# pbenner/kmerLr

Measured on NVIDIA B200. Metric: kmer_sequences_per_sec, higher is better.
Workload: dtype f64

## Files before the change

### kmerlr_b200/csrc/abi.cu

```cuda
#include <cmath>
#include <map>
#include <mutex>
#include <unordered_map>
#include <vector>

#include "common.cuh"

namespace kl {

namespace {
Ctx g_ctx;
std::mutex g_mutex;
std::unordered_map<uint64_t, std::shared_ptr<Object>> g_objects;
uint64_t g_next = 1;
thread_local std::string g_error;
}

Ctx &ctx() { return g_ctx; }

namespace {
std::multimap<size_t, void *> g_free_blocks;
std::unordered_map<void *, size_t> g_block_size;
constexpr size_t ARENA_GRAIN = (size_t)2 << 20;
}
void *arena_alloc(size_t bytes) {
  size_t want = (bytes + ARENA_GRAIN - 1) / ARENA_GRAIN * ARENA_GRAIN;
  auto it = g_free_blocks.lower_bound(want);
  if (it != g_free_blocks.end() && it->first <= 2 * want + 8 * ARENA_GRAIN) {
    void *p = it->second;
    g_free_blocks.erase(it);
    return p;
  }
  void *p = nullptr;
  cudaError_t e = cudaMalloc(&p, want);
  if (e != cudaSuccess) {
    cudaGetLastError();
    cudaStreamSynchronize(g_ctx.stream);
    for (auto &kv : g_free_blocks) { cudaFree(kv.second); g_block_size.erase(kv.second); }
    g_free_blocks.clear();
    KL_CUDA(cudaMalloc(&p, want));
  }
  g_block_size[p] = want;
  return p;
}
void arena_free(void *p) {
  auto it = g_block_size.find(p);
  if (it == g_block_size.end()) return;
  g_free_blocks.emplace(it->second, p);
}
void arena_release_all() {
  for (auto &kv : g_block_size) cudaFree(kv.first);
  g_block_size.clear();
  g_free_blocks.clear();
}

namespace {
struct ProfRec { std::string name; cudaEvent_t e0, e1; };
std::vector<ProfRec> g_prof_pending;
std::vector<cudaEvent_t> g_prof_pool;
std::unordered_map<std::string, std::pair<double, int64_t>> g_prof_totals;
cudaEvent_t prof_event() {
  if (!g_prof_pool.empty()) { cudaEvent_t e = g_prof_pool.back(); g_prof_pool.pop_back(); return e; }
  cudaEvent_t e;
  KL_CUDA(cudaEventCreate(&e));
  return e;
}
void prof_resolve() {
  if (g_prof_pending.empty()) return;
  KL_CUDA(cudaStreamSynchronize(g_ctx.stream));
  for (auto &r : g_prof_pending) {
    float ms = 0.f;
    KL_CUDA(cudaEventElapsedTime(&ms, r.e0, r.e1));
    auto &t = g_prof_totals[r.name];
    t.first += ms; t.second += 1;
    g_prof_pool.push_back(r.e0); g_prof_pool.push_back(r.e1);
  }
  g_prof_pending.clear();
}
}
void profile_begin(const char *name) {
  if (g_prof_pending.size() > 8192) prof_resolve();
  ProfRec r{name, prof_event(), prof_event()};
  KL_CUDA(cudaEventRecord(r.e0, g_ctx.stream));
  g_prof_pending.push_back(r);
}
void profile_end() { KL_CUDA(cudaEventRecord(g_prof_pending.back().e1, g_ctx.stream)); }

void require_ready() {
  if (!g_ctx.ready) fail(KMERLR_ERR_NOGPU, "kmerlr_init() has not succeeded: no usable sm_100 GPU (there is no CPU fallback)");
}

uint64_t register_object(std::shared_ptr<Object> o) {
  uint64_t h = g_next++;
  g_objects[h] = std::move(o);
  return h;
}
std::shared_ptr<Object> lookup_object(uint64_t h) {
  auto it = g_objects.find(h);
  return it == g_objects.end() ? nullptr : it->second;
}

template <typename F>
int guarded(F &&f, bool timed = true) {
  std::lock_guard<std::mutex> lock(g_mutex);
  try {
    if (g_ctx.ready) KL_CUDA(cudaSetDevice(g_ctx.device));
    if (timed && g_ctx.ready) KL_CUDA(cudaEventRecord(g_ctx.ev0, g_ctx.stream));
    f();
    if (timed && g_ctx.ready) {
      KL_CUDA(cudaEventRecord(g_ctx.ev1, g_ctx.stream));
      KL_CUDA(cudaEventSynchronize(g_ctx.ev1));
      float ms = 0.f;
      KL_CUDA(cudaEventElapsedTime(&ms, g_ctx.ev0, g_ctx.ev1));
      g_ctx.last_ms = ms;
    }
    return KMERLR_OK;
  } catch (const Error &e) {
    g_error = e.msg;
    if (g_ctx.ready) cudaGetLastError();
    return e.code;
  } catch (const std::exception &e) {
    g_error = e.what();
    return KMERLR_ERR_INTERNAL;
  }
}

}

using namespace kl;

extern "C" {

int kmerlr_version(void) { return 100; }

const char *kmerlr_last_error(void) { return g_error.c_str(); }

double kmerlr_last_device_ms(void) { return g_ctx.last_ms; }

int64_t kmerlr_launch_count(void) { return g_ctx.launches; }

int kmerlr_profile(int enable) {
  return guarded([&] {
    prof_resolve();
    if (enable) g_prof_totals.clear();
    g_ctx.profiling = enable != 0;
  }, false);
}

int kmerlr_profile_read(const char *kernel_substr, double *ms_total, int64_t *launches) {
  return guarded([&] {
    prof_resolve();
    double ms = 0.0; int64_t n = 0;
    for (auto &kv : g_prof_totals)
      if (kv.first.find(kernel_substr) != std::string::npos) { ms += kv.second.first; n += kv.second.second; }
    *ms_total = ms; *launches = n;
  }, false);
}

int kmerlr_profile_dump(char *buf, int64_t buflen) {
  return guarded([&] {
    prof_resolve();
    std::string out;
    for (auto &kv : g_prof_totals)
      out += kv.first + "\t" + std::to_string(kv.second.first) + "\t" + std::to_string(kv.second.second) + "\n";
    KL_REQUIRE((int64_t)out.size() + 1 <= buflen, "profile_dump: buffer too small");
    memcpy(buf, out.c_str(), out.size() + 1);
  }, false);
}

int kmerlr_option(const char *name, int64_t value) {
  return guarded([&] {
    KL_REQUIRE(name != nullptr, "option: null name");
    if (!strcmp(name, "implicit")) g_ctx.implicit_ok = value != 0;
    else if (!strcmp(name, "super_len")) g_ctx.super_len = (int)(value < 0 ? -1 : (value > IMP_SUPER_MAX ? IMP_SUPER_MAX : value));
    else if (!strcmp(name, "p2p")) g_ctx.p2p_ok = value != 0;
    else if (!strcmp(name, "feed_growth")) g_ctx.feed_growth = (int)(value < 100 ? 100 : (value > 400 ? 400 : value));
    else if (!strcmp(name, "small_long")) g_ctx.small_long = (int)(value < 0 ? -1 : (value > 2 ? 2 : value));
    else if (!strcmp(name, "persist_bps")) g_ctx.persist_bps = (int)(value < 0 ? 0 : value);
    else if (!strcmp(name, "p2p_allreduce")) g_ctx.p2p_allreduce = value != 0;
    else if (!strcmp(name, "persistent")) g_ctx.coop_ok = value != 0 && g_ctx.coop_supported;
    else if (!strcmp(name, "fused_ticket")) g_ctx.fused_ticket = (int)(value < 0 ? 0 : (value > 4096 ? 4096 : value));
    else if (!strcmp(name, "hot_cols")) g_ctx.hot_cols = (int)(value < 0 ? 0 : (value > 16384 ? 16384 : value));
    else fail(KMERLR_ERR_ARG, std::string("unknown option ") + name);
  }, false);
}

int kmerlr_init(int device) {
  return guarded([&] {
    if (g_ctx.ready) {
      KL_REQUIRE(device == g_ctx.device, "kmerlr_init: already initialised on another device");
      return;
    }
    int count = 0;
    cudaError_t e = cudaGetDeviceCount(&count);
    if (e != cudaSuccess || count == 0) {
      cudaGetLastError();
      fail(KMERLR_ERR_NOGPU, "no CUDA device visible (there is no CPU fallback)");
    }
    KL_REQUIRE(device >= 0 && device < count, "kmerlr_init: device index out of range");
    cudaDeviceProp prop;
    KL_CUDA(cudaGetDeviceProperties(&prop, device));
    if (prop.major != 10) fail(KMERLR_ERR_NOGPU, std::string("device is ") + prop.name + " (sm_" + std::to_string(prop.major) + std::to_string(prop.minor) + "); this library is built for sm_100a only");
    KL_CUDA(cudaSetDevice(device));
    g_ctx.device = device;
    g_ctx.sm_count = prop.multiProcessorCount;
    g_ctx.coop_supported = prop.cooperativeLaunch != 0;
    g_ctx.coop_ok = g_ctx.coop_supported;
    KL_CUDA(cudaStreamCreateWithFlags(&g_ctx.stream, cudaStreamNonBlocking));
    KL_CUDA(cudaStreamCreateWithFlags(&g_ctx.copy_stream, cudaStreamNonBlocking));
    KL_CUDA(cudaStreamCreateWithFlags(&g_ctx.alt_stream, cudaStreamNonBlocking));
    for (int i = 0; i < 2; i++) KL_CUDA(cudaEventCreateWithFlags(&g_ctx.join_ev[i], cudaEventDisableTiming));
    for (int i = 0; i < CTX_COPY_EVENTS; i++) KL_CUDA(cudaEventCreateWithFlags(&g_ctx.copy_ev[i], cudaEventDisableTiming));

    KL_CUDA(cudaEventCreate(&g_ctx.ev0));
    KL_CUDA(cudaEventCreate(&g_ctx.ev1));
    g_ctx.ready = true;
  }, false);
}

int kmerlr_shutdown(void) {
  return guarded([&] {
    g_objects.clear();
    if (g_ctx.ready) {
      cudaStreamSynchronize(g_ctx.stream);
      arena_release_all();
      comm_destroy();
      cudaEventDestroy(g_ctx.ev0); cudaEventDestroy(g_ctx.ev1);
      cudaStreamSynchronize(g_ctx.copy_stream);
      for (int i = 0; i < CTX_COPY_EVENTS; i++) cudaEventDestroy(g_ctx.copy_ev[i]);
      cudaStreamDestroy(g_ctx.copy_stream);
      cudaStreamSynchronize(g_ctx.alt_stream);
      cudaStreamDestroy(g_ctx.alt_stream);
      for (int i = 0; i < 2; i++) cudaEventDestroy(g_ctx.join_ev[i]);
      cudaStreamDestroy(g_ctx.stream);
      g_ctx = Ctx();
    }
  }, false);
}

int kmerlr_comm_unique_id(void *id128) { return guarded([&] { comm_unique_id(id128); }, false); }
int kmerlr_comm_init(int rank, int world, const void *id128) { return guarded([&] { comm_init(rank, world, id128); }, false); }
int kmerlr_comm_destroy(void) { return guarded([&] { comm_destroy(); }, false); }

int kmerlr_sequences_create(const uint8_t *seq, const int64_t *off, int64_t n, kmerlr_handle *out) {
  return guarded([&] {
    KL_REQUIRE(out, "null output handle");
    *out = register_object(sequences_create(seq, off, n));
  });
}

int kmerlr_extract_resident(const kmerlr_config *cfg, kmerlr_handle sequences, const int32_t *frozen_k,
                            const uint64_t *frozen_code, int64_t n_frozen, const int32_t *features,
                            int64_t n_features, int flags, kmerlr_handle *out) {
  return guarded([&] {
    KL_REQUIRE(cfg && out, "null argument");
    auto s = lookup<SeqSet>(sequences, "sequences");
    *out = register_object(extract(*cfg, s, frozen_k, frozen_code, n_frozen, features, n_features, flags));
  });
}

int kmerlr_extract(const kmerlr_config *cfg, const uint8_t *seq, const int64_t *off, int64_t n,
                   const int32_t *frozen_k, const uint64_t *frozen_code, int64_t n_frozen,
                   const int32_t *features, int64_t n_features, int flags, kmerlr_handle *out) {
  return guarded([&] {
    KL_REQUIRE(cfg && out, "null argument");
    *out = register_object(extract_host(*cfg, seq, off, n, frozen_k, frozen_code, n_frozen, features, n_features, flags));
  });
}

int kmerlr_matrix_info(kmerlr_handle h, int64_t *n, int64_t *m, int64_t *nnz, int64_t *n_classes) {
  return guarded([&] {
    auto M = lookup<Matrix>(h, "matrix");
    if (n) *n = M->n;
    if (m) *m = M->m;
    if (nnz) *nnz = M->nnz;
    if (n_classes) *n_classes = M->n_classes;
  }, false);
}

int kmerlr_matrix_rows_global(kmerlr_handle h, int64_t *n_global) {
  return guarded([&] {
    KL_REQUIRE(n_global, "null argument");
    *n_global = lookup<Matrix>(h, "matrix")->n_global;
  }, false);
}

int kmerlr_matrix_classes(kmerlr_handle h, int32_t *k_out, uint64_t *code_out) {
  return guarded([&] {
    auto M = lookup<Matrix>(h, "matrix");
    matrix_class_list(*M);
    for (size_t j = 0; j < M->class_k.size(); j++) { k_out[j] = M->class_k[j]; code_out[j] = M->class_code[j]; }
  }, false);
}

int kmerlr_matrix_rows(kmerlr_handle h, int64_t *rowptr, int32_t *col, double *val) {
  return guarded([&] { matrix_rows(*lookup<Matrix>(h, "matrix"), rowptr, col, val); });
}

int kmerlr_matrix_set_labels(kmerlr_handle h, const uint8_t *labels, int64_t n) {
  return guarded([&] { matrix_set_labels(*lookup<Matrix>(h, "matrix"), labels, n); });
}

int kmerlr_matrix_from_csr(int64_t n, int64_t m, const int64_t *rowptr, const int32_t *col, const double *val,
                           int flags, kmerlr_handle *out) {
  return guarded([&] {
    KL_REQUIRE(out, "null output handle");
    *out = register_object(matrix_from_csr(n, m, rowptr, col, val, flags));
  });
}

// ... 204 lines not shown
```

### kmerlr_b200/csrc/common.cuh

```cuda
#pragma once

#include <cuda_runtime.h>
#include <stdint.h>

#include <chrono>
#include <cstdio>
#include <cstdlib>
#include <cstring>
#include <memory>
#include <string>
#include <vector>

#include "../../include/kmerlr_b200.h"

namespace kl {

struct Error {
  int code;
  std::string msg;
};

[[noreturn]] inline void fail(int code, const std::string &msg) { throw Error{code, msg}; }

#define KL_CUDA(expr)                                                                              \
  do {                                                                                             \
    cudaError_t _e = (expr);                                                                       \
    if (_e != cudaSuccess)                                                                         \
      ::kl::fail(KMERLR_ERR_CUDA, std::string(#expr) + ": " + cudaGetErrorString(_e) + " (" +      \
                                      __FILE__ + ":" + std::to_string(__LINE__) + ")");            \
  } while (0)

#define KL_REQUIRE(cond, msg)                                                                      \
  do {                                                                                             \
    if (!(cond)) ::kl::fail(KMERLR_ERR_ARG, std::string(msg));                                     \
  } while (0)

#define KL_INVARIANT(cond)                                                                         \
  do {                                                                                             \
    if (!(cond)) ::kl::fail(KMERLR_ERR_INTERNAL, std::string("internal error: ") + #cond + " (" +  \
                                                     __FILE__ + ":" + std::to_string(__LINE__) + ")"); \
  } while (0)

constexpr int PEER_MAX_WORLD = 8;
constexpr int PEER_PAYLOAD = 1024 + 8;
struct PeerMail {
  unsigned long long slot[2][PEER_MAX_WORLD][PEER_PAYLOAD];
  unsigned long long flag[2][PEER_MAX_WORLD];
  unsigned long long seq;
  unsigned int senders_done;
  unsigned long long ar_flag[2][PEER_MAX_WORLD];
  unsigned long long ar_seq;
  unsigned int ar_error;
};
constexpr int64_t PEER_AR_CAP = (int64_t)4 << 20;
struct PeerBox {
  PeerMail *box[PEER_MAX_WORLD];
  unsigned long long *sym[PEER_MAX_WORLD];
  int rank, world;
};

constexpr int CTX_COPY_EVENTS = 11;
struct Ctx {
  bool ready = false;
  int device = 0;
  int sm_count = 0;
  cudaStream_t stream = nullptr;
  cudaStream_t copy_stream = nullptr;
  cudaStream_t alt_stream = nullptr;
  cudaEvent_t join_ev[2] = {nullptr, nullptr};
  cudaEvent_t copy_ev[CTX_COPY_EVENTS] = {nullptr};
  cudaEvent_t ev0 = nullptr, ev1 = nullptr;
  int64_t launches = 0;
  double last_ms = 0.0;
  bool profiling = false;
  bool implicit_ok = true;
  int super_len = -1;
  int hot_cols = 6144;
  int fused_ticket = 8;
  void *comm = nullptr;
  int rank = 0, world = 1;
  PeerBox *peer = nullptr;
  bool p2p_ok = true;
  bool p2p_allreduce = false;
  int feed_growth = 135;
  int small_long = -1;
  int persist_bps = 0;
  bool coop_supported = true;
  bool coop_ok = true;
};
Ctx &ctx();
void require_ready();

void profile_begin(const char *name);
void profile_end();

#define KL_LAUNCH(kernel, grid, block, smem, ...)                                                  \
  do {                                                                                             \
    if (::kl::ctx().profiling) ::kl::profile_begin(#kernel);                                       \
    kernel<<<(grid), (block), (smem), ::kl::ctx().stream>>>(__VA_ARGS__);                          \
    if (::kl::ctx().profiling) ::kl::profile_end();                                                \
    ::kl::ctx().launches++;                                                                        \
    KL_CUDA(cudaGetLastError());                                                                   \
  } while (0)

inline void sync_stream() { KL_CUDA(cudaStreamSynchronize(ctx().stream)); }

struct Trace {
  bool on;
  std::chrono::steady_clock::time_point t0, last;
  const char *what;
  explicit Trace(const char *w) : what(w) {
    static int env = -1;
    if (env < 0) { const char *e = getenv("KMERLR_TRACE"); env = (e && *e == '1') ? 1 : 0; }
    on = env == 1;
    if (on) t0 = last = std::chrono::steady_clock::now();
  }
  void mark(const char *phase, bool sync = true) {
    if (!on) return;
    if (sync) cudaStreamSynchronize(ctx().stream);
    auto t = std::chrono::steady_clock::now();
    fprintf(stderr, "[trace %s] %-28s %8.3f ms (total %8.3f)\n", what, phase,
            std::chrono::duration<double, std::milli>(t - last).count(),
            std::chrono::duration<double, std::milli>(t - t0).count());
    last = t;
  }
};

void *arena_alloc(size_t bytes);
void arena_free(void *p);
void arena_release_all();

template <typename T>
struct DevBuf {
  T *p = nullptr;
  size_t n = 0;
  DevBuf() = default;
  explicit DevBuf(size_t count) { alloc(count); }
  DevBuf(const DevBuf &) = delete;
  DevBuf &operator=(const DevBuf &) = delete;
  DevBuf(DevBuf &&o) noexcept : p(o.p), n(o.n) { o.p = nullptr; o.n = 0; }
  DevBuf &operator=(DevBuf &&o) noexcept {
    if (this != &o) { release(); p = o.p; n = o.n; o.p = nullptr; o.n = 0; }
    return *this;
  }
  ~DevBuf() { release(); }
  void alloc(size_t count) {
    release();
    n = count;
    if (count) p = (T *)arena_alloc(count * sizeof(T) + 32);
  }
  void release() {
    if (p) arena_free(p);
    p = nullptr; n = 0;
  }
  void zero() { if (n) KL_CUDA(cudaMemsetAsync(p, 0, n * sizeof(T), ctx().stream)); }
  void upload(const T *h, size_t count) {
    if (count) KL_CUDA(cudaMemcpyAsync(p, h, count * sizeof(T), cudaMemcpyHostToDevice, ctx().stream));
  }
  void download(T *h, size_t count) const {
    if (count) KL_CUDA(cudaMemcpyAsync(h, p, count * sizeof(T), cudaMemcpyDeviceToHost, ctx().stream));
  }
  size_t bytes() const { return n * sizeof(T); }
};

struct Object {
  virtual ~Object() {}
};

struct SeqSet : Object {
  int64_t n = 0;
  int64_t total_bases = 0;
  int64_t total_blocks = 0;
  int64_t max_len = 0;
  DevBuf<int64_t> len;
  DevBuf<int64_t> blk;
  DevBuf<uint32_t> bits2;
  DevBuf<uint16_t> inv16;
};

enum ValType : int { VAL_ONE = 0, VAL_U32 = 1, VAL_F64 = 2 };

constexpr int IMP_MAX_N = 10;
constexpr int IMP_SUPER_MAX = 11;
constexpr uint32_t NOCOL = 0xFFFFFFFFu;
struct Implicit {
  std::shared_ptr<SeqSet> seqs;
  int M = 0, N = 0, op = 0;
  int Mlo = 0;
  uint32_t level_off[16] = {0};
  uint32_t fo[16] = {0};
  DevBuf<uint32_t> bitmap, rank;
  bool binarized = false;
  int low_words = 0;
  DevBuf<uint32_t> lowbits;
  DevBuf<uint32_t> lowcol;
  DevBuf<int64_t> evptr;
  DevBuf<uint32_t> events;
};

struct Rows {
  const int64_t *rowptr;
  const uint32_t *rowcnt;
  int64_t stride;
#ifdef __CUDACC__
  __device__ __forceinline__ void range(int64_t row, int64_t &a, int64_t &b) const {
    if (stride) { a = row * stride; b = a + rowcnt[row]; }
    else { a = rowptr[row]; b = rowptr[row + 1]; }
  }
#endif
};

struct Matrix : Object {
  int64_t n = 0, m = 0, nnz = 0;
  ValType vt = VAL_U32;
  int64_t row_stride = 0;
  DevBuf<uint32_t> rowcnt;
  DevBuf<int64_t> rowptr;
  DevBuf<uint32_t> col;
  DevBuf<uint32_t> val_u32;
  DevBuf<double> val_f64;
  Rows rows() const { return Rows{rowptr.p, rowcnt.p, row_stride}; }
  bool has_csc = false;
  DevBuf<int64_t> colptr;
  DevBuf<uint32_t> crow;
  DevBuf<uint32_t> cval_u32;
  DevBuf<double> cval_f64;
  bool has_sliced = false;
  DevBuf<int64_t> slice_off;
  DevBuf<uint32_t> scol;
  DevBuf<uint32_t> sval_u32;
  DevBuf<double> sval_f64;
  bool has_packed = false, packable = false;
  int pack_row_bits = 0;
  DevBuf<uint32_t> spack, cpack;
  int bv_grid = 0, bv_row_bits = 0, bv_rows = 0;
  bool bv_ok = false;
  DevBuf<int64_t> bv_off;
  DevBuf<uint32_t> bv_pack;
  bool has_labels = false;
  DevBuf<uint8_t> labels;
  int64_t n_pos = 0, n_neg = 0;
  bool counts_global = true;
  int64_t n_classes = 0;
  DevBuf<uint32_t> class_ids;
  int class_M = 0, class_N = 0;
  uint32_t class_level_off[16] = {0};
  bool classes_on_host = true;
  std::vector<int32_t> class_k;
  std::vector<uint64_t> class_code;
  bool sharded = false;
  int64_t n_global = 0;
  bool has_maxsq = false;
  double maxsq = 0.0;
  bool has_vmax = false;
  double vmax = 0.0;
  std::shared_ptr<Implicit> imp;
  bool has_local_stats = false;
  double local_maxsq = 0.0, local_vmax = 0.0;
};

uint64_t register_object(std::shared_ptr<Object> o);
std::shared_ptr<Object> lookup_object(uint64_t h);
template <typename T>
std::shared_ptr<T> lookup(uint64_t h, const char *what) {
  auto o = std::dynamic_pointer_cast<T>(lookup_object(h));
  if (!o) fail(KMERLR_ERR_ARG, std::string("invalid ") + what + " handle");
  return o;
}

void exclusive_scan_i64(const int64_t *in, int64_t *out, int64_t n);
void exclusive_scan_u32_to_i64(const uint32_t *in, int64_t *out, int64_t n);
void exclusive_scan_u32(const uint32_t *in, uint32_t *out, int64_t n);
std::shared_ptr<SeqSet> sequences_create(const uint8_t *seq, const int64_t *off, int64_t n);
struct SeqFeed {
  virtual ~SeqFeed() {}
  virtual int chunks() const = 0;
  virtual int64_t first_row(int c) const = 0;
  virtual void feed(int c) = 0;
};
std::shared_ptr<SeqSet> sequences_begin_chunked(const uint8_t *seq, const int64_t *off, int64_t n, std::unique_ptr<SeqFeed> &feed);
std::shared_ptr<Matrix> extract(const kmerlr_config &cfg, std::shared_ptr<SeqSet> seqs, const int32_t *frozen_k,
                                const uint64_t *frozen_code, int64_t n_frozen, const int32_t *features,
                                int64_t n_features, int flags);
std::shared_ptr<Matrix> extract_host(const kmerlr_config &cfg, const uint8_t *seq, const int64_t *off, int64_t n,
                                     const int32_t *frozen_k, const uint64_t *frozen_code, int64_t n_frozen,
                                     const int32_t *features, int64_t n_features, int flags);
std::shared_ptr<Matrix> extract_gapped(const kmerlr_config &cfg, std::shared_ptr<SeqSet> seqs, const int32_t *frozen_k,
                                       const uint64_t *frozen_code, int64_t n_frozen, int flags);
void matrix_class_list(Matrix &M);
std::shared_ptr<Matrix> matrix_from_csr(int64_t n, int64_t m, const int64_t *rowptr, const int32_t *col,
                                        const double *val, int flags);
void matrix_rows(Matrix &M, int64_t *rowptr, int32_t *col, double *val);
void matrix_set_labels(Matrix &M, const uint8_t *labels, int64_t n);
void matrix_label_counts(Matrix &M);
void matrix_column_moments(Matrix &M, double *sum, double *sumsq, double *absmax, int64_t *count);
void matrix_pair_moments(Matrix &M, double *sum, double *sumsq, double *absmax, int64_t *count);
std::shared_ptr<Matrix> matrix_transform(Matrix &M, const double *offset, const double *scale, int64_t len);
void matrix_compact(Matrix &M);
void ensure_csc(Matrix &M);
void ensure_sliced(Matrix &M);
bool ensure_packed(Matrix &M);
bool ensure_blockview(Matrix &M, int grid);
std::shared_ptr<Matrix> matrix_reduce(Matrix &M, const int64_t *sel, int64_t nsel);
double matrix_maxsq(Matrix &M);
double matrix_vmax(Matrix &M);
void linear_pdf(Matrix &M, const double *theta, int64_t ntheta, int cooc, double *out_host, bool logpdf);
void gradient(Matrix &M, const double *theta, int64_t ntheta, const double cw[2], double lambda, int cooc,
              double *g_host, DevBuf<double> *g_dev = nullptr);
double loss(Matrix &M, const double *theta, int64_t ntheta, const double cw[2], double lambda, int cooc);
void coordinate(Matrix &M, double *theta, int64_t ntheta, const double cw_hook[2], double l1reg, double l2reg,
                double epsilon, double epsilon_loss, int64_t max_iter, double hook[2], int64_t *sweeps_out,
                double *delta_out);
void proxgrad(Matrix &M, double *theta, int64_t ntheta, const double cw[2], double lambda, double l2,
              double step_factor, double epsilon, double epsilon_loss, int64_t max_iter, double hook[2],
              int64_t *iters, double *delta);
void select(Matrix &M, const double cw[2], int cooc, int64_t N, double theta0, const int64_t *active_idx,
            const double *active_theta, int64_t n_active, int tie, double eps_lambda, double prev_lambda,
            uint8_t *mask, int64_t ntheta, double *lambda_out, int64_t *c_out, int *ok_out, double *g_out);
void select_from_gradient(const double *g, int64_t ntheta, int64_t N, const int64_t *active_idx, const double *active_theta,
                          int64_t n_active, int tie, double eps_lambda, double prev_lambda, uint8_t *mask,
                          double *lambda_out, int64_t *c_out, int *ok_out);
void score_windows(const kmerlr_model *models, int n_models, const SeqSet &s, int64_t W, int64_t step,
                   double *out_host, std::shared_ptr<Object> *out_dev, int layout = 0, SeqFeed *feed = nullptr);
int64_t wiggle_records(const double *pred, bool pred_on_device, int64_t n, char *out);
void save_wiggle(const char *filename, const char *track_name, int64_t n_regions, const char *const *seqnames,
                 const int64_t *from, const int64_t *slot_off, const double *pred, bool pred_on_device, int64_t window_size,
                 int64_t window_step);
std::string class_name(const kmerlr_config &cfg, int k, uint64_t code);
void export_kmers(Matrix &M, const kmerlr_config &cfg, const char *filename, bool as_float);
void export_path(const char *filename, int64_t n, const int64_t *estimator, const double *lambda, const double *norm,
                 const int64_t *theta_off, const double *theta);
void export_trace(const char *filename, int64_t n, const int64_t *duration_ns, const int64_t *iteration, const double *change,
                  const int64_t *nonzero, const double *lambda, const double *loss);

void comm_unique_id(void *id128);
void comm_init(int rank, int world, const void *id128);
void comm_destroy();
void comm_allreduce_sum_f64(double *dev, int64_t count);
void comm_allreduce_sum_i64(int64_t *dev, int64_t count);
void comm_allreduce_sum_i64_fast(int64_t *dev, int64_t count);
void comm_check_peer_errors();
void comm_allreduce_max_f64(double *dev, int64_t count);
void comm_allreduce_max_u8(uint8_t *dev, int64_t count);
void comm_allgather_f64(const double *dev_in, double *dev_out, int64_t count_per_rank);
void comm_allgather_bytes(const void *dev_in, void *dev_out, int64_t bytes_per_rank);

#ifdef __CUDACC__
__device__ __forceinline__ unsigned lane_id() { return threadIdx.x & 31u; }
__device__ __forceinline__ unsigned lanemask_lt() {
  unsigned m;
  asm("mov.u32 %0, %%lanemask_lt;" : "=r"(m));
  return m;
}
__device__ __forceinline__ uint32_t swap_pairs(uint32_t y) {
  return ((y >> 1) & 0x55555555u) | ((y & 0x55555555u) << 1);
}
__device__ __forceinline__ uint32_t kmer_op(uint32_t u, int k, int op) {
  if (op == 1) return swap_pairs(__brev(~u)) >> (32 - 2 * k);
  if (op == 2) return (~u) & ((1u << (2 * k)) - 1u);
  return swap_pairs(__brev(u)) >> (32 - 2 * k);
}
__device__ __forceinline__ double warp_sum(double v) {
#pragma unroll
  for (int o = 16; o > 0; o >>= 1) v += __shfl_xor_sync(0xffffffffu, v, o);
  return v;
}
__device__ __forceinline__ double warp_sum_down(double v) {
#pragma unroll
  for (int o = 16; o > 0; o >>= 1) v += __shfl_down_sync(0xffffffffu, v, o);
  return v;
}
__device__ __forceinline__ uint32_t smem_u32(const void *p) { return (uint32_t)__cvta_generic_to_shared(p); }
__device__ __forceinline__ void mbar_init(unsigned long long *bar, uint32_t arrivals) {
  asm volatile("mbarrier.init.shared::cta.b64 [%0], %1;" ::"r"(smem_u32(bar)), "r"(arrivals) : "memory");
  asm volatile("fence.mbarrier_init.release.cluster;" ::: "memory");
}
// ... 27 lines not shown
```

### kmerlr_b200/csrc/extract.cu

```cuda
#include <cmath>

#include "extract_kernel.cuh"

namespace kl {

namespace {

using namespace xk;

__global__ void pack_kernel(const uint8_t *__restrict__ seq, const int64_t *__restrict__ off,
                            const int64_t *__restrict__ blk, int64_t n, int64_t total_blocks, int64_t w0, int64_t w1,
                            uint32_t *__restrict__ bits2, uint16_t *__restrict__ inv16) {
  int64_t w = w0 + (int64_t)blockIdx.x * blockDim.x + threadIdx.x;
  if (w >= w1) return;
  const int64_t b = w >> 2;
  int64_t g = (int64_t)((double)b * (double)n / (double)total_blocks);
  g = g < 0 ? 0 : (g > n - 1 ? n - 1 : g);
  int64_t lo, hi, stepw = 1;
  if (blk[g] <= b) {
    lo = g; hi = g + 1;
    while (hi < n && blk[hi] <= b) { lo = hi; stepw <<= 1; hi = hi + stepw < n ? hi + stepw : n; }
  } else {
    hi = g; lo = g - 1;
    while (lo > 0 && blk[lo] > b) { hi = lo; stepw <<= 1; lo = lo - stepw > 0 ? lo - stepw : 0; }
// ... 7 lines not shown
  uint32_t bits = 0, inv = 0;
#pragma unroll
  for (int j = 0; j < 16; j++) {
    if (j0 + j < L) {
      uint32_t ch = s[j0 + j] | 0x20u, c;
      if (ch == 'a') c = 0; else if (ch == 'c') c = 1; else if (ch == 'g') c = 2; else if (ch == 't') c = 3;
      else { c = 0; inv |= 1u << j; }
      bits |= c << (2 * j);
    }
  }
  bits2[w] = bits;
  inv16[w] = (uint16_t)inv;
}

__global__ void popc_words(const uint32_t *__restrict__ bm, int64_t nw, uint32_t *__restrict__ out) {
  int64_t i = (int64_t)blockIdx.x * blockDim.x + threadIdx.x;
  if (i < nw) out[i] = __popc(bm[i]);
}
__global__ void pack_exchange(const uint32_t *__restrict__ bm, int64_t nw, unsigned long long n_local,
                              const unsigned long long *__restrict__ stats, uint32_t *__restrict__ out) {
  int64_t i = (int64_t)blockIdx.x * blockDim.x + threadIdx.x;
  if (i < nw) out[i] = bm[i];
  if (i == 0) {
    unsigned long long v[3] = {n_local, stats[0], stats[1]};
    for (int k = 0; k < 3; k++) { out[nw + 2 * k] = (uint32_t)v[k]; out[nw + 2 * k + 1] = (uint32_t)(v[k] >> 32); }
  }
}
__global__ void merge_exchange(const uint32_t *__restrict__ all, int world, int64_t nw, uint32_t *__restrict__ bm,
                               unsigned long long *__restrict__ res) {
  int64_t i = (int64_t)blockIdx.x * blockDim.x + threadIdx.x;
  const int64_t per = nw + 6;
  if (i < nw) {
    uint32_t v = 0;
    for (int r = 0; r < world; r++) v |= all[(int64_t)r * per + i];
    bm[i] = v;
  }
  if (i == 0) {
    unsigned long long n = 0, a = 0, b = 0;
    for (int r = 0; r < world; r++) {
      const uint32_t *t = all + (int64_t)r * per + nw;
      n += (unsigned long long)t[0] | ((unsigned long long)t[1] << 32);
      const unsigned long long x = (unsigned long long)t[2] | ((unsigned long long)t[3] << 32);
      const unsigned long long y = (unsigned long long)t[4] | ((unsigned long long)t[5] << 32);
      a = x > a ? x : a; b = y > b ? y : b;
    }
    res[0] = n; res[1] = a; res[2] = b;
  }
}
__global__ void enumerate_bits(const uint32_t *__restrict__ bm, const uint32_t *__restrict__ rank, int64_t nw,
                               uint32_t *__restrict__ ids) {
  int64_t w = (int64_t)blockIdx.x * blockDim.x + threadIdx.x;
  if (w >= nw) return;
  uint32_t v = bm[w], r = rank[w];
  while (v) {
    int b = __ffs(v) - 1;
    ids[r++] = (uint32_t)(w * 32 + b);
    v &= v - 1;
  }
}

struct LevelInfo {
  int M, N, op;
  uint32_t level_off[16];
};
__global__ void all_classes_bits(const LevelInfo I, uint32_t *__restrict__ bm, int64_t nw) {
  int64_t w = (int64_t)blockIdx.x * blockDim.x + threadIdx.x;
  if (w >= nw) return;
  const uint32_t id0 = (uint32_t)(w * 32);
  int k = I.M;
  while (k < I.N && id0 >= I.level_off[k + 1]) k++;
  const uint32_t u0 = id0 - I.level_off[k], nk = 1u << (2 * k);
  uint32_t v = 0;
  for (int b = 0; b < 32; b++) {
    const uint32_t u = u0 + b;
    if (u < nk && (I.op == 0 || u <= kmer_op(u, k, I.op))) v |= 1u << b;
  }
  bm[w] = v;
}
__global__ void interleave_numbering(const uint32_t *__restrict__ bits, const uint32_t *__restrict__ rank, int64_t nw,
                                     uint2 *__restrict__ out) {
  int64_t w = (int64_t)blockIdx.x * blockDim.x + threadIdx.x;
  if (w < nw) out[w] = make_uint2(bits[w], rank[w]);
}
__global__ void bitmaps_differ(const uint32_t *__restrict__ a, const uint32_t *__restrict__ b, int64_t nw,
                               uint32_t *__restrict__ flag) {
  int64_t w = (int64_t)blockIdx.x * blockDim.x + threadIdx.x;
  if (w < nw && a[w] != b[w]) atomicOr(flag, 1u);
}
__global__ void renumber_rows(uint32_t *__restrict__ col, const uint32_t *__restrict__ rowcnt, int64_t stride, int64_t n,
                              const uint32_t *__restrict__ ids, const uint32_t *__restrict__ bm,
                              const uint32_t *__restrict__ rank, const uint32_t *__restrict__ rowdup) {
  int64_t row = ((int64_t)blockIdx.x * blockDim.x + threadIdx.x) >> 5;
  if (row >= n) return;
  const unsigned lane = lane_id();
  uint32_t *c = col + row * stride;
  const uint32_t cnt = rowcnt[row];
  for (uint32_t j = lane; j < cnt; j += 32) {
    const uint32_t id = __ldg(ids + c[j]), w = __ldg(bm + (id >> 5));
    c[j] = __ldg(rank + (id >> 5)) + __popc(w & ((1u << (id & 31)) - 1u));
  }
  const uint32_t nd = rowdup ? rowdup[row] : 0u;
  uint32_t *t = c + stride - 1;
  for (uint32_t j = lane; j < nd; j += 32) {
    const uint32_t id = __ldg(ids + t[-(int64_t)j]), w = __ldg(bm + (id >> 5));
    t[-(int64_t)j] = __ldg(rank + (id >> 5)) + __popc(w & ((1u << (id & 31)) - 1u));
  }
}
__global__ void gather_events(const uint32_t *__restrict__ col, int64_t stride, int64_t n,
                              const int64_t *__restrict__ evptr, uint32_t *__restrict__ events) {
  int64_t row = ((int64_t)blockIdx.x * blockDim.x + threadIdx.x) >> 5;
  if (row >= n) return;
  const unsigned lane = lane_id();
  const int64_t a = evptr[row], cnt = evptr[row + 1] - a;
  const uint32_t *t = col + (row + 1) * stride - 1;
  for (int64_t j = lane; j < cnt; j += 32) events[a + j] = t[-j];
}
__global__ void low_columns(const uint2 *__restrict__ tl, uint32_t tl_cnt, int slots, const uint32_t *__restrict__ bm,
                            const uint32_t *__restrict__ rank, uint32_t *__restrict__ lowcol) {
  const int j = blockIdx.x * blockDim.x + threadIdx.x;
  if (j >= slots) return;
  uint32_t col = NOCOL;
  if ((uint32_t)j < tl_cnt) {
    const uint32_t id = tl[j].y, w = bm[id >> 5], bit = 1u << (id & 31);
    if (w & bit) col = rank[id >> 5] + __popc(w & (bit - 1u));
  }
  lowcol[j] = col;
}

__device__ __forceinline__ uint32_t row_lookup(const uint32_t *col, const uint32_t *val, int64_t a, int64_t b, uint32_t c) {
  int64_t lo = a, hi = b;
  while (lo < hi) {
    int64_t mid = (lo + hi) >> 1;
    if (col[mid] < c) lo = mid + 1; else hi = mid;
  }
  if (lo < b && col[lo] == c) return val ? val[lo] : 1u;
  return 0u;
}
template <bool WRITE>
__global__ void features_rows(const Rows R, const uint32_t *__restrict__ col,
                              const uint32_t *__restrict__ val, int64_t n, const int32_t *__restrict__ feat,
                              int64_t nf, uint32_t *__restrict__ cnt_out, const int64_t *__restrict__ orowptr,
                              uint32_t *__restrict__ ocol, uint32_t *__restrict__ oval) {
  int64_t row = ((int64_t)blockIdx.x * blockDim.x + threadIdx.x) >> 5;
  if (row >= n) return;
  unsigned lane = lane_id();
  int64_t a, b;
  R.range(row, a, b);
  int64_t outp = WRITE ? orowptr[row] : 0;
  uint32_t tot = 0;
  for (int64_t j0 = 0; j0 < nf; j0 += 32) {
    int64_t j = j0 + lane;
    uint32_t v = 0;
    if (j < nf) {
      int32_t i1 = feat[2 * j], i2 = feat[2 * j + 1];
      uint32_t c1 = row_lookup(col, val, a, b, (uint32_t)i1);
      if (i1 == i2) v = c1;
      else if (c1) v = c1 * row_lookup(col, val, a, b, (uint32_t)i2);
    }
    unsigned km = __ballot_sync(0xffffffffu, v != 0);
    if (WRITE && v != 0) {
      int64_t pos = outp + __popc(km & lanemask_lt());
      ocol[pos] = (uint32_t)j;
      if (oval) oval[pos] = v;
    }
    outp += __popc(km);
    tot += __popc(km);
  }
  if (!WRITE && lane == 0) cnt_out[row] = tot;
}

// ... 115 lines not shown
  hf.doff.alloc((size_t)n + 1);
  hf.doff.upload(off, (size_t)n + 1);
  s->len.alloc((size_t)(n ? n : 1));
  s->blk.alloc((size_t)n + 1);
  if (n > 0) {
    DevBuf<uint32_t> nblk((size_t)n);
    KL_LAUNCH(seq_meta_kernel, (unsigned)((n + 255) / 256), 256, 0, hf.doff.p, n, s->len.p, nblk.p);
    exclusive_scan_u32_to_i64(nblk.p, s->blk.p, n);
  } else {
    s->blk.zero();
  }
  const int64_t words = blocks * 4;
  s->bits2.alloc((size_t)words + 4);
  s->inv16.alloc((size_t)words + 4);
  KL_CUDA(cudaMemsetAsync(s->bits2.p + words, 0, 4 * sizeof(uint32_t), ctx().stream));
  KL_CUDA(cudaMemsetAsync(s->inv16.p + words, 0, 4 * sizeof(uint16_t), ctx().stream));
  hf.raw.alloc((size_t)(s->total_bases ? s->total_bases : 1));
  KL_CUDA(cudaEventRecord(ctx().copy_ev[CTX_COPY_EVENTS - 1], ctx().stream));
  KL_CUDA(cudaStreamWaitEvent(ctx().copy_stream, ctx().copy_ev[CTX_COPY_EVENTS - 1], 0));
  tr.mark("offsets, metadata");
  return s;
}

namespace {
struct FeedImpl : SeqFeed {
  HostFeed hf;
  std::shared_ptr<SeqSet> s;
  int chunks() const override { return hf.nchunks; }
  int64_t first_row(int c) const override { return hf.row[c]; }
  void feed(int c) override { if (s->n > 0) hf.feed(*s, c); }
};
}

std::shared_ptr<SeqSet> sequences_begin_chunked(const uint8_t *seq, const int64_t *off, int64_t n, std::unique_ptr<SeqFeed> &feed) {
  auto f = std::make_unique<FeedImpl>();
  f->s = sequences_begin(seq, off, n, f->hf, true);
  auto s = f->s;
  feed = std::move(f);
  return s;
}

std::shared_ptr<SeqSet> sequences_create(const uint8_t *seq, const int64_t *off, int64_t n) {
  HostFeed hf;
  auto s = sequences_begin(seq, off, n, hf);
  if (n > 0) hf.feed(*s, -1);
  sync_stream();
  return s;
}

static std::shared_ptr<Matrix> apply_features(Matrix &cls, const int32_t *features, int64_t nf) {
  for (int64_t j = 0; j < nf; j++) {
    KL_REQUIRE(features[2 * j] >= 0 && features[2 * j] < cls.m && features[2 * j + 1] >= 0 && features[2 * j + 1] < cls.m,
               "features: class index out of range");
  }
  auto out = std::make_shared<Matrix>();
  out->n = cls.n; out->m = nf; out->vt = cls.vt;
  matrix_class_list(cls);
  out->class_k = cls.class_k; out->class_code = cls.class_code; out->n_classes = cls.n_classes;
  out->sharded = cls.sharded; out->n_global = cls.n_global;
  DevBuf<int32_t> dfeat((size_t)(2 * nf));
  dfeat.upload(features, (size_t)(2 * nf));
  DevBuf<uint32_t> cnt((size_t)(cls.n ? cls.n : 1));
  const uint32_t *val = cls.vt == VAL_U32 ? cls.val_u32.p : nullptr;
  unsigned grid = (unsigned)((cls.n * 32 + 127) / 128);
  out->rowptr.alloc((size_t)cls.n + 1);
  if (cls.n > 0) {
    KL_LAUNCH((features_rows<false>), grid, 128, 0, cls.rows(), cls.col.p, val, cls.n, dfeat.p, nf, cnt.p, nullptr,
              nullptr, nullptr);
    exclusive_scan_u32_to_i64(cnt.p, out->rowptr.p, cls.n);
    KL_CUDA(cudaMemcpyAsync(&out->nnz, out->rowptr.p + cls.n, sizeof(int64_t), cudaMemcpyDeviceToHost, ctx().stream));
    sync_stream();
  } else {
    out->rowptr.zero(); out->nnz = 0;
  }
  out->col.alloc((size_t)(out->nnz ? out->nnz : 1));
  if (out->vt == VAL_U32) out->val_u32.alloc((size_t)(out->nnz ? out->nnz : 1));
  if (cls.n > 0)
    KL_LAUNCH((features_rows<true>), grid, 128, 0, cls.rows(), cls.col.p, val, cls.n, dfeat.p, nf, nullptr,
              out->rowptr.p, out->col.p, out->vt == VAL_U32 ? out->val_u32.p : nullptr);
  sync_stream();
  return out;
}

static std::shared_ptr<Matrix> extract_impl(const kmerlr_config &cfg, std::shared_ptr<SeqSet> seqs,
                                            const int32_t *frozen_k, const uint64_t *frozen_code, int64_t n_frozen,
                                            const int32_t *features, int64_t n_features, int flags, HostFeed *feed) {
  require_ready();
  const SeqSet &s = *seqs;
  KL_REQUIRE(cfg.alphabet == 0 || cfg.alphabet == 1, "alphabet: 0 = nucleotide, 1 = gapped nucleotide (IUPAC is not implemented)");
  if (cfg.alphabet == 1) {
    KL_REQUIRE(n_features == 0 || n_frozen > 0, "an explicit feature list needs a frozen class list");
    if (feed && s.n > 0) feed->feed(*seqs, -1);
    auto g = extract_gapped(cfg, seqs, frozen_k, frozen_code, n_frozen, flags);
    if (n_features > 0) return apply_features(*g, features, n_features);
    return g;
  }
  KL_REQUIRE(cfg.M >= 1 && cfg.M <= cfg.N, "need 1 <= M <= N");
  KL_REQUIRE(n_features == 0 || n_frozen > 0, "an explicit feature list needs a frozen class list");
  {
    const int nops = (cfg.complement != 0) + (cfg.reverse != 0) + (cfg.revcomp != 0);
    const bool long_sorted = cfg.N > KB_MAX && (s.max_len + 31) / 32 > 64;
    const bool long_tables = s.max_len >= 65536 && cfg.M <= KT_MAX;
    if (nops > 1 || cfg.N > MAX_N || long_sorted || long_tables) {
      if (feed && s.n > 0) feed->feed(*seqs, -1);
      auto g = extract_gapped(cfg, seqs, frozen_k, frozen_code, n_frozen, flags);
      if (n_features > 0) return apply_features(*g, features, n_features);
      return g;
    }
  }
  const bool sharded = (flags & KMERLR_FLAG_SHARDED) != 0 && ctx().world > 1;

  XParams P{};
  P.M = cfg.M; P.N = cfg.N; P.binarize = cfg.binarize != 0;
  P.op = cfg.revcomp ? 1 : (cfg.complement ? 2 : (cfg.reverse ? 3 : 0));
  P.t_lo = cfg.M; P.t_hi = cfg.N < KT_MAX ? cfg.N : KT_MAX;
  const int64_t steps = (s.max_len + 31) / 32;
  const int kb = steps > 64 ? KB_MAX : KB_DEFAULT;
  P.b_lo = cfg.M > KT_MAX + 1 ? cfg.M : KT_MAX + 1; P.b_hi = cfg.N < kb ? cfg.N : kb;
  P.s_lo = cfg.M > kb + 1 ? cfg.M : kb + 1;
  P.n = s.n;
  P.len = s.len.p; P.blk = s.blk.p; P.bits2 = s.bits2.p; P.inv16 = s.inv16.p;
  uint64_t dense = 0;
  for (int k = cfg.M; k <= cfg.N; k++) {
    P.level_off[k] = (uint32_t)dense;
    dense += ((1ull << (2 * k)) + 31) / 32 * 32;
  }
  P.level_off[cfg.N + 1] = (uint32_t)dense;
  const int64_t nbits = (int64_t)dense, nw = (nbits + 31) / 32;
  int64_t stride = 0;
  for (int k = cfg.M; k <= cfg.N; k++) {
    int64_t inst = s.max_len - k + 1; if (inst < 0) inst = 0;
    int64_t cls = (int64_t)1 << (2 * k);
    stride += inst < cls ? inst : cls;
  }
  if (stride < 1) stride = 1;
  P.stride = stride;
  bool hybrid = P.binarize && cfg.N <= IMP_MAX_N && n_features == 0 && s.n > 0;
  for (int k = cfg.M > KT_MAX + 1 ? cfg.M : KT_MAX + 1; k <= cfg.N && hybrid; k++)
    if (s.max_len - k + 1 > ((int64_t)1 << (2 * k))) hybrid = false;
  KL_INVARIANT(s.max_len < 65536 || P.t_lo > P.t_hi);
  KL_REQUIRE(s.max_len < ((int64_t)1 << 30), "sequence too long");
  int E = 0;
  if (P.s_lo <= cfg.N) {
    E = 2; while (E < steps && E < 128) E <<= 1;
    KL_INVARIANT(E <= 64);
  }
  P.bm_words = 0; P.pf_words = 0;
  int nbl = 0;
  for (int k = P.b_lo; k <= P.b_hi; k++) {
    P.bm_off[k] = (uint32_t)P.bm_words; P.pf_off[k] = (uint32_t)P.pf_words;
    P.bm_words += 1 << (2 * k - 5); P.pf_words += 1 << (2 * k - 7);
    nbl++;
  }
  P.pf_words = (P.pf_words + 3) / 4 * 4;
  P.ts_words = 32 * E > TAB_WORDS ? 32 * E : TAB_WORDS;
  P.warp_words = P.bm_words + P.pf_words + P.ts_words + 8;
  P.warp_words = (P.warp_words + 3) / 4 * 4;
  {
    int top = cfg.N < OBS_MAX_LEVEL ? cfg.N : OBS_MAX_LEVEL;
    P.obs_id_words = top >= cfg.M ? (int)(P.level_off[top + 1] / 32) : 0;
    P.obs_id_words = (P.obs_id_words + 3) / 4 * 4;
  }
  if (P.t_lo <= P.t_hi) P.tl = table_classes(P.op, P.t_lo, P.t_hi, P.level_off, &P.tl_cnt);
  P.obs_words = P.obs_id_words + (P.t_lo <= P.t_hi ? (int)((P.tl_cnt + 127) / 128 * 4) : 0);
  Trace tr("extract");
  auto out = std::make_shared<Matrix>();
  out->n = s.n; out->vt = P.binarize ? VAL_ONE : VAL_U32;
  out->sharded = sharded; out->n_global = s.n;
  out->row_stride = stride;
  out->col.alloc((size_t)(s.n ? s.n * stride : 1));
  if (!P.binarize) out->val_u32.alloc((size_t)(s.n ? s.n * stride : 1));
  out->rowcnt.alloc((size_t)(s.n ? s.n : 1));
  DevBuf<uint32_t> dummy_cnt(1);
  DevBuf<uint32_t> nb((size_t)nw), nbrank((size_t)nw + 1), pc((size_t)nw), bitmap((size_t)nw);
  std::vector<uint32_t> frozen_bits;
  LevelInfo LI{};
  LI.M = cfg.M; LI.N = cfg.N; LI.op = P.op;
  for (int k = cfg.M; k <= cfg.N + 1; k++) LI.level_off[k] = P.level_off[k];
  if (n_frozen > 0) {
    frozen_bits.assign((size_t)nw, 0u);
    uint64_t prev = 0;
    for (int64_t j = 0; j < n_frozen; j++) {
      int k = frozen_k[j];
      KL_REQUIRE(k >= cfg.M && k <= cfg.N && frozen_code[j] < (1ull << (2 * k)), "frozen class outside [M,N]");
      uint64_t id = (uint64_t)P.level_off[k] + frozen_code[j];
      KL_REQUIRE(j == 0 || id > prev, "frozen class list must be sorted by (k, code) without duplicates");
      prev = id;
      frozen_bits[id >> 5] |= 1u << (id & 31);
    }
    nb.upload(frozen_bits.data(), (size_t)nw);
  } else {
    KL_LAUNCH(all_classes_bits, (unsigned)((nw + 255) / 256), 256, 0, LI, nb.p, nw);
  }
  KL_LAUNCH(popc_words, (unsigned)((nw + 255) / 256), 256, 0, nb.p, nw, pc.p);
  exclusive_scan_u32(pc.p, nbrank.p, nw);
  bitmap.zero();
  DevBuf<uint32_t> full(1);
  full.zero();
  P.full = full.p; P.nb_words = nw;
  DevBuf<unsigned long long> stats(2);
  stats.zero();
  P.st_id = out->col.p; P.st_cnt = P.binarize ? dummy_cnt.p : out->val_u32.p; P.rowcnt = out->rowcnt.p;
  DevBuf<uint2> nbx((size_t)nw);
  KL_LAUNCH(interleave_numbering, (unsigned)((nw + 255) / 256), 256, 0, nb.p, nbrank.p, nw, nbx.p);
  P.bitmap = bitmap.p; P.nbx = nbx.p; P.filter = n_frozen > 0; P.stats = stats.p;
  P.mark = n_frozen == 0;
  DevBuf<uint32_t> lowbits, rowdup;
  if (hybrid) {
    P.events = 1;
    P.low_words = P.t_lo <= P.t_hi ? (int)((P.tl_cnt + 31) / 32) : 0;
    if (P.low_words) { lowbits.alloc((size_t)s.n * P.low_words); P.lowbits = lowbits.p; }
    rowdup.alloc((size_t)s.n);
    P.rowdup = rowdup.p;
  }
  DevBuf<uint32_t> ovf;
  P.ovf_stride = nbl * (s.max_len > 0 ? s.max_len : 1);
  if (nbl && (!P.binarize || hybrid) && s.n > 0) {
    ovf.alloc((size_t)ctx().sm_count * 64 * (size_t)P.ovf_stride);
    P.ovf = ovf.p;
  }
  tr.mark("alloc");

  if (s.n > 0) {
    const int nchunks = feed ? feed->nchunks : 1;
    DevBuf<uint32_t> ticket((size_t)nchunks);
    ticket.zero();
    const bool two_streams = feed && nchunks > 1;
    DevBuf<uint32_t> ovf2;
    if (two_streams && P.ovf) ovf2.alloc((size_t)ctx().sm_count * 64 * (size_t)P.ovf_stride);
    struct StreamSwap {
      cudaStream_t saved;
      explicit StreamSwap(cudaStream_t run) : saved(ctx().stream) { ctx().stream = run; }
      ~StreamSwap() { ctx().stream = saved; }
    };
    if (two_streams) {
      KL_CUDA(cudaEventRecord(ctx().join_ev[0], ctx().stream));
      KL_CUDA(cudaStreamWaitEvent(ctx().alt_stream, ctx().join_ev[0], 0));
    }
    uint32_t *const ovf_even = P.ovf;
    for (int c = 0; c < nchunks; c++) {
      StreamSwap on((two_streams && (c & 1)) ? ctx().alt_stream : ctx().stream);
      P.ovf = (two_streams && (c & 1) && ovf_even) ? ovf2.p : ovf_even;
      P.ticket = ticket.p + c;
      const int64_t r0 = feed ? feed->row[c] : 0, r1 = feed ? feed->row[c + 1] : s.n;
      if (feed) feed->feed(*seqs, c);
      P.row0 = r0; P.n = r1;
      switch (E) {
        case 0: launch_extract<0>(P); break;
        case 2: launch_extract<2>(P); break;
        case 4: launch_extract<4>(P); break;
        case 8: launch_extract<8>(P); break;
        case 16: launch_extract<16>(P); break;
        case 32: launch_extract<32>(P); break;
        default: launch_extract<64>(P); break;
      }
    }
    P.ovf = ovf_even;
    if (two_streams) {
      KL_CUDA(cudaEventRecord(ctx().join_ev[1], ctx().alt_stream));
      KL_CUDA(cudaStreamWaitEvent(ctx().stream, ctx().join_ev[1], 0));
    }
    P.row0 = 0; P.n = s.n;
  }
  tr.mark("extract_kernel");
  DevBuf<uint32_t> differ(1);
  differ.zero();
  DevBuf<unsigned long long> gres(3);
  if (sharded) {
    const int64_t xw = n_frozen == 0 ? nw : 0, per = xw + 6;
    DevBuf<uint32_t> mine((size_t)per), all((size_t)(per * ctx().world));
    KL_LAUNCH(pack_exchange, (unsigned)((xw + 256) / 256), 256, 0, bitmap.p, xw, (unsigned long long)s.n, stats.p, mine.p);
    comm_allgather_bytes(mine.p, all.p, per * 4);
    KL_LAUNCH(merge_exchange, (unsigned)((xw + 256) / 256), 256, 0, all.p, ctx().world, xw, bitmap.p, gres.p);
  }
  if (n_frozen == 0)
    KL_LAUNCH(bitmaps_differ, (unsigned)((nw + 255) / 256), 256, 0, bitmap.p, nb.p, nw, differ.p);
  DevBuf<int64_t> rp((size_t)s.n + 1);
  if (s.n > 0) exclusive_scan_u32_to_i64(out->rowcnt.p, rp.p, s.n); else rp.zero();
  int64_t nn = s.n;
  unsigned long long hres[3] = {0, 0, 0};
  if (sharded) gres.download(hres, 3);
  uint32_t m32 = 0, hdiffer = 0;
  unsigned long long hstats[2] = {0, 0};
  DevBuf<int64_t> evptr;
  int64_t n_events = 0;
  if (hybrid) {
    evptr.alloc((size_t)s.n + 1);
    exclusive_scan_u32_to_i64(rowdup.p, evptr.p, s.n);
    KL_CUDA(cudaMemcpyAsync(&n_events, evptr.p + s.n, sizeof(int64_t), cudaMemcpyDeviceToHost, ctx().stream));
  }
  KL_CUDA(cudaMemcpyAsync(&m32, nbrank.p + nw, sizeof(uint32_t), cudaMemcpyDeviceToHost, ctx().stream));
  KL_CUDA(cudaMemcpyAsync(&out->nnz, rp.p + s.n, sizeof(int64_t), cudaMemcpyDeviceToHost, ctx().stream));
  differ.download(&hdiffer, 1);
  stats.download(hstats, 2);
  sync_stream();
  if (sharded) {
    nn = (int64_t)hres[0];
    out->maxsq = (double)hres[1]; out->vmax = (double)hres[2];
    out->has_maxsq = out->has_vmax = true;
  }
  out->n_global = nn;
  out->has_local_stats = true;
  out->local_maxsq = (double)hstats[0]; out->local_vmax = (double)hstats[1];
  tr.mark("sizes");
  if (hdiffer) {
    DevBuf<uint32_t> rank2((size_t)nw + 1), ids_nb((size_t)(m32 ? m32 : 1));
    KL_LAUNCH(popc_words, (unsigned)((nw + 255) / 256), 256, 0, bitmap.p, nw, pc.p);
    exclusive_scan_u32(pc.p, rank2.p, nw);
    KL_LAUNCH(enumerate_bits, (unsigned)((nw + 255) / 256), 256, 0, nb.p, nbrank.p, nw, ids_nb.p);
    if (s.n > 0)
      KL_LAUNCH(renumber_rows, (unsigned)((s.n * 32 + 127) / 128), 128, 0, out->col.p, out->rowcnt.p, stride, s.n, ids_nb.p,
                bitmap.p, rank2.p, hybrid ? rowdup.p : (const uint32_t *)nullptr);
    KL_CUDA(cudaMemcpyAsync(&m32, rank2.p + nw, sizeof(uint32_t), cudaMemcpyDeviceToHost, ctx().stream));
    sync_stream();
    nb = std::move(bitmap); nbrank = std::move(rank2);
    tr.mark("renumber");
  }
  out->m = (int64_t)m32;
  out->n_classes = (int64_t)m32;
  out->class_ids.alloc((size_t)(m32 ? m32 : 1));
  KL_LAUNCH(enumerate_bits, (unsigned)((nw + 255) / 256), 256, 0, nb.p, nbrank.p, nw, out->class_ids.p);
  out->class_M = cfg.M; out->class_N = cfg.N; out->classes_on_host = false;
  for (int k = cfg.M; k <= cfg.N + 1; k++) out->class_level_off[k] = P.level_off[k];
  if (n_features > 0) { sync_stream(); return apply_features(*out, features, n_features); }
  if ((!P.binarize || hybrid) && cfg.N <= IMP_MAX_N && s.n > 0 && m32 > 0) {
    auto imp = std::make_shared<Implicit>();
    imp->seqs = seqs; imp->M = cfg.M; imp->N = cfg.N; imp->op = P.op;
    imp->Mlo = P.binarize ? (cfg.M > KT_MAX + 1 ? cfg.M : KT_MAX + 1) : cfg.M;
    uint32_t fo = 0;
    for (int k = cfg.M; k <= cfg.N + 1; k++) {
      imp->level_off[k] = P.level_off[k];
      imp->fo[k] = fo;
      if (k <= cfg.N && k >= imp->Mlo) fo += 1u << (2 * k);
    }
    if (P.binarize) {
      imp->binarized = true;
      imp->low_words = P.low_words;
      imp->lowcol.alloc((size_t)(P.low_words ? P.low_words * 32 : 1));
      if (P.low_words)
        KL_LAUNCH(low_columns, (unsigned)((P.low_words * 32 + 127) / 128), 128, 0, P.tl, P.tl_cnt, P.low_words * 32, nb.p,
                  nbrank.p, imp->lowcol.p);
      imp->lowbits = std::move(lowbits);
      imp->events.alloc((size_t)(n_events ? n_events : 1));
      KL_LAUNCH(gather_events, (unsigned)((s.n * 32 + 127) / 128), 128, 0, out->col.p, stride, s.n, evptr.p, imp->events.p);
      imp->evptr = std::move(evptr);
    }
    imp->bitmap = std::move(nb); imp->rank = std::move(nbrank);
    out->imp = imp;
  }
  sync_stream();
  return out;
}

void matrix_class_list(Matrix &M) {
  if (M.classes_on_host) return;
  std::vector<uint32_t> hid((size_t)M.n_classes);
  M.class_ids.download(hid.data(), (size_t)M.n_classes);
  sync_stream();
  M.class_k.resize((size_t)M.n_classes); M.class_code.resize((size_t)M.n_classes);
  int k = M.class_M;
  for (size_t j = 0; j < hid.size(); j++) {
    while (k < M.class_N && hid[j] >= M.class_level_off[k + 1]) k++;
    M.class_k[j] = k; M.class_code[j] = hid[j] - M.class_level_off[k];
  }
  M.classes_on_host = true;
}

std::shared_ptr<Matrix> extract(const kmerlr_config &cfg, std::shared_ptr<SeqSet> seqs, const int32_t *frozen_k,
                                const uint64_t *frozen_code, int64_t n_frozen, const int32_t *features,
                                int64_t n_features, int flags) {
  return extract_impl(cfg, seqs, frozen_k, frozen_code, n_frozen, features, n_features, flags, nullptr);
}

std::shared_ptr<Matrix> extract_host(const kmerlr_config &cfg, const uint8_t *seq, const int64_t *off, int64_t n,
                                     const int32_t *frozen_k, const uint64_t *frozen_code, int64_t n_frozen,
                                     const int32_t *features, int64_t n_features, int flags) {
  HostFeed hf;
  auto s = sequences_begin(seq, off, n, hf);
  auto out = extract_impl(cfg, s, frozen_k, frozen_code, n_frozen, features, n_features, flags, &hf);
  sync_stream();
  return out;
}

}
```

### kmerlr_b200/csrc/logistic.cu

```cuda
#include <cooperative_groups.h>

#include "common.cuh"

#include <cmath>

namespace kl {

namespace {

constexpr int RED_BLOCKS = 256;

struct PgState {
  long long iter;
  int done;
  int first;
  double delta, loss_old, loss_new, lossval;
  int error;
};

__device__ __forceinline__ int64_t ind2sub(int64_t n, int64_t k1, int64_t k2) {
  return n + (n * (n - 1) / 2) - (n - k1) * ((n - k1) - 1) / 2 + k2 - k1;
}

template <typename VT>
// ... 98 lines not shown
    double s = 0.0;
    for (int64_t p = a + lane; p < b; p += 32) s += valf(val, p) * __ldg(theta + col[p] + 1);
    s = warp_sum_down(s);
    double w = 0.0;
    if (lane == 0) {
      double z = theta[0] + s, r = -log_add0(-z);
      if (labels[row]) { w = inv_n * cw1 * (exp(r) - 1.0); lossterm[row] = -cw1 * r; }
      else             { w = inv_n * cw0 * exp(r);         lossterm[row] = cw0 * log_add0(z); }
      bias_acc += __double2ll_rn(w * scale);
    }
    if (!scatter) return;
    w = __shfl_sync(0xffffffffu, w, 0);
    const double ws = w * scale;
    for (int64_t p = a + lane; p < b; p += 32) {
      const uint32_t c = col[p];
      const unsigned long long q = (unsigned long long)__double2ll_rn(ws * valf(val, p));
      if (c < (uint32_t)hot_cols) {
        const uint32_t lo = (uint32_t)q, hi = (uint32_t)(q >> 32);
        const uint32_t old = atomicAdd(&hot_lo[c], lo);
        const uint32_t add_hi = hi + ((old + lo) < old ? 1u : 0u);
        if (add_hi) atomicAdd(&hot_hi[c], add_hi);
      } else atomicAdd(&G[c + 1], q);
    }
  };
  if (ticket) {
    for (;;) {
      unsigned long long t0 = 0;
      if (lane == 0) t0 = atomicAdd(ticket, (unsigned long long)rpb);
      const int64_t first = (int64_t)__shfl_sync(0xffffffffu, t0, 0);
      if (first >= n) break;
      const int64_t last = first + rpb < n ? first + rpb : n;
      for (int64_t row = first; row < last; row++) do_row(row);
    }
  } else {
    const int64_t first = (int64_t)blockIdx.x * rpb, last = first + rpb < n ? first + rpb : n;
    for (int64_t row = first + (threadIdx.x >> 5); row < last; row += (blockDim.x >> 5)) do_row(row);
  }
  if (lane == 0 && bias_acc != 0) atomicAdd(&G[0], (unsigned long long)bias_acc);
  __syncthreads();
  for (int i = threadIdx.x; i < hot_cols; i += blockDim.x) {
    unsigned long long v = ((unsigned long long)hot_hi[i] << 32) | hot_lo[i];
    if (v) atomicAdd(&G[i + 1], v);
  }
}

struct ImpParams {
  int M, N, op;
  int Mlo;
  int S, c;
  uint32_t sup0;
  uint32_t level_off[16], fo[16];
};

__global__ void imp_build_T(const ImpParams P, const uint32_t *__restrict__ bitmap, const uint32_t *__restrict__ rank,
                            const double *__restrict__ theta, double *__restrict__ T, int64_t total,
                            const PgState *st) {
  if (st && st->done == 1) return;
  const int64_t t = (int64_t)blockIdx.x * blockDim.x + threadIdx.x;
  if (t >= total) return;
  int j = P.Mlo;
  while (j < P.N && t >= (int64_t)P.fo[j + 1]) j++;
  const uint32_t u = (uint32_t)(t - P.fo[j]);
  double s = 0.0;
  for (int k = P.Mlo; k <= j; k++) {
    uint32_t c = u >> (2 * (j - k));
    if (P.op) c = min(c, kmer_op(c, k, P.op));
    const uint32_t id = P.level_off[k] + c, w = bitmap[id >> 5], bit = 1u << (id & 31);
    if (w & bit) s += theta[rank[id >> 5] + __popc(w & (bit - 1u)) + 1];
  }
  T[t] = s;
}

__global__ void imp_build_TS(const ImpParams P, double *__restrict__ T, const PgState *st) {
  if (st && st->done == 1) return;
  const uint32_t U = blockIdx.x * blockDim.x + threadIdx.x;
  if (U >= (1u << (2 * P.S))) return;
  const uint32_t maskN = (1u << (2 * P.N)) - 1u;
  const double *TN = T + P.fo[P.N];
  double s = 0.0;
  for (int t = 0; t < P.c; t++) s += TN[(U >> (2 * (P.S - P.N - t))) & maskN];
  T[P.sup0 + U] = s;
}

__global__ void imp_fold_super(const ImpParams P, unsigned long long *__restrict__ H, const PgState *st) {
  if (st && st->done == 1) return;
  const uint32_t U = blockIdx.x * blockDim.x + threadIdx.x;
  if (U >= (1u << (2 * P.S))) return;
  const unsigned long long h = H[P.sup0 + U];
  if (!h) return;
  const uint32_t maskN = (1u << (2 * P.N)) - 1u;
  for (int t = 0; t < P.c; t++) atomicAdd(H + P.fo[P.N] + ((U >> (2 * (P.S - P.N - t))) & maskN), h);
}

__global__ void imp_build_low(const uint32_t *__restrict__ lowcol, int low_words, int lwp,
                              const double *__restrict__ theta, double *__restrict__ lowtab, const PgState *st) {
  if (st && st->done == 1) return;
  const int e = blockIdx.x * blockDim.x + threadIdx.x;
  if (e >= 128 * lwp) return;
  const int l = e % lwp, v = (e / lwp) & 15, i = e / (16 * lwp);
  double s = 0.0;
  if (l < low_words)
    for (int b = 0; b < 4; b++)
      if ((v >> b) & 1) {
        const uint32_t col = lowcol[l * 32 + 4 * i + b];
        if (col != NOCOL) s += theta[col + 1];
      }
  lowtab[e] = s;
}

constexpr uint32_t IMP_NOIDX = 0xFFFFFFFFu, IMP_SINGLES = 0xFFFFFFFEu;

struct ImpWindow {
  unsigned long long rev;
  uint32_t inv;
  int left;
  __device__ __forceinline__ void load(const uint32_t *__restrict__ b2, const uint16_t *__restrict__ iv, int L, int p0) {
    left = L - p0;
    if (p0 >= L) { rev = 0ull; inv = 0xFFFFFFFFu; return; }
    const int wi = p0 >> 4, sh = p0 & 15;
    const uint32_t w0 = __ldg(b2 + wi), w1 = __ldg(b2 + wi + 1), w2 = __ldg(b2 + wi + 2);
    const uint32_t lo = __funnelshift_r(w0, w1, 2 * sh), hi = __funnelshift_r(w1, w2, 2 * sh);
    rev = ((unsigned long long)swap_pairs(__brev(lo)) << 32) | swap_pairs(__brev(hi));
    const unsigned long long iw = (unsigned long long)__ldg(iv + wi) | ((unsigned long long)__ldg(iv + wi + 1) << 16) |
                                  ((unsigned long long)__ldg(iv + wi + 2) << 32);
    inv = (uint32_t)(iw >> sh);
    if (left < 32) inv |= 0xFFFFFFFFu << left;
  }
  __device__ __forceinline__ uint32_t code(int x, int k) const {
    return (uint32_t)(rev >> (64 - 2 * (x + k))) & ((1u << (2 * k)) - 1u);
  }
};

__device__ __forceinline__ uint32_t imp_group(const ImpParams &P, const ImpWindow &W, int x) {
  if (x >= W.left) return IMP_NOIDX;
  const uint32_t bits = (W.inv >> x) & ((1u << P.S) - 1u);
  return bits == 0u ? P.sup0 + W.code(x, P.S) : IMP_SINGLES;
}
__device__ __forceinline__ uint32_t imp_single(const ImpParams &P, const ImpWindow &W, int x) {
  const uint32_t bits = W.inv >> x;
  int lf = bits ? __ffs(bits) - 1 : P.N;
  if (lf > P.N) lf = P.N;
  if (lf < P.Mlo) return IMP_NOIDX;
  return P.fo[lf] + W.code(x, lf);
}

struct ImpArgs {
  int64_t n;
  const int64_t *len, *blk;
  const uint32_t *bits2;
  const uint16_t *inv16;
  const double *T, *theta;
  const uint8_t *labels;
  double cw0, cw1, inv_n, scale;
  unsigned long long *H, *G;
  double *lossterm;
  const PgState *st;
  int scatter;
  int rpb;
  int gw;
  const uint32_t *lowbits;
  int low_words, lwp;
  const double *lowtab;
  const int64_t *evptr;
  const uint32_t *events;
  unsigned long long *q_out;
};

constexpr int IMP_R = 2;

#ifndef KL_IMP_MINB
#define KL_IMP_MINB 0
#endif
template <int CACHE, bool BIN>
__global__ void
// ... 109 lines not shown
      const int G = gpl[r];
      if (CACHE > 0) {
#pragma unroll
        for (int i = 0; i < CC; i++) {
          if (IDX[r][i] < IMP_SINGLES) atomicAdd(A.H + IDX[r][i], q);
          else if (IDX[r][i] == IMP_SINGLES)
            for (int t = 0; t < c; t++) {
              const uint32_t i1 = imp_single(P, W[r], i * c + t);
              if (i1 != IMP_NOIDX) atomicAdd(A.H + i1, q);
            }
        }
      } else {
        const int L = (int)A.len[row];
        const uint32_t *b2 = A.bits2 + A.blk[row] * 4;
        const uint16_t *iv = A.inv16 + A.blk[row] * 4;
        const int p0 = (int)lane * G * c;
        for (int g0 = 0; g0 < G; g0 += A.gw) {
          ImpWindow V;
          V.load(b2, iv, L, p0 + g0 * c);
          const int ge = G - g0 < A.gw ? G - g0 : A.gw;
          for (int i = 0; i < ge; i++) {
            const uint32_t ix = imp_group(P, V, i * c);
            if (ix == IMP_SINGLES) {
              for (int t = 0; t < c; t++) {
                const uint32_t i1 = imp_single(P, V, i * c + t);
                if (i1 != IMP_NOIDX) atomicAdd(A.H + i1, q);
              }
            } else if (ix != IMP_NOIDX) atomicAdd(A.H + ix, q);
          }
        }
      }
      if (BIN) {
        const unsigned long long nq = 0ull - q;
        const int64_t e0 = A.evptr[row];
        const uint32_t nd = (uint32_t)(A.evptr[row + 1] - e0);
        for (uint32_t e = lane; e < nd; e += 32) atomicAdd(A.G + A.events[e0 + e] + 1, nq);
      }
    }
  }
  if (bias_acc != 0) atomicAdd(&s_bias, (unsigned long long)bias_acc);
  __syncthreads();
  if (threadIdx.x == 0 && s_bias != 0ull) atomicAdd(&A.G[0], s_bias);
}

__global__ void __launch_bounds__(256) low_accumulate(const uint32_t *__restrict__ lowbits, int low_words, int w0, int64_t n,
                                                      const unsigned long long *__restrict__ q,
                                                      const uint32_t *__restrict__ lowcol, unsigned long long *__restrict__ G,
                                                      const PgState *st) {
  if (st && st->done == 1) return;
  __shared__ unsigned long long sacc[32 * 32];
  const unsigned lane = lane_id();
  const int word = w0 + (int)lane, wib = threadIdx.x >> 5;
  const bool on = word < low_words;
  const int64_t nwarps = ((int64_t)gridDim.x * blockDim.x) >> 5;
  unsigned long long acc[32];
#pragma unroll
  for (int b = 0; b < 32; b++) acc[b] = 0ull;
  for (int64_t row = ((int64_t)blockIdx.x * blockDim.x + threadIdx.x) >> 5; row < n; row += nwarps) {
    const unsigned long long qq = q[row];
    const uint32_t w = on ? __ldcs(lowbits + row * low_words + word) : 0u;
#pragma unroll
    for (int b = 0; b < 32; b++)
      if ((w >> b) & 1u) acc[b] += qq;
  }
  for (int i = threadIdx.x; i < 1024; i += blockDim.x) sacc[i] = 0ull;
  __syncthreads();
  for (int v = 0; v < (int)(blockDim.x >> 5); v++) {
    if (wib == v) {
#pragma unroll
      for (int b = 0; b < 32; b++) sacc[b * 32 + lane] += acc[b];
    }
    __syncthreads();
  }
  for (int i = threadIdx.x; i < 1024; i += blockDim.x) {
    const int b = i >> 5, l = i & 31;
    const unsigned long long v = sacc[i];
    if (v && w0 + l < low_words) {
      const uint32_t col = lowcol[(w0 + l) * 32 + b];
      if (col != NOCOL) atomicAdd(G + col + 1, v);
    }
  }
}

__global__ void imp_fold_level(const ImpParams P, int j, unsigned long long *__restrict__ H, const PgState *st) {
  if (st && st->done == 1) return;
  const uint32_t u = blockIdx.x * blockDim.x + threadIdx.x;
  if (u >= (1u << (2 * j))) return;
  const unsigned long long *c = H + P.fo[j + 1] + 4ull * u;
  H[P.fo[j] + u] += c[0] + c[1] + c[2] + c[3];
}

__global__ void imp_columns(const ImpParams P, const uint32_t *__restrict__ col_id, int64_t m,
                            const unsigned long long *__restrict__ F, unsigned long long *__restrict__ G,
                            const PgState *st) {
  if (st && st->done == 1) return;
  const int64_t j = (int64_t)blockIdx.x * blockDim.x + threadIdx.x;
  if (j >= m) return;
  const uint32_t id = col_id[j];
  int k = P.M;
  while (k < P.N && id >= P.level_off[k + 1]) k++;
  if (k < P.Mlo) return;
  const uint32_t c = id - P.level_off[k];
  unsigned long long g = F[P.fo[k] + c];
  if (P.op) { const uint32_t r = kmer_op(c, k, P.op); if (r != c) g += F[P.fo[k] + r]; }
  G[j + 1] += g;
}

template <typename VT>
__global__ void scatter_w(const Rows R, const uint32_t *__restrict__ col,
                          const VT *__restrict__ val, int64_t n, const double *__restrict__ w, double scale,
                          unsigned long long *__restrict__ G) {
  int64_t row = ((int64_t)blockIdx.x * blockDim.x + threadIdx.x) >> 5;
  if (row >= n) return;
  unsigned lane = lane_id();
  const double ws = w[row] * scale;
  if (lane == 0) atomicAdd(&G[0], (unsigned long long)__double2ll_rn(ws));
  int64_t a, b;
  R.range(row, a, b);
  for (int64_t p = a + lane; p < b; p += 32)
    atomicAdd(&G[col[p] + 1], (unsigned long long)__double2ll_rn(ws * valf(val, p)));
}

__global__ void finalize_g(const unsigned long long *__restrict__ G, int64_t count, double inv_scale,
                           double *__restrict__ g) {
  int64_t j = (int64_t)blockIdx.x * blockDim.x + threadIdx.x;
  if (j < count) g[j] = (double)(long long)G[j] * inv_scale;
}

constexpr int PAIR_T = 32;
constexpr int PAIR_CH = 256;
template <typename VT>
__global__ void __launch_bounds__(256) pairs_gradient(const int64_t *__restrict__ colptr, const uint32_t *__restrict__ crow,
                                                      const VT *__restrict__ cval, int64_t m, int64_t n, int ntile,
                                                      const double *__restrict__ w, double *__restrict__ g) {
  extern __shared__ __align__(16) double Bd[];
  __shared__ int64_t pb[PAIR_T];
  double *st_t = Bd + PAIR_CH * PAIR_T + (threadIdx.x >> 5) * PAIR_CH;
  unsigned short *st_r = reinterpret_cast<unsigned short *>(Bd + PAIR_CH * PAIR_T + 8 * PAIR_CH) + (threadIdx.x >> 5) * PAIR_CH;
  int64_t rest = blockIdx.x;
  int ta = 0;
  while (rest >= ntile - ta) { rest -= ntile - ta; ta++; }
  const int tb = ta + (int)rest;
  const int64_t a0 = (int64_t)ta * PAIR_T, b0 = (int64_t)tb * PAIR_T;
  const unsigned lane = lane_id();
  const int wib = threadIdx.x >> 5;
  int64_t pa[4], ea[4];
  double acc[4];
#pragma unroll
  for (int i = 0; i < 4; i++) {
    const int64_t a = a0 + wib * 4 + i;
    pa[i] = a < m ? colptr[a] : 0; ea[i] = a < m ? colptr[a + 1] : 0;
    acc[i] = 0.0;
  }
  if (threadIdx.x < PAIR_T) pb[threadIdx.x] = b0 + threadIdx.x < m ? colptr[b0 + threadIdx.x] : 0;
  for (int64_t lo = 0; lo < n; lo += PAIR_CH) {
    const int64_t hi = lo + PAIR_CH < n ? lo + PAIR_CH : n;
    for (int i = threadIdx.x; i < PAIR_CH * PAIR_T / 2; i += blockDim.x) reinterpret_cast<double2 *>(Bd)[i] = make_double2(0.0, 0.0);
    __syncthreads();
#pragma unroll
    for (int i = 0; i < 4; i++) {
      const int bc = wib * 4 + i;
      const int64_t b = b0 + bc;
      if (b >= m) continue;
      int64_t p = pb[bc];
      const int64_t end = colptr[b + 1];
      for (;;) {
        const int64_t q = p + lane;
        const uint32_t r = q < end ? crow[q] : 0xFFFFFFFFu;
        const bool in = q < end && (int64_t)r < hi;
        if (in) Bd[(r - lo) * PAIR_T + bc] = valf(cval, q);
        const int cnt = __popc(__ballot_sync(0xffffffffu, in));
        p += cnt;
        if (cnt < 32) break;
      }
      __syncwarp();
      if (lane == 0) pb[bc] = p;
    }
    __syncthreads();
#pragma unroll
    for (int i = 0; i < 4; i++) {
      int64_t p = pa[i];
      int cnt_tot = 0;
      for (;;) {
        const int64_t q = p + lane;
        const uint32_t r = q < ea[i] ? crow[q] : 0xFFFFFFFFu;
        const bool in = q < ea[i] && (int64_t)r < hi;
        if (in) { st_r[cnt_tot + lane] = (unsigned short)(r - lo); st_t[cnt_tot + lane] = __ldg(w + r) * valf(cval, q); }
        const int cnt = __popc(__ballot_sync(0xffffffffu, in));
        p += cnt; cnt_tot += cnt;
        if (cnt < 32) break;
      }
      pa[i] = p;
      __syncwarp();
      double a_ = acc[i];
      int e = 0;
      for (; e + 4 <= cnt_tot; e += 4) {
        double d[4], t[4];
#pragma unroll
        for (int q = 0; q < 4; q++) { t[q] = st_t[e + q]; d[q] = Bd[(int)st_r[e + q] * PAIR_T + lane]; }
#pragma unroll
        for (int q = 0; q < 4; q++) a_ += t[q] * d[q];
      }
      for (; e < cnt_tot; e++) a_ += st_t[e] * Bd[(int)st_r[e] * PAIR_T + lane];
      acc[i] = a_;
      __syncwarp();
    }
    __syncthreads();
  }
#pragma unroll
  for (int i = 0; i < 4; i++) {
    const int64_t a = a0 + wib * 4 + i, b = b0 + lane;
    if (a < m && b < m && a < b) g[ind2sub(m, a, b)] = acc[i];
  }
}

__global__ void add_l1_sign(const double *__restrict__ theta, double *__restrict__ g, int64_t ntheta, double lambda) {
  int64_t j = (int64_t)blockIdx.x * blockDim.x + threadIdx.x;
  if (j < 1 || j >= ntheta) return;
  if (theta[j] < 0) g[j] -= lambda; else if (theta[j] > 0) g[j] += lambda;
}

__global__ void sum_ranks(const double *__restrict__ gathered, int world, int64_t count, double *__restrict__ out) {
  int64_t j = (int64_t)blockIdx.x * blockDim.x + threadIdx.x;
  if (j >= count) return;
  double s = 0.0;
  for (int r = 0; r < world; r++) s += gathered[(int64_t)r * count + j];
  out[j] = s;
}

__global__ void pack_loss_slots(const PgState *st, const double *__restrict__ local, unsigned long long *__restrict__ slots,
                                int rank, int world) {
  if (st && st->done == 1) return;
  const int r = threadIdx.x;
  if (r < world) slots[r] = r == rank ? (unsigned long long)__double_as_longlong(local[0]) : 0ull;
}
__global__ void unpack_loss_slots(const PgState *st, const unsigned long long *__restrict__ slots, int world,
                                  double *__restrict__ out) {
  if (st && st->done == 1) return;
  if (threadIdx.x == 0) {
    double s = 0.0;
    for (int r = 0; r < world; r++) s += __longlong_as_double((long long)slots[r]);
    out[0] = s;
  }
}

__global__ void l1_partials(const PgState *st, const double *__restrict__ theta, int64_t ntheta, double lambda,
                            double *__restrict__ l1part) {
  if (st && st->done == 1) return;
  __shared__ double sh[256];
  double s = 0.0;
  if (!isnan(lambda) && lambda != 0.0)
    for (int64_t j = 1 + (int64_t)blockIdx.x * blockDim.x + threadIdx.x; j < ntheta; j += (int64_t)gridDim.x * blockDim.x)
      s += lambda * fabs(theta[j]);
  sh[threadIdx.x] = s;
  __syncthreads();
  for (int o = 128; o > 0; o >>= 1) {
    if ((int)threadIdx.x < o) sh[threadIdx.x] += sh[threadIdx.x + o];
    __syncthreads();
  }
  if (threadIdx.x == 0) l1part[blockIdx.x] = sh[0];
}
__global__ void hook_kernel(PgState *st, const double *__restrict__ losssum, const double *__restrict__ l1part, int nparts,
                            double inv_n, double eps_loss) {
  if (st->done == 1) return;
  double l1 = 0.0;
  for (int b = threadIdx.x; b < nparts; b += 32) l1 += l1part[b];
  l1 = warp_sum_down(l1);
  if (threadIdx.x == 0) {
    double l = losssum[0] * inv_n + l1;
    st->lossval = l;
    if (st->first) { st->first = 0; return; }
    double t = st->loss_old; st->loss_old = st->loss_new; st->loss_new = t;
    if (eps_loss != 0.0) {
      st->loss_new = l;
      if (st->done == 0 && fabs(st->loss_old - st->loss_new) < eps_loss) st->done = 1;
    }
    if (st->done == 2) st->done = 1;
  }
}

__global__ void prox_update(const PgState *st, double *__restrict__ theta, const unsigned long long *__restrict__ G,
                            double inv_scale, int64_t ntheta, double step, double lambda,
                            double *__restrict__ blockmax) {
  if (st->done) return;
  __shared__ double shx[256], shd[256], shn[256];
  double mx = 0.0, md = 0.0, nn = 0.0;
  for (int64_t k = (int64_t)blockIdx.x * blockDim.x + threadIdx.x; k < ntheta; k += (int64_t)gridDim.x * blockDim.x) {
    double g = (double)(long long)G[k] * inv_scale;
    double t0 = theta[k], t1 = t0 - step * g;
    if (k > 0) {
      if (t1 >= 0.0) t1 = fmax(fabs(t1) - step * lambda, 0.0);
      else           t1 = -fmax(fabs(t1) - step * lambda, 0.0);
    }
    theta[k] = t1;
    if (isnan(t1)) nn = 1.0;
    mx = fmax(mx, fabs(t1));
    md = fmax(md, fabs(t1 - t0));
  }
  shx[threadIdx.x] = mx; shd[threadIdx.x] = md; shn[threadIdx.x] = nn;
  __syncthreads();
  for (int o = 128; o > 0; o >>= 1) {
    if ((int)threadIdx.x < o) {
      shx[threadIdx.x] = fmax(shx[threadIdx.x], shx[threadIdx.x + o]);
      shd[threadIdx.x] = fmax(shd[threadIdx.x], shd[threadIdx.x + o]);
      shn[threadIdx.x] = fmax(shn[threadIdx.x], shn[threadIdx.x + o]);
    }
    __syncthreads();
  }
  if (threadIdx.x == 0) { blockmax[3 * blockIdx.x] = shx[0]; blockmax[3 * blockIdx.x + 1] = shd[0]; blockmax[3 * blockIdx.x + 2] = shn[0]; }
}
__global__ void prox_finish(PgState *st, const double *__restrict__ blockmax, int nblocks, double eps, long long max_iter) {
  if (st->done) return;
  double mx = 0.0, md = 0.0, nn = 0.0;
  for (int i = threadIdx.x; i < nblocks; i += 32) {
    mx = fmax(mx, blockmax[3 * i]); md = fmax(md, blockmax[3 * i + 1]); nn = fmax(nn, blockmax[3 * i + 2]);
  }
#pragma unroll
  for (int o = 16; o > 0; o >>= 1) {
    mx = fmax(mx, __shfl_xor_sync(0xffffffffu, mx, o));
    md = fmax(md, __shfl_xor_sync(0xffffffffu, md, o));
    nn = fmax(nn, __shfl_xor_sync(0xffffffffu, nn, o));
  }
  if (threadIdx.x == 0) {
    st->iter += 1;
    if (nn != 0.0) { st->delta = nan(""); st->done = 1; return; }
    st->delta = mx != 0.0 ? md / mx : md;
    if ((mx != 0.0 && md / mx <= eps) || (mx == 0.0 && md == 0.0)) st->done = 1;
    else if (st->iter >= max_iter) st->done = 2;
  }
}

constexpr int SMALL_MAX_THETA = 1024;

template <int BT = 256>
__device__ __forceinline__ void small_tail(PgState *st, const double *blockloss, int nblocks, double *theta,
                                           unsigned long long *G,
                                           double inv_scale, int64_t ntheta, double inv_n, double lambda,
                                           double eps_loss, double step, double eps, long long max_iter,
                                           bool clear_g = true, int replicas = 1) {
  constexpr int NW = BT / 32;
  __shared__ double sh[3][NW];
  __shared__ int s_done;
  const int t = threadIdx.x, lane = t & 31, wid = t >> 5;
  double s = 0.0, l1 = 0.0;
  for (int i = t; i < nblocks; i += 4 * BT) {
    const double v0 = __ldcg(blockloss + i);
    const double v1 = i + BT < nblocks ? __ldcg(blockloss + i + BT) : 0.0;
    const double v2 = i + 2 * BT < nblocks ? __ldcg(blockloss + i + 2 * BT) : 0.0;
    const double v3 = i + 3 * BT < nblocks ? __ldcg(blockloss + i + 3 * BT) : 0.0;
    s += v0; s += v1; s += v2; s += v3;
  }
  if (!isnan(lambda) && lambda != 0.0)
    for (int64_t j = 1 + t; j < ntheta; j += BT) l1 += lambda * fabs(theta[j]);
#pragma unroll
  for (int o = 16; o > 0; o >>= 1) { s += __shfl_down_sync(0xffffffffu, s, o); l1 += __shfl_down_sync(0xffffffffu, l1, o); }
  if (lane == 0) { sh[0][wid] = s; sh[1][wid] = l1; }
  __syncthreads();
  if (t == 0) {
    double ssum = sh[0][0], lsum = sh[1][0];
    for (int w = 1; w < NW; w++) { ssum += sh[0][w]; lsum += sh[1][w]; }
    const double l = ssum * inv_n + lsum;
    st->lossval = l;
    if (st->first) st->first = 0;
    else {
      double tmp = st->loss_old; st->loss_old = st->loss_new; st->loss_new = tmp;
      if (eps_loss != 0.0) {
        st->loss_new = l;
        if (st->done == 0 && fabs(st->loss_old - st->loss_new) < eps_loss) st->done = 1;
      }
      if (st->done == 2) st->done = 1;
    }
    s_done = st->done;
  }
  __syncthreads();
  if (!s_done) {
    double mx = 0.0, md = 0.0, nn = 0.0;
    for (int64_t k = t; k < ntheta; k += BT) {
      unsigned long long gi = __ldcg(G + k);
      for (int r = 1; r < replicas; r++) gi += __ldcg(G + r * ntheta + k);
      double g = (double)(long long)gi * inv_scale;
      double t0 = theta[k], t1 = t0 - step * g;
      if (k > 0) {
        if (t1 >= 0.0) t1 = fmax(fabs(t1) - step * lambda, 0.0);
        else           t1 = -fmax(fabs(t1) - step * lambda, 0.0);
      }
      theta[k] = t1;
      if (isnan(t1)) nn = 1.0;
      mx = fmax(mx, fabs(t1));
      md = fmax(md, fabs(t1 - t0));
    }
#pragma unroll
    for (int o = 16; o > 0; o >>= 1) {
      mx = fmax(mx, __shfl_down_sync(0xffffffffu, mx, o));
      md = fmax(md, __shfl_down_sync(0xffffffffu, md, o));
      nn = fmax(nn, __shfl_down_sync(0xffffffffu, nn, o));
    }
    if (lane == 0) { sh[0][wid] = mx; sh[1][wid] = md; sh[2][wid] = nn; }
    __syncthreads();
    if (t == 0) {
      for (int w = 1; w < NW; w++) { mx = fmax(mx, sh[0][w]); md = fmax(md, sh[1][w]); nn = fmax(nn, sh[2][w]); }
      st->iter += 1;
      if (nn != 0.0) { st->delta = nan(""); st->done = 1; }
      else {
        st->delta = mx != 0.0 ? md / mx : md;
        if ((mx != 0.0 && md / mx <= eps) || (mx == 0.0 && md == 0.0)) st->done = 1;
        else if (st->iter >= max_iter) st->done = 2;
// ... 391 lines not shown
  if (threadIdx.x == 0) out[0] = sh[0];
}
__global__ void __launch_bounds__(256) small_tail_kernel(PgState *st, const double *partials, int nparts, double *theta,
                                                         unsigned long long *G, double inv_scale, int64_t ntheta,
                                                         double inv_n, double lambda, double eps_loss, double step,
                                                         double eps, long long max_iter) {
  if (st->done == 1) return;
  small_tail(st, partials, nparts, theta, G, inv_scale, ntheta, inv_n, lambda, eps_loss, step, eps, max_iter);
}

__global__ void __launch_bounds__(256) small_p2p_tail_kernel(PgState *st, const PeerBox *pb, const double *__restrict__ blockloss,
                                                             int nblocks, double *theta, unsigned long long *G,
                                                             double *scratch, double inv_scale, int64_t ntheta, double inv_n,
                                                             double lambda, double eps_loss, double step, double eps,
                                                             long long max_iter) {
  if (st->done == 1) return;
  __shared__ double shs[256];
  __shared__ int s_timeout;
  const int t = threadIdx.x, me = pb->rank, world = pb->world;
  PeerMail *mine = pb->box[me];
  const unsigned long long seq = mine->seq + 1ull;
  const int par = (int)(seq & 1ull);
  if ((int)blockIdx.x < world) {
    const int dst_rank = (int)blockIdx.x;
    double s = 0.0;
    for (int i = t; i < nblocks; i += 256) s += blockloss[i];
    shs[t] = s;
    __syncthreads();
    for (int o = 128; o > 0; o >>= 1) {
      if (t < o) shs[t] += shs[t + o];
      __syncthreads();
    }
    unsigned long long *dst = pb->box[dst_rank]->slot[par][me];
    for (int64_t k = t; k < ntheta; k += 256) dst[k] = G[k];
    if (t == 0) dst[ntheta] = (unsigned long long)__double_as_longlong(shs[0]);
    __threadfence_system();
    __syncthreads();
    if (t == 0) {
      *(volatile unsigned long long *)&pb->box[dst_rank]->flag[par][me] = seq;
      __threadfence();
      atomicAdd(&mine->senders_done, 1u);
    }
    return;
  }
  if (t == 0) s_timeout = 0;
  __syncthreads();
  if (t < world) {
    volatile unsigned long long *g = &mine->flag[par][t];
    const long long t0 = clock64();
    while (*g < seq)
      if (clock64() - t0 > 6000000000LL) { s_timeout = 1; break; }
  }
  if (t == 32) {
    volatile unsigned int *d = &mine->senders_done;
    const long long t0 = clock64();
    while (*d < (unsigned)world)
      if (clock64() - t0 > 6000000000LL) { s_timeout = 1; break; }
  }
  __syncthreads();
  if (s_timeout) {
    if (t == 0) { st->error = 1; st->done = 1; mine->senders_done = 0u; }
    return;
  }
  __threadfence_system();
  for (int64_t k = t; k < ntheta; k += 256) {
    unsigned long long g = 0ull;
    for (int r = 0; r < world; r++) g += __ldcv(&mine->slot[par][r][k]);
    G[k] = g;
  }
  if (t < world) scratch[t] = __longlong_as_double((long long)__ldcv(&mine->slot[par][t][ntheta]));
  __threadfence();
  __syncthreads();
  if (t == 0) { mine->senders_done = 0u; mine->seq = seq; }
  small_tail(st, scratch, world, theta, G, inv_scale, ntheta, inv_n, lambda, eps_loss, step, eps, max_iter);
}

constexpr int PROX_BLOCKS = 256;

struct Work {
  DevBuf<double> theta, w, lossterm, g, red, scalars, gathered, blockmax;
  DevBuf<unsigned long long> G, H;
  DevBuf<double> T, lowtab;
  DevBuf<unsigned long long> q;
  double scale = 1.0, inv_scale = 1.0;
};

template <typename VT>
const VT *csr_val(const Matrix &M);
template <> const uint32_t *csr_val<uint32_t>(const Matrix &M) { return M.vt == VAL_U32 ? M.val_u32.p : nullptr; }
template <> const double *csr_val<double>(const Matrix &M) { return M.val_f64.p; }
template <typename VT>
const VT *sliced_val(const Matrix &M);
template <> const uint32_t *sliced_val<uint32_t>(const Matrix &M) { return M.vt == VAL_U32 ? M.sval_u32.p : nullptr; }
template <> const double *sliced_val<double>(const Matrix &M) { return M.sval_f64.p; }
template <typename VT>
const void *persistent_kernel(bool sharded, int long_mode) {
  if (sharded) return long_mode == 2 ? (const void *)fused_small_persistent<VT, true, 2>
                    : long_mode == 1 ? (const void *)fused_small_persistent<VT, true, 1> : (const void *)fused_small_persistent<VT, true, 0>;
  return long_mode == 2 ? (const void *)fused_small_persistent<VT, false, 2>
       : long_mode == 1 ? (const void *)fused_small_persistent<VT, false, 1> : (const void *)fused_small_persistent<VT, false, 0>;
}
template <typename VT>
const VT *csc_val(const Matrix &M);
template <> const uint32_t *csc_val<uint32_t>(const Matrix &M) { return M.vt == VAL_U32 ? M.cval_u32.p : nullptr; }
template <> const double *csc_val<double>(const Matrix &M) { return M.cval_f64.p; }

inline unsigned warp_grid(int64_t items, int threads) { return (unsigned)((items * 32 + threads - 1) / threads); }

void reduce_sum(const Matrix &M, const double *x, int64_t n, Work &wk, double *out, const PgState *st,
                bool all_ranks = true) {
  KL_LAUNCH(reduce_stage1, RED_BLOCKS, 256, 0, x, n, wk.red.p, st);
  KL_LAUNCH(reduce_stage2, 1, 32, 0, wk.red.p, RED_BLOCKS, out, st);
  if (M.sharded && all_ranks) {
    comm_allgather_f64(out, wk.gathered.p, 1);
    KL_LAUNCH(sum_ranks, 1, 32, 0, wk.gathered.p, ctx().world, (int64_t)1, out);
  }
}

constexpr int64_t PAIR_TERMS_MAX = 8192;
struct PairTerms {
  bool sparse = false;
  DevBuf<PairTerm> dev;
  int n = 0;
};
void collect_pair_terms(const Matrix &M, const double *theta_host, int64_t ntheta, int cooc, PairTerms &T) {
  if (!cooc) return;
  std::vector<PairTerm> h;
  const uint64_t *bits = reinterpret_cast<const uint64_t *>(theta_host);
  for (int64_t j = M.m + 1; j < ntheta; j++) {
    if (j + 8 <= ntheta && (((bits[j] | bits[j + 1] | bits[j + 2] | bits[j + 3] | bits[j + 4] | bits[j + 5] | bits[j + 6] | bits[j + 7]) << 1) == 0)) { j += 7; continue; }
    if (theta_host[j] == 0.0) continue;
    if ((int64_t)h.size() >= PAIR_TERMS_MAX) return;
    int64_t a, b;
    kmerlr_coeff_sub2ind(M.m, j - 1, &a, &b);
    h.push_back(PairTerm{(uint32_t)a, (uint32_t)b, theta_host[j]});
  }
  T.sparse = true; T.n = (int)h.size();
  T.dev.alloc(h.size() ? h.size() : 1);
  T.dev.upload(h.data(), h.size());
  sync_stream();
}

template <typename VT, int MODE>
void launch_rows(const Matrix &M, const double *theta, int cooc, const double cw[2], double *out, double *lossterm,
                 const PgState *st, const PairTerms *T = nullptr) {
  if (M.n == 0) return;
  double inv_n = 1.0 / (double)M.n_global;
  const bool sparse = cooc && T && T->sparse;
  KL_LAUNCH((rows_kernel<VT, MODE>), warp_grid(M.n, 256), 256, 0, M.rows(), M.col.p, csr_val<VT>(M), M.n, M.m,
            theta, sparse ? 2 : cooc, M.labels.p, cw ? cw[0] : 1.0, cw ? cw[1] : 1.0, inv_n, out, lossterm, st,
            sparse ? T->dev.p : (const PairTerm *)nullptr, sparse ? T->n : 0);
}

void set_scale(Matrix &M, Work &wk, const double cw[2]) {
  double bound = std::fmax(std::fabs(cw[0]), std::fabs(cw[1])) * std::fmax(matrix_vmax(M), 1.0);
  if (!(bound > 0.0) || !std::isfinite(bound)) bound = 1.0;
  int e = 60 - (int)std::ceil(std::log2(bound));
  if (e > 1000) e = 1000;
  wk.scale = std::ldexp(1.0, e);
  wk.inv_scale = std::ldexp(1.0, -e);
}

bool use_implicit(const Matrix &M) {
  static int env = -1;
  if (env < 0) { const char *e = getenv("KMERLR_IMPLICIT"); env = (e && *e == '0') ? 0 : 1; }
  if (!(env == 1 && ctx().implicit_ok && M.imp)) return false;
  return M.imp->binarized ? M.vt == VAL_ONE : M.vt == VAL_U32;
}

int super_length(int N) {
  int S = ctx().super_len;
  if (S < 0) S = N <= 8 ? 10 : IMP_SUPER_MAX;
  if (S > IMP_SUPER_MAX) S = IMP_SUPER_MAX;
  return S < N ? N : S;
}

template <int CACHE, bool BIN>
void launch_imp_pass(const ImpParams &P, const ImpArgs &A, size_t smem) {
  if (smem > 48 * 1024)
    KL_CUDA(cudaFuncSetAttribute((imp_pass<CACHE, BIN>), cudaFuncAttributeMaxDynamicSharedMemorySize, (int)smem));
  const int64_t blocks = (A.n + A.rpb - 1) / A.rpb;
  KL_LAUNCH((imp_pass<CACHE, BIN>), (unsigned)blocks, 256, smem, P, A);
}

void launch_implicit(Matrix &M, Work &wk, const double cw[2], const PgState *st, int scatter) {
  const Implicit &I = *M.imp;
  const SeqSet &S = *I.seqs;
  ImpParams P{};
  P.M = I.M; P.N = I.N; P.op = I.op; P.Mlo = I.Mlo;
  for (int k = 0; k < 16; k++) { P.level_off[k] = I.level_off[k]; P.fo[k] = I.fo[k]; }
  const bool levels = I.Mlo <= I.N;
  P.S = levels ? super_length(I.N) : I.N;
  P.c = P.S - I.N + 1;
  const int64_t tlev = levels ? I.fo[I.N + 1] : 0, tsup = P.c > 1 ? (int64_t)1 << (2 * P.S) : 0, total = tlev + tsup;
  P.sup0 = P.c > 1 ? (uint32_t)tlev : I.fo[I.N];
  if (wk.T.n < (size_t)(total ? total : 1)) { wk.T.alloc((size_t)(total ? total : 1)); wk.H.alloc((size_t)(total ? total : 1)); }
  if (scatter && total) KL_CUDA(cudaMemsetAsync(wk.H.p, 0, (size_t)total * sizeof(unsigned long long), ctx().stream));
  if (levels) {
    KL_LAUNCH(imp_build_T, (unsigned)((tlev + 255) / 256), 256, 0, P, I.bitmap.p, I.rank.p, wk.theta.p, wk.T.p, tlev, st);
    if (P.c > 1) KL_LAUNCH(imp_build_TS, (unsigned)((tsup + 255) / 256), 256, 0, P, wk.T.p, st);
  }
  ImpArgs A{};
  A.n = M.n; A.len = S.len.p; A.blk = S.blk.p; A.bits2 = S.bits2.p; A.inv16 = S.inv16.p;
  A.T = wk.T.p; A.theta = wk.theta.p; A.labels = M.labels.p;
  A.cw0 = cw[0]; A.cw1 = cw[1]; A.inv_n = 1.0 / (double)M.n_global; A.scale = wk.scale;
  A.H = wk.H.p; A.G = wk.G.p; A.lossterm = wk.lossterm.p; A.st = st; A.scatter = scatter;
  A.rpb = I.binarized ? 128 : 32;
  while ((M.n + A.rpb - 1) / A.rpb > 0x7fffffffLL) A.rpb *= 2;
  size_t smem = 0;
  if (I.binarized) {
    A.lowbits = I.lowbits.p; A.low_words = I.low_words; A.lwp = I.low_words <= 32 ? 32 : 64;
    if (!wk.lowtab.p) { wk.lowtab.alloc((size_t)128 * 64); wk.q.alloc((size_t)M.n); }
    A.lowtab = wk.lowtab.p; A.evptr = I.evptr.p; A.events = I.events.p; A.q_out = wk.q.p;
    smem = (size_t)128 * A.lwp * sizeof(double);
    KL_LAUNCH(imp_build_low, (unsigned)((128 * A.lwp + 255) / 256), 256, 0, I.lowcol.p, I.low_words, A.lwp, wk.theta.p,
              wk.lowtab.p, st);
  }
  A.gw = (32 - P.S) / P.c + 1;
  const int64_t groups_per_lane = ((S.max_len + P.c - 1) / P.c + 31) / 32;
  const int64_t cached = groups_per_lane <= A.gw ? groups_per_lane : 1000;
  if (I.binarized) {
    if (cached <= 4) launch_imp_pass<4, true>(P, A, smem);
    else if (cached <= 8) launch_imp_pass<8, true>(P, A, smem);
    else launch_imp_pass<0, true>(P, A, smem);
  } else {
    if (cached <= 4) launch_imp_pass<4, false>(P, A, smem);
    else if (cached <= 8) launch_imp_pass<8, false>(P, A, smem);
    else launch_imp_pass<0, false>(P, A, smem);
  }
  if (!scatter) return;
  if (I.binarized)
    for (int w0 = 0; w0 < I.low_words; w0 += 32)
      KL_LAUNCH(low_accumulate, (unsigned)(ctx().sm_count * 2), 256, 0, I.lowbits.p, I.low_words, w0, M.n, wk.q.p, I.lowcol.p,
                wk.G.p, st);
  if (!scatter) return;
  if (!levels) return;
  if (P.c > 1) KL_LAUNCH(imp_fold_super, (unsigned)((tsup + 255) / 256), 256, 0, P, wk.H.p, st);
  for (int j = I.N - 1; j >= I.Mlo; j--)
    KL_LAUNCH(imp_fold_level, (unsigned)(((1u << (2 * j)) + 255) / 256), 256, 0, P, j, wk.H.p, st);
  KL_LAUNCH(imp_columns, (unsigned)((M.m + 255) / 256), 256, 0, P, M.class_ids.p, M.m, wk.H.p, wk.G.p, st);
}

template <typename VT>
void launch_fused(Matrix &M, Work &wk, const double cw[2], const PgState *st, int scatter = 1) {
  if (scatter) KL_CUDA(cudaMemsetAsync(wk.G.p, 0, (size_t)(M.m + 2 + PEER_MAX_WORLD) * sizeof(unsigned long long), ctx().stream));
  if (M.n > 0) {
    if (use_implicit(M)) {
      launch_implicit(M, wk, cw, st, scatter);
    } else {
      int hot = ctx().hot_cols;
      if (hot > M.m) hot = (int)M.m;
      const size_t smem = (size_t)hot * 8;
      KL_CUDA(cudaFuncSetAttribute(fused_kernel<VT>, cudaFuncAttributeMaxDynamicSharedMemorySize, HOT_COLS_MAX * 8));
      const int tk = ctx().fused_ticket;
      if (tk > 0) {
        unsigned long long *ticket = wk.G.p + M.m + 1 + PEER_MAX_WORLD;
        KL_CUDA(cudaMemsetAsync(ticket, 0, sizeof(unsigned long long), ctx().stream));
        int per_sm = 0;
        KL_CUDA(cudaOccupancyMaxActiveBlocksPerMultiprocessor(&per_sm, fused_kernel<VT>, 256, smem));
        if (per_sm < 1) per_sm = 1;
        int64_t blocks = (int64_t)ctx().sm_count * per_sm, need = (M.n + 8 * tk - 1) / (8 * tk);
        if (blocks > need) blocks = need;
        KL_LAUNCH((fused_kernel<VT>), (unsigned)blocks, 256, smem, M.rows(), M.col.p, csr_val<VT>(M), M.n, M.m, wk.theta.p,
                  M.labels.p, cw[0], cw[1], 1.0 / (double)M.n_global, wk.scale, wk.G.p, wk.lossterm.p, st, scatter, hot, tk,
                  ticket);
      } else {
        int rpb = FUSED_RPB;
        while ((M.n + rpb - 1) / rpb > 0x7fffffffLL) rpb *= 2;
        KL_LAUNCH((fused_kernel<VT>), (unsigned)((M.n + rpb - 1) / rpb), 256, smem, M.rows(), M.col.p, csr_val<VT>(M), M.n,
                  M.m, wk.theta.p, M.labels.p, cw[0], cw[1], 1.0 / (double)M.n_global, wk.scale, wk.G.p, wk.lossterm.p, st,
                  scatter, hot, rpb, (unsigned long long *)nullptr);
      }
    }
  }
}

void alloc_work(const Matrix &M, int64_t ntheta, Work &wk) {
  wk.theta.alloc((size_t)ntheta);
  wk.w.alloc((size_t)(M.n ? M.n : 1));
  wk.lossterm.alloc((size_t)(M.n ? M.n : 1));
  wk.g.alloc((size_t)ntheta);
  wk.G.alloc((size_t)M.m + 2 + PEER_MAX_WORLD);
  wk.red.alloc(RED_BLOCKS);
  wk.scalars.alloc(8);
  wk.blockmax.alloc(4 * PROX_BLOCKS);
  wk.gathered.alloc((size_t)(M.sharded ? ntheta * ctx().world : 1));
}

void check_theta(const Matrix &M, int64_t ntheta, int cooc) {
  if (cooc) KL_INVARIANT(ntheta == kmerlr_coeff_dim(M.m));
  else KL_INVARIANT(ntheta == M.m + 1);
}

template <typename F>
void dispatch_vt(const Matrix &M, F &&f) {
  if (M.vt == VAL_F64) f((double *)nullptr);
  else f((uint32_t *)nullptr);
}

}

void linear_pdf(Matrix &M, const double *theta, int64_t ntheta, int cooc, double *out_host, bool logpdf) {
  require_ready();
  check_theta(M, ntheta, cooc);
  DevBuf<double> dth((size_t)ntheta), out((size_t)(M.n ? M.n : 1));
  dth.upload(theta, (size_t)ntheta);
  PairTerms terms;
  collect_pair_terms(M, theta, ntheta, cooc, terms);
  dispatch_vt(M, [&](auto *tag) {
    using VT = typename std::remove_pointer<decltype(tag)>::type;
    if (logpdf) launch_rows<VT, 1>(M, dth.p, cooc, nullptr, out.p, nullptr, nullptr, &terms);
    else launch_rows<VT, 0>(M, dth.p, cooc, nullptr, out.p, nullptr, nullptr, &terms);
  });
  out.download(out_host, (size_t)M.n);
  sync_stream();
}

void gradient(Matrix &M, const double *theta, int64_t ntheta, const double cw[2], double lambda, int cooc,
              double *g_host, DevBuf<double> *g_dev) {
  require_ready();
  check_theta(M, ntheta, cooc);
  KL_REQUIRE(M.has_labels, "gradient: the matrix has no labels (kmerlr_matrix_set_labels)");
  Work wk; alloc_work(M, ntheta, wk);
  set_scale(M, wk, cw);
  wk.theta.upload(theta, (size_t)ntheta);
  wk.g.zero();
  dispatch_vt(M, [&](auto *tag) {
    using VT = typename std::remove_pointer<decltype(tag)>::type;
    if (!cooc) {
      launch_fused<VT>(M, wk, cw, nullptr);
      if (M.sharded) comm_allreduce_sum_i64_fast((int64_t *)wk.G.p, M.m + 1);
    } else {
      PairTerms terms;
      collect_pair_terms(M, theta, ntheta, cooc, terms);
      launch_rows<VT, 2>(M, wk.theta.p, cooc, cw, wk.w.p, wk.lossterm.p, nullptr, &terms);
      ensure_csc(M);
      KL_CUDA(cudaMemsetAsync(wk.G.p, 0, (size_t)(M.m + 1) * sizeof(unsigned long long), ctx().stream));
      if (M.n > 0)
        KL_LAUNCH((scatter_w<VT>), warp_grid(M.n, 256), 256, 0, M.rows(), M.col.p, csr_val<VT>(M), M.n, wk.w.p,
                  wk.scale, wk.G.p);
      if (M.sharded) comm_allreduce_sum_i64((int64_t *)wk.G.p, M.m + 1);
      if (M.m > 1) {
        const int ntile = (int)((M.m + PAIR_T - 1) / PAIR_T);
        const size_t smem = (size_t)PAIR_CH * PAIR_T * sizeof(double) + (size_t)8 * PAIR_CH * (sizeof(double) + sizeof(unsigned short));
        KL_CUDA(cudaFuncSetAttribute(pairs_gradient<VT>, cudaFuncAttributeMaxDynamicSharedMemorySize, (int)smem));
        KL_LAUNCH((pairs_gradient<VT>), (unsigned)((int64_t)ntile * (ntile + 1) / 2), 256, smem, M.colptr.p, M.crow.p,
                  csc_val<VT>(M), M.m, M.n, ntile, wk.w.p, wk.g.p);
        if (M.sharded) {
          comm_allgather_f64(wk.g.p, wk.gathered.p, ntheta);
          KL_LAUNCH(sum_ranks, (unsigned)((ntheta + 255) / 256), 256, 0, wk.gathered.p, ctx().world, ntheta, wk.g.p);
        }
      }
    }
  });
  KL_LAUNCH(finalize_g, (unsigned)((M.m + 1 + 255) / 256), 256, 0, wk.G.p, M.m + 1, wk.inv_scale, wk.g.p);
  if (!std::isnan(lambda) && lambda != 0.0)
    KL_LAUNCH(add_l1_sign, (unsigned)((ntheta + 255) / 256), 256, 0, wk.theta.p, wk.g.p, ntheta, lambda);
  if (g_host) wk.g.download(g_host, (size_t)ntheta);
  sync_stream();
  if (M.sharded) comm_check_peer_errors();
  if (g_dev) *g_dev = std::move(wk.g);
}

double loss(Matrix &M, const double *theta, int64_t ntheta, const double cw[2], double lambda, int cooc) {
  require_ready();
  check_theta(M, ntheta, cooc);
  KL_REQUIRE(M.has_labels, "loss: the matrix has no labels (kmerlr_matrix_set_labels)");
  if (M.n_global == 0) return 0.0;
  Work wk; alloc_work(M, ntheta, wk);
  wk.theta.upload(theta, (size_t)ntheta);
  PairTerms terms;
  collect_pair_terms(M, theta, ntheta, cooc, terms);
  dispatch_vt(M, [&](auto *tag) {
    using VT = typename std::remove_pointer<decltype(tag)>::type;
    launch_rows<VT, 2>(M, wk.theta.p, cooc, cw, wk.w.p, wk.lossterm.p, nullptr, &terms);
  });
  reduce_sum(M, wk.lossterm.p, M.n, wk, wk.scalars.p, nullptr);
  double s = 0.0;
  wk.scalars.download(&s, 1);
  sync_stream();
  double r = s / (double)M.n_global;
  if (!std::isnan(lambda) && lambda != 0.0)
    for (int64_t j = 1; j < M.m + 1; j++) r += lambda * std::fabs(theta[j]);
  return r;
}

void proxgrad(Matrix &M, double *theta, int64_t ntheta, const double cw[2], double lambda, double l2,
              double step_factor, double epsilon, double epsilon_loss, int64_t max_iter, double hook[2],
              int64_t *iters, double *delta) {
  require_ready();
  check_theta(M, ntheta, 0);
  KL_REQUIRE(M.has_labels, "proxgrad: the matrix has no labels (kmerlr_matrix_set_labels)");
  KL_REQUIRE(M.n_global > 0, "proxgrad: empty data set");
  Trace tr("proxgrad");
  double L = 0.25 * (matrix_maxsq(M) + 1.0) + l2 / (double)M.n_global;
  double step = 1.0 / (2.0 * L + std::fmin(2.0 * l2, L)) * step_factor;
  Work wk; alloc_work(M, ntheta, wk);
  set_scale(M, wk, cw);
  wk.theta.upload(theta, (size_t)ntheta);
  DevBuf<PgState> st(1);
  PgState h{};
  h.iter = 0; h.done = max_iter > 0 ? 0 : 1; h.first = 1; h.delta = 0.0;
  h.loss_old = hook ? hook[0] : NAN; h.loss_new = hook ? hook[1] : NAN; h.lossval = NAN; h.error = 0;
  st.upload(&h, 1);
  const double inv_n = 1.0 / (double)M.n_global;
  const bool small = ntheta <= SMALL_MAX_THETA && !use_implicit(M);
  const bool p2p = M.sharded && ctx().peer && ctx().p2p_ok;
  bool persistent = small && ctx().coop_ok && (!M.sharded || p2p);
  bool long_rows = persistent && M.nnz > 0 && (ctx().small_long >= 1 || (ctx().small_long < 0 && M.nnz >= 4 * M.n));
  DevBuf<double> wbuf;
  bool packed = false;
  if (long_rows) { ensure_sliced(M); ensure_csc(M); packed = ensure_packed(M); wbuf.alloc((size_t)M.n); }
  int long_mode = long_rows ? 1 : 0;
  size_t dyn_smem = 0;
  const bool want_block = long_rows && packed && (ctx().small_long == 2 || ctx().small_long < 0);
  const int64_t BATCH = persistent ? 4096 : (small ? 256 : 16);
  int small_blocks = 0;
  DevBuf<double> blockloss;
  DevBuf<unsigned int> counter;
  DevBuf<unsigned long long> G3;
  if (small) {
    int64_t nb = (int64_t)ctx().sm_count * SMALL_BLOCKS_PER_SM, need = (M.n + 63) / 64;
    if (persistent) {
      auto resident = [&](int mode, size_t smem) {
        int per_sm = 0;
        dispatch_vt(M, [&](auto *tag) {
          using VT = typename std::remove_pointer<decltype(tag)>::type;
          if (smem > 16 * 1024)
            KL_CUDA(cudaFuncSetAttribute(persistent_kernel<VT>(M.sharded, mode), cudaFuncAttributeMaxDynamicSharedMemorySize, 32 * 1024));
          KL_CUDA(cudaOccupancyMaxActiveBlocksPerMultiprocessor(&per_sm, persistent_kernel<VT>(M.sharded, mode), PERSIST_THREADS, smem));
        });
        if (ctx().persist_bps > 0 && ctx().persist_bps < per_sm) per_sm = ctx().persist_bps;
        return per_sm;
      };
      if (want_block) {
        int per_sm = resident(2, 0);
        for (int round = 0; round < 4 && per_sm >= 1; round++) {
          int64_t g = (int64_t)ctx().sm_count * per_sm;
          if (g > need) g = need;
          const size_t smem = (size_t)((M.n + g - 1) / g + 1) * sizeof(double);
          const int p2 = smem <= 32 * 1024 ? resident(2, smem) : 0;
          if (p2 >= per_sm) { dyn_smem = smem; break; }
          per_sm = p2;
        }
        if (per_sm >= 1 && dyn_smem > 0) {
          int64_t g = (int64_t)ctx().sm_count * per_sm;
          if (g > need) g = need;
          if (ensure_blockview(M, (int)g)) { long_mode = 2; nb = (int64_t)ctx().sm_count * per_sm; }
          else dyn_smem = 0;
        } else dyn_smem = 0;
      }
      if (long_mode != 2 && long_rows && ctx().small_long < 0 && M.nnz < 8 * M.n) { long_rows = false; long_mode = 0; }
      if (long_mode != 2) {
        const int per_sm = resident(long_mode, 0);
        KL_INVARIANT(per_sm >= 1);
        nb = (int64_t)ctx().sm_count * per_sm;
      }
    }
    small_blocks = (int)(nb < need ? nb : need);
    if (small_blocks < 1) small_blocks = 1;
    blockloss.alloc((size_t)small_blocks * (persistent ? 2 : 1));
    if (persistent) { G3.alloc((size_t)(3 * SMALL_REPLICAS * ntheta)); G3.zero(); }
    counter.alloc(1);
    counter.zero();
    KL_CUDA(cudaMemsetAsync(wk.G.p, 0, (size_t)ntheta * sizeof(unsigned long long), ctx().stream));
  }
  int64_t issued = 0;
  while (true) {
    int64_t nb = max_iter + 1 - issued;
    if (nb > BATCH) nb = BATCH;
    if (nb < 1) nb = 1;
    issued += nb;
    if (persistent) {
      dispatch_vt(M, [&](auto *tag) {
        using VT = typename std::remove_pointer<decltype(tag)>::type;
        Rows rows = M.rows();
        const uint32_t *colp = M.col.p;
        const VT *valp = csr_val<VT>(M);
        int64_t n = M.n, nt = ntheta;
        double *thp = wk.theta.p;
        const uint8_t *lab = M.labels.p;
        double cw0 = cw[0], cw1 = cw[1], invn = inv_n, scale = wk.scale, inv_scale = wk.inv_scale;
        unsigned long long *Gp = G3.p;
        double *bl = blockloss.p;
        PgState *stp = st.p;
        long long pass0 = (long long)(issued - nb), mi = (long long)max_iter;
        int npass = (int)nb;
        double lam = lambda, el = epsilon_loss, stp_size = step, eps = epsilon;
        const PeerBox *pbp = ctx().peer;
        unsigned long long *gx = wk.G.p;
        double *scr = wk.gathered.p;
        unsigned int *abortp = counter.p;
        LongView<VT> lv{};
        if (long_rows) {
          lv.slice_off = M.slice_off.p; lv.scol = M.scol.p; lv.sval = sliced_val<VT>(M);
          lv.colptr = M.colptr.p; lv.crow = M.crow.p; lv.cval = csc_val<VT>(M);
          if (packed) { lv.spack = M.spack.p; lv.cpack = M.cpack.p; lv.row_bits = M.pack_row_bits; }
          lv.wbuf = wbuf.p; lv.nnz = M.nnz;
          if (long_mode == 2) { lv.bv_off = M.bv_off.p; lv.bv_pack = M.bv_pack.p; lv.bv_row_bits = M.bv_row_bits; }
        }
        void *args[] = {&rows, &colp, &valp, &n, &nt, &thp, &lab, &cw0, &cw1, &invn, &scale, &Gp, &bl, &stp, &pass0, &npass,
                        &inv_scale, &lam, &el, &stp_size, &eps, &mi, &pbp, &gx, &scr, &abortp, &lv};
        if (ctx().profiling) profile_begin("fused_small_persistent");
        const cudaError_t e = cudaLaunchCooperativeKernel(
            persistent_kernel<VT>(M.sharded, long_mode),
            dim3((unsigned)small_blocks), dim3(PERSIST_THREADS), args, dyn_smem, ctx().stream);
        if (ctx().profiling) profile_end();
        if (e == cudaErrorCooperativeLaunchTooLarge && !M.sharded) {
          (void)cudaGetLastError();
          persistent = false;
        } else {
          KL_CUDA(e);
          ctx().launches++;
        }
      });
    }
    for (int64_t it = 0; it < nb && !persistent; it++) {
      const int scatter = (issued - nb + it) < max_iter ? 1 : 0;
      if (small) {
        dispatch_vt(M, [&](auto *tag) {
          using VT = typename std::remove_pointer<decltype(tag)>::type;
          KL_LAUNCH((fused_small_kernel<VT>), (unsigned)small_blocks, 256, 0, M.rows(), M.col.p, csr_val<VT>(M), M.n, ntheta,
                    wk.theta.p, M.labels.p, cw[0], cw[1], inv_n, wk.scale, wk.G.p, blockloss.p, st.p, scatter,
                    M.sharded ? (unsigned int *)nullptr : counter.p, wk.inv_scale, lambda, epsilon_loss, step, epsilon,
                    (long long)max_iter);
        });
        if (M.sharded && ctx().peer && ctx().p2p_ok) {
          KL_LAUNCH(small_p2p_tail_kernel, (unsigned)(ctx().world + 1), 256, 0, st.p, ctx().peer, blockloss.p, small_blocks, wk.theta.p, wk.G.p,
                    wk.gathered.p, wk.inv_scale, ntheta, inv_n, lambda, epsilon_loss, step, epsilon, (long long)max_iter);
        } else if (M.sharded) {
          unsigned long long *slots = wk.G.p + ntheta;
          KL_LAUNCH(small_presum_kernel, 1, 256, 0, st.p, blockloss.p, small_blocks, wk.scalars.p);
          KL_LAUNCH(pack_loss_slots, 1, 32, 0, st.p, wk.scalars.p, slots, ctx().rank, ctx().world);
          if (scatter) comm_allreduce_sum_i64((int64_t *)wk.G.p, ntheta + ctx().world);
          else comm_allreduce_sum_i64((int64_t *)slots, ctx().world);
          KL_LAUNCH(small_tail_kernel, 1, 256, 0, st.p, reinterpret_cast<const double *>(slots), ctx().world, wk.theta.p,
                    wk.G.p, wk.inv_scale, ntheta, inv_n, lambda, epsilon_loss, step, epsilon, (long long)max_iter);
        }
        continue;
      }
      dispatch_vt(M, [&](auto *tag) {
        using VT = typename std::remove_pointer<decltype(tag)>::type;
        launch_fused<VT>(M, wk, cw, st.p, scatter);
        reduce_sum(M, wk.lossterm.p, M.n, wk, wk.scalars.p, st.p, false);
        if (M.sharded) {
          unsigned long long *slots = wk.G.p + M.m + 1;
          KL_LAUNCH(pack_loss_slots, 1, 32, 0, st.p, wk.scalars.p, slots, ctx().rank, ctx().world);
          if (scatter) comm_allreduce_sum_i64_fast((int64_t *)wk.G.p, M.m + 1 + ctx().world);
          else comm_allreduce_sum_i64_fast((int64_t *)slots, ctx().world);
          KL_LAUNCH(unpack_loss_slots, 1, 32, 0, st.p, slots, ctx().world, wk.scalars.p);
        }
        KL_LAUNCH(l1_partials, PROX_BLOCKS, 256, 0, st.p, wk.theta.p, M.m + 1, lambda, wk.blockmax.p + 3 * PROX_BLOCKS);
        KL_LAUNCH(hook_kernel, 1, 32, 0, st.p, wk.scalars.p, wk.blockmax.p + 3 * PROX_BLOCKS, PROX_BLOCKS, inv_n, epsilon_loss);
        KL_LAUNCH(prox_update, PROX_BLOCKS, 256, 0, st.p, wk.theta.p, wk.G.p, wk.inv_scale, ntheta, step, lambda,
                  wk.blockmax.p);
        KL_LAUNCH(prox_finish, 1, 32, 0, st.p, wk.blockmax.p, PROX_BLOCKS, epsilon, (long long)max_iter);
      });
    }
    st.download(&h, 1);
    sync_stream();
    if (h.error) fail(KMERLR_ERR_CUDA, "proxgrad: a rank did not answer the gradient exchange over peer memory");
    if (M.sharded) comm_check_peer_errors();
    if (h.done == 1) break;
  }
  wk.theta.download(theta, (size_t)ntheta);
  sync_stream();
  tr.mark("iterations");
  if (hook) { hook[0] = h.loss_old; hook[1] = h.loss_new; }
  if (iters) *iters = (int64_t)h.iter;
  if (delta) *delta = h.delta;
}

}
```

### kmerlr_b200/csrc/matrix.cu

```cuda
#include "common.cuh"

#include <cmath>

namespace kl {

namespace {

constexpr int RS_THREADS = 256;
constexpr int RS_GROUPS = 32;
constexpr int RS_WARP_ITEMS = 32 * RS_GROUPS;
constexpr int RS_TILE = (RS_THREADS / 32) * RS_WARP_ITEMS;

__global__ void __launch_bounds__(RS_THREADS) radix_hist(const uint32_t *__restrict__ keys, int64_t nnz, int shift,
                                                         uint32_t *__restrict__ hist, int64_t ntiles) {
  __shared__ uint32_t h[256];
  h[threadIdx.x] = 0;
  __syncthreads();
  int64_t base = (int64_t)blockIdx.x * RS_TILE;
#pragma unroll 8
  for (int i = 0; i < RS_TILE / RS_THREADS; i++) {
    int64_t p = base + (int64_t)i * RS_THREADS + threadIdx.x;
    if (p < nnz) atomicAdd(&h[(keys[p] >> shift) & 255u], 1u);
  }
  __syncthreads();
// ... 231 lines not shown
      const unsigned long long y = __shfl_xor_sync(0xffffffffu, tm, o);
      tm = y > tm ? y : tm;
    }
    if (lane == 0) { s1[pi] = t1; s2[pi] = t2; mx[pi] = tm; cnt[pi] = tc; }
  }
}

template <typename VT>
__global__ void transform_dense(const Rows R, const uint32_t *__restrict__ col, const VT *__restrict__ val, int64_t n,
                                int64_t m, const double *__restrict__ offset, const double *__restrict__ scale,
                                uint32_t *__restrict__ ocol, double *__restrict__ oval) {
  const int64_t row = ((int64_t)blockIdx.x * blockDim.x + threadIdx.x) >> 5;
  if (row >= n) return;
  int64_t a, b;
  R.range(row, a, b);
  for (int64_t j = lane_id(); j < m; j += 32) {
    int64_t lo = a, hi = b;
    while (lo < hi) { const int64_t mid = (lo + hi) >> 1; if (col[mid] < (uint32_t)j) lo = mid + 1; else hi = mid; }
    const double v = (lo < b && col[lo] == (uint32_t)j) ? (val ? (double)val[lo] : 1.0) : 0.0;
    double t = v - offset[j + 1];
    if (scale) t *= scale[j + 1];
    ocol[row * m + j] = (uint32_t)j;
    oval[row * m + j] = t;
  }
}
template <typename VT>
__global__ void transform_scale(const uint32_t *__restrict__ col, const VT *__restrict__ val, int64_t nnz,
                                const double *__restrict__ scale, double *__restrict__ oval) {
  const int64_t p = (int64_t)blockIdx.x * blockDim.x + threadIdx.x;
  if (p < nnz) oval[p] = (val ? (double)val[p] : 1.0) * scale[col[p] + 1];
}

}

std::shared_ptr<Matrix> matrix_transform(Matrix &M, const double *offset, const double *scale, int64_t len) {
  require_ready();
  KL_REQUIRE(len == M.m + 1, "transform: offset / scale must have one entry per coefficient (m + 1)");
  KL_REQUIRE(offset || scale, "transform: neither offset nor scale given");
  auto R = std::make_shared<Matrix>();
  R->n = M.n; R->m = M.m; R->vt = VAL_F64;
  R->sharded = M.sharded; R->n_global = M.n_global;
  R->n_classes = M.n_classes; R->class_k = M.class_k; R->class_code = M.class_code;
  DevBuf<double> doff, dsc;
  if (offset) { doff.alloc((size_t)len); doff.upload(offset, (size_t)len); }
  if (scale) { dsc.alloc((size_t)len); dsc.upload(scale, (size_t)len); }
  R->rowptr.alloc((size_t)M.n + 1);
  if (offset) {
    KL_REQUIRE(M.n * M.m < ((int64_t)1 << 31), "transform: a data transform with an offset makes the rows dense; "
               "this matrix would not fit (apply it to the reduced matrix of the selected features)");
    R->nnz = M.n * M.m;
    R->col.alloc((size_t)(R->nnz ? R->nnz : 1));
    R->val_f64.alloc((size_t)(R->nnz ? R->nnz : 1));
    std::vector<int64_t> rp((size_t)M.n + 1);
    for (int64_t i = 0; i <= M.n; i++) rp[(size_t)i] = i * M.m;
    R->rowptr.upload(rp.data(), (size_t)M.n + 1);
    if (M.n > 0 && M.m > 0) {
      const unsigned grid = (unsigned)((M.n * 32 + 127) / 128);
      if (M.vt == VAL_U32)
        KL_LAUNCH((transform_dense<uint32_t>), grid, 128, 0, M.rows(), M.col.p, M.val_u32.p, M.n, M.m, doff.p, dsc.p, R->col.p, R->val_f64.p);
      else if (M.vt == VAL_F64)
        KL_LAUNCH((transform_dense<double>), grid, 128, 0, M.rows(), M.col.p, M.val_f64.p, M.n, M.m, doff.p, dsc.p, R->col.p, R->val_f64.p);
      else
        KL_LAUNCH((transform_dense<uint32_t>), grid, 128, 0, M.rows(), M.col.p, (const uint32_t *)nullptr, M.n, M.m, doff.p, dsc.p, R->col.p, R->val_f64.p);
    }
    sync_stream();
  } else {
    matrix_compact(M);
    R->nnz = M.nnz;
    R->col.alloc((size_t)(R->nnz ? R->nnz : 1));
    R->val_f64.alloc((size_t)(R->nnz ? R->nnz : 1));
    KL_CUDA(cudaMemcpyAsync(R->rowptr.p, M.rowptr.p, (size_t)(M.n + 1) * sizeof(int64_t), cudaMemcpyDeviceToDevice, ctx().stream));
    if (M.nnz > 0) {
      KL_CUDA(cudaMemcpyAsync(R->col.p, M.col.p, (size_t)M.nnz * sizeof(uint32_t), cudaMemcpyDeviceToDevice, ctx().stream));
      const unsigned grid = (unsigned)((M.nnz + 255) / 256);
      if (M.vt == VAL_U32) KL_LAUNCH((transform_scale<uint32_t>), grid, 256, 0, M.col.p, M.val_u32.p, M.nnz, dsc.p, R->val_f64.p);
      else if (M.vt == VAL_F64) KL_LAUNCH((transform_scale<double>), grid, 256, 0, M.col.p, M.val_f64.p, M.nnz, dsc.p, R->val_f64.p);
      else KL_LAUNCH((transform_scale<uint32_t>), grid, 256, 0, M.col.p, (const uint32_t *)nullptr, M.nnz, dsc.p, R->val_f64.p);
    }
    sync_stream();
  }
  if (M.has_labels) {
    R->labels.alloc((size_t)(M.n ? M.n : 1));
    KL_CUDA(cudaMemcpyAsync(R->labels.p, M.labels.p, (size_t)M.n, cudaMemcpyDeviceToDevice, ctx().stream));
    R->n_pos = M.n_pos; R->n_neg = M.n_neg; R->counts_global = M.counts_global; R->has_labels = true;
    sync_stream();
  }
  return R;
}

void matrix_pair_moments(Matrix &M, double *sum, double *sumsq, double *absmax, int64_t *count) {
  require_ready();
  KL_REQUIRE(M.vt != VAL_F64, "pair_moments: only count / binarized matrices (integer values) are supported");
  KL_REQUIRE(!M.sharded, "pair_moments: not available on a sharded matrix");
  const int64_t np = M.m * (M.m - 1) / 2;
  if (np <= 0) return;
  ensure_csc(M);
  DevBuf<unsigned long long> d((size_t)(4 * np));
  if (M.vt == VAL_U32)
    KL_LAUNCH((pair_moments<uint32_t>), (unsigned)(ctx().sm_count * 8), 256, 0, M.colptr.p, M.crow.p, M.cval_u32.p, M.m, d.p,
              d.p + np, d.p + 2 * np, d.p + 3 * np);
  else
    KL_LAUNCH((pair_moments<uint32_t>), (unsigned)(ctx().sm_count * 8), 256, 0, M.colptr.p, M.crow.p, (const uint32_t *)nullptr,
              M.m, d.p, d.p + np, d.p + 2 * np, d.p + 3 * np);
  std::vector<unsigned long long> h((size_t)(4 * np));
  d.download(h.data(), (size_t)(4 * np));
  sync_stream();
  for (int64_t j = 0; j < np; j++) {
    sum[j] = (double)h[(size_t)j]; sumsq[j] = (double)h[(size_t)(np + j)];
    absmax[j] = (double)h[(size_t)(2 * np + j)]; count[j] = (int64_t)h[(size_t)(3 * np + j)];
  }
}

void matrix_column_moments(Matrix &M, double *sum, double *sumsq, double *absmax, int64_t *count) {
  require_ready();
  KL_REQUIRE(M.vt != VAL_F64, "column_moments: only count / binarized matrices (integer values) are supported");
  DevBuf<unsigned long long> d((size_t)(4 * (M.m ? M.m : 1)));
  d.zero();
  if (M.n > 0 && M.m > 0)
    KL_LAUNCH((column_moments<uint32_t>), (unsigned)((M.n * 32 + 255) / 256), 256, 0, M.rows(), M.col.p,
              M.vt == VAL_U32 ? M.val_u32.p : (const uint32_t *)nullptr, M.n, d.p, d.p + M.m, d.p + 2 * M.m, d.p + 3 * M.m);
  if (M.sharded) {
    DevBuf<double> mxd((size_t)(M.m ? M.m : 1));
    std::vector<unsigned long long> tmp((size_t)M.m);
    KL_CUDA(cudaMemcpyAsync(tmp.data(), d.p + 2 * M.m, (size_t)M.m * 8, cudaMemcpyDeviceToHost, ctx().stream));
    sync_stream();
    std::vector<double> hm((size_t)M.m);
    for (int64_t j = 0; j < M.m; j++) hm[(size_t)j] = (double)tmp[(size_t)j];
    mxd.upload(hm.data(), (size_t)M.m);
    comm_allreduce_max_f64(mxd.p, M.m);
    mxd.download(hm.data(), (size_t)M.m);
    KL_CUDA(cudaMemsetAsync(d.p + 2 * M.m, 0, (size_t)M.m * 8, ctx().stream));
    comm_allreduce_sum_i64((int64_t *)d.p, 4 * M.m);
    sync_stream();
    for (int64_t j = 0; j < M.m; j++) absmax[j] = hm[(size_t)j];
  }
  std::vector<unsigned long long> h((size_t)(4 * M.m));
  d.download(h.data(), (size_t)(4 * M.m));
  sync_stream();
  for (int64_t j = 0; j < M.m; j++) {
    sum[j] = (double)h[(size_t)j];
    sumsq[j] = (double)h[(size_t)(M.m + j)];
    if (!M.sharded) absmax[j] = (double)h[(size_t)(2 * M.m + j)];
    count[j] = (int64_t)h[(size_t)(3 * M.m + j)];
  }
}

std::shared_ptr<Matrix> matrix_from_csr(int64_t n, int64_t m, const int64_t *rowptr, const int32_t *col,
                                        const double *val, int flags) {
  require_ready();
  KL_REQUIRE(n >= 0 && m >= 0 && rowptr && rowptr[0] == 0, "from_csr: bad arguments");
  int64_t nnz = rowptr[n];
  for (int64_t i = 0; i < n; i++) {
    KL_REQUIRE(rowptr[i + 1] >= rowptr[i], "from_csr: rowptr must be non-decreasing");
    for (int64_t p = rowptr[i]; p < rowptr[i + 1]; p++) {
      KL_REQUIRE(col[p] >= 0 && col[p] < m, "from_csr: column out of range");
      KL_REQUIRE(p == rowptr[i] || col[p] > col[p - 1], "from_csr: columns must be strictly increasing in a row");
    }
  }
  auto M = std::make_shared<Matrix>();
  M->n = n; M->m = m; M->nnz = nnz; M->vt = VAL_F64;
  M->sharded = (flags & KMERLR_FLAG_SHARDED) != 0 && ctx().world > 1;
  M->n_global = n;
  M->rowptr.alloc((size_t)n + 1);
  M->col.alloc((size_t)(nnz ? nnz : 1));
  M->val_f64.alloc((size_t)(nnz ? nnz : 1));
  M->rowptr.upload(rowptr, (size_t)n + 1);
  std::vector<uint32_t> c32((size_t)nnz);
  for (int64_t p = 0; p < nnz; p++) c32[p] = (uint32_t)col[p];
  M->col.upload(c32.data(), (size_t)nnz);
  M->val_f64.upload(val, (size_t)nnz);
  if (M->sharded) {
    DevBuf<int64_t> tmp(1);
    int64_t nn = n;
    tmp.upload(&nn, 1);
    comm_allreduce_sum_i64(tmp.p, 1);
    tmp.download(&nn, 1);
    sync_stream();
    M->n_global = nn;
  }
  sync_stream();
  return M;
}

template <typename VT>
__global__ void gather_rows(const uint32_t *__restrict__ rowcnt, int64_t stride, int64_t n,
                            const int64_t *__restrict__ rowptr, const uint32_t *__restrict__ col,
                            const VT *__restrict__ val, uint32_t *__restrict__ ocol, VT *__restrict__ oval) {
  int64_t row = ((int64_t)blockIdx.x * blockDim.x + threadIdx.x) >> 5;
  if (row >= n) return;
  const unsigned lane = lane_id();
  const int64_t a = row * stride, o = rowptr[row];
  const uint32_t c = rowcnt[row];
  for (uint32_t j = lane; j < c; j += 32) {
    ocol[o + j] = col[a + j];
    if (val) oval[o + j] = val[a + j];
  }
}

void matrix_compact(Matrix &M) {
  if (M.row_stride == 0) return;
  require_ready();
  M.rowptr.alloc((size_t)M.n + 1);
  if (M.n > 0) exclusive_scan_u32_to_i64(M.rowcnt.p, M.rowptr.p, M.n); else M.rowptr.zero();
  DevBuf<uint32_t> ncol((size_t)(M.nnz ? M.nnz : 1)), nval;
  if (M.vt == VAL_U32) nval.alloc((size_t)(M.nnz ? M.nnz : 1));
  if (M.n > 0)
    KL_LAUNCH((gather_rows<uint32_t>), (unsigned)((M.n * 32 + 127) / 128), 128, 0, M.rowcnt.p, M.row_stride, M.n,
              M.rowptr.p, M.col.p, M.vt == VAL_U32 ? M.val_u32.p : (const uint32_t *)nullptr, ncol.p,
              M.vt == VAL_U32 ? nval.p : (uint32_t *)nullptr);
  sync_stream();
  M.col = std::move(ncol);
  if (M.vt == VAL_U32) M.val_u32 = std::move(nval);
  M.rowcnt.release();
  M.row_stride = 0;
}

void matrix_rows(Matrix &M, int64_t *rowptr, int32_t *col, double *val) {
  require_ready();
  matrix_compact(M);
  M.rowptr.download(rowptr, (size_t)M.n + 1);
  std::vector<uint32_t> c32((size_t)M.nnz);
  M.col.download(c32.data(), (size_t)M.nnz);
  std::vector<uint32_t> v32;
  if (M.vt == VAL_U32) { v32.resize((size_t)M.nnz); M.val_u32.download(v32.data(), (size_t)M.nnz); }
  else if (M.vt == VAL_F64) M.val_f64.download(val, (size_t)M.nnz);
  sync_stream();
  for (int64_t p = 0; p < M.nnz; p++) {
    col[p] = (int32_t)c32[p];
    if (M.vt == VAL_U32) val[p] = (double)v32[p];
    else if (M.vt == VAL_ONE) val[p] = 1.0;
  }
}

void matrix_set_labels(Matrix &M, const uint8_t *labels, int64_t n) {
  require_ready();
  KL_REQUIRE(n == M.n, "labels: length does not match the number of rows");
  M.labels.alloc((size_t)(n ? n : 1));
  std::vector<uint8_t> l((size_t)n);
  int64_t ones = 0;
  for (int64_t i = 0; i < n; i++) { const uint8_t v = labels[i] != 0; l[i] = v; ones += v; }
  M.labels.upload(l.data(), (size_t)n);
  sync_stream();
  M.n_neg = n - ones; M.n_pos = ones;
  M.counts_global = !M.sharded;
  M.has_labels = true;
}

void matrix_label_counts(Matrix &M) {
  if (M.counts_global) return;
  int64_t cnt[2] = {M.n_neg, M.n_pos};
  DevBuf<int64_t> tmp(2);
  tmp.upload(cnt, 2);
  comm_allreduce_sum_i64(tmp.p, 2);
  tmp.download(cnt, 2);
  sync_stream();
  M.n_neg = cnt[0]; M.n_pos = cnt[1];
  M.counts_global = true;
}

template <typename VT>
static void build_csc(Matrix &M, const VT *val, VT *cval) {
  const int64_t nnz = M.nnz, ntiles = (nnz + RS_TILE - 1) / RS_TILE;
  int bits = 1;
  while (((int64_t)1 << bits) < M.m) bits++;
  const int passes = (bits + 7) / 8;
  Trace tr("csc");
  DevBuf<uint32_t> hist((size_t)(256 * ntiles));
  DevBuf<int64_t> offs((size_t)(256 * ntiles) + 1);
  DevBuf<uint32_t> kA((size_t)nnz), kB(passes > 1 ? (size_t)nnz : 1), rA(passes > 1 ? (size_t)nnz : 1),
      rB(passes > 2 ? (size_t)nnz : 1);
  DevBuf<VT> vA(val && passes > 1 ? (size_t)nnz : 1), vB(val && passes > 2 ? (size_t)nnz : 1);
  const uint32_t *kin = M.col.p, *rin = nullptr;
  const VT *vin = val;
  tr.mark("alloc");
  for (int ps = 0; ps < passes; ps++) {
    const bool last = ps == passes - 1;
    uint32_t *kout = (ps & 1) ? kB.p : kA.p;
    if (passes == 1) kout = kA.p;
    uint32_t *rout = last ? M.crow.p : ((ps & 1) ? rB.p : rA.p);
    VT *vout = val ? (last ? cval : ((ps & 1) ? vB.p : vA.p)) : nullptr;
    KL_LAUNCH(radix_hist, (unsigned)ntiles, RS_THREADS, 0, kin, nnz, 8 * ps, hist.p, ntiles);
    exclusive_scan_u32_to_i64(hist.p, offs.p, 256 * ntiles);
    const size_t smem = (size_t)RS_TILE * (8 + (val ? sizeof(VT) : 0));
    if (ps == 0) {
      KL_CUDA(cudaFuncSetAttribute(radix_scatter<VT, true>, cudaFuncAttributeMaxDynamicSharedMemorySize, (int)smem));
      KL_LAUNCH((radix_scatter<VT, true>), (unsigned)ntiles, RS_THREADS, smem, kin, rin, M.rowptr.p, M.n, vin, nnz, 8 * ps,
                offs.p, ntiles, kout, rout, vout);
    } else {
      KL_CUDA(cudaFuncSetAttribute(radix_scatter<VT, false>, cudaFuncAttributeMaxDynamicSharedMemorySize, (int)smem));
      KL_LAUNCH((radix_scatter<VT, false>), (unsigned)ntiles, RS_THREADS, smem, kin, rin, M.rowptr.p, M.n, vin, nnz, 8 * ps,
                offs.p, ntiles, kout, rout, vout);
    }
    kin = kout; rin = rout; vin = vout;
    tr.mark("pass");
  }
  KL_LAUNCH(lower_bounds, (unsigned)((M.m + 1 + 255) / 256), 256, 0, kin, nnz, M.m, M.colptr.p);
  sync_stream();
}

void ensure_csc(Matrix &M) {
  if (M.has_csc) return;
  matrix_compact(M);
  M.colptr.alloc((size_t)M.m + 1);
  M.crow.alloc((size_t)(M.nnz ? M.nnz : 1));
  if (M.m == 0 || M.n == 0 || M.nnz == 0) {
    M.colptr.zero();
  } else if (M.vt == VAL_U32) {
    M.cval_u32.alloc((size_t)(M.nnz ? M.nnz : 1));
    build_csc<uint32_t>(M, M.val_u32.p, M.cval_u32.p);
  } else if (M.vt == VAL_F64) {
    M.cval_f64.alloc((size_t)(M.nnz ? M.nnz : 1));
    build_csc<double>(M, M.val_f64.p, M.cval_f64.p);
  } else {
    build_csc<uint32_t>(M, nullptr, nullptr);
  }
  sync_stream();
  M.has_csc = true;
}

__global__ void slice_widths(const int64_t *__restrict__ rowptr, int64_t n, int64_t nslices, uint32_t *__restrict__ width32) {
  const int64_t s = (int64_t)blockIdx.x * blockDim.x + threadIdx.x;
  if (s >= nslices) return;
  int64_t w = 0;
  for (int64_t r = 32 * s; r < 32 * s + 32 && r < n; r++) w = max(w, rowptr[r + 1] - rowptr[r]);
  width32[s] = (uint32_t)w;
}

template <typename VT>
__global__ void slice_fill(const int64_t *__restrict__ rowptr, const uint32_t *__restrict__ col, const VT *__restrict__ val,
                           int64_t n, const int64_t *__restrict__ slice_off, uint32_t *__restrict__ scol, VT *__restrict__ sval) {
  const int64_t row = (int64_t)blockIdx.x * blockDim.x + threadIdx.x;
// ... 124 lines not shown
}

bool ensure_blockview(Matrix &M, int grid) {
  if (M.bv_grid == grid) return M.bv_ok;
  M.bv_grid = grid; M.bv_ok = false;
  if (!ensure_packed(M) || grid < 1 || M.m < 1 || M.m > 1024) return false;
  const int64_t rows = (M.n + grid - 1) / grid + 1;
  int rb = 1;
  while (((int64_t)1 << rb) < rows) rb++;
  if (rb + 10 > 28 || rows * 8 > 32 * 1024) return false;
  DevBuf<int64_t> lb((size_t)(grid + 1) * M.m), start((size_t)grid * M.m);
  DevBuf<uint32_t> width((size_t)grid);
  const uint32_t rmask = (1u << M.pack_row_bits) - 1u;
  KL_LAUNCH(bv_bounds, (unsigned)(((int64_t)(grid + 1) * M.m + 255) / 256), 256, 0, M.colptr.p, M.cpack.p, rmask, M.n, M.m, grid, lb.p);
  KL_LAUNCH(bv_starts, (unsigned)((grid + 127) / 128), 128, 0, lb.p, M.m, grid, start.p, width.p);
  M.bv_off.alloc((size_t)grid + 1);
  exclusive_scan_u32_to_i64(width.p, M.bv_off.p, grid);
  int64_t total = 0;
  KL_CUDA(cudaMemcpyAsync(&total, M.bv_off.p + grid, sizeof(int64_t), cudaMemcpyDeviceToHost, ctx().stream));
  sync_stream();
  M.bv_pack.alloc((size_t)(total > 0 ? 256 * total : 1));
  KL_CUDA(cudaMemsetAsync(M.bv_pack.p, 0xFF, (size_t)(total > 0 ? 256 * total : 1) * sizeof(uint32_t), ctx().stream));
  DevBuf<unsigned int> bad(1);
  bad.zero();
  KL_LAUNCH(bv_fill, (unsigned)(((int64_t)grid * M.m + 255) / 256), 256, 0, lb.p, start.p, width.p, M.bv_off.p, M.cpack.p,
            M.pack_row_bits, M.n, M.m, grid, rb, M.bv_pack.p, bad.p);
  unsigned int nbad = 0;
  bad.download(&nbad, 1);
  sync_stream();
  if (nbad) return false;
  M.bv_row_bits = rb; M.bv_rows = (int)rows;
  M.bv_ok = true;
  return true;
}

std::shared_ptr<Matrix> matrix_reduce(Matrix &M, const int64_t *sel, int64_t nsel) {
  require_ready();
  KL_REQUIRE(nsel >= 1 && sel[0] == 0, "reduce: sel[0] must be the bias (0)");
  const int64_t dim = kmerlr_coeff_dim(M.m);
  std::vector<int64_t> A((size_t)(nsel - 1)), B((size_t)(nsel - 1));
  for (int64_t j = 1; j < nsel; j++) {
    KL_REQUIRE(sel[j] > sel[j - 1] && sel[j] < dim, "reduce: coefficient indices must be ascending and in range");
    if (sel[j] >= M.m + 1) {
      int64_t i1, i2;
      kmerlr_coeff_sub2ind(M.m, sel[j] - 1, &i1, &i2);
      A[j - 1] = i1; B[j - 1] = i2;
    } else {
      A[j - 1] = sel[j] - 1; B[j - 1] = -1;
    }
  }
  auto R = std::make_shared<Matrix>();
  R->n = M.n; R->m = nsel - 1; R->vt = VAL_F64;
  R->sharded = M.sharded; R->n_global = M.n_global;
  const int64_t ns = nsel - 1;
  DevBuf<int64_t> dA((size_t)(ns ? ns : 1)), dB((size_t)(ns ? ns : 1));
  dA.upload(A.data(), (size_t)ns); dB.upload(B.data(), (size_t)ns);
  DevBuf<uint32_t> cnt((size_t)(M.n ? M.n : 1));
  R->rowptr.alloc((size_t)M.n + 1);
  unsigned wgrid = (unsigned)((M.n * 32 + 127) / 128);
  auto run = [&](auto *valp) {
    using VT = typename std::remove_const<typename std::remove_pointer<decltype(valp)>::type>::type;
    if (M.n > 0) {
      KL_LAUNCH((reduce_rows<VT, false>), wgrid, 128, 0, M.rows(), M.col.p, valp, M.n, dA.p, dB.p, ns, cnt.p,
                nullptr, nullptr, nullptr);
      exclusive_scan_u32_to_i64(cnt.p, R->rowptr.p, M.n);
      KL_CUDA(cudaMemcpyAsync(&R->nnz, R->rowptr.p + M.n, sizeof(int64_t), cudaMemcpyDeviceToHost, ctx().stream));
      sync_stream();
    } else {
      R->rowptr.zero(); R->nnz = 0;
    }
    R->col.alloc((size_t)(R->nnz ? R->nnz : 1));
    R->val_f64.alloc((size_t)(R->nnz ? R->nnz : 1));
    if (M.n > 0)
      KL_LAUNCH((reduce_rows<VT, true>), wgrid, 128, 0, M.rows(), M.col.p, valp, M.n, dA.p, dB.p, ns, nullptr,
                R->rowptr.p, R->col.p, R->val_f64.p);
    sync_stream();
  };
  if (M.vt == VAL_U32) run((const uint32_t *)M.val_u32.p);
  else if (M.vt == VAL_F64) run((const double *)M.val_f64.p);
  else run((const uint32_t *)nullptr);
  if (M.has_labels) {
    R->labels.alloc((size_t)(M.n ? M.n : 1));
    KL_CUDA(cudaMemcpyAsync(R->labels.p, M.labels.p, (size_t)M.n, cudaMemcpyDeviceToDevice, ctx().stream));
    R->n_pos = M.n_pos; R->n_neg = M.n_neg; R->counts_global = M.counts_global; R->has_labels = true;
    sync_stream();
  }
  return R;
}

static void ensure_stats(Matrix &M) {
  if (M.has_maxsq && M.has_vmax) return;
  double v[2] = {0.0, 0.0};
  if (M.has_local_stats) {
    v[0] = M.local_maxsq; v[1] = M.local_vmax;
  } else {
    matrix_compact(M);
    DevBuf<unsigned long long> d(2);
    d.zero();
    if (M.n > 0) {
      unsigned wgrid = (unsigned)((M.n * 32 + 127) / 128);
      if (M.vt == VAL_U32) KL_LAUNCH((row_sqnorm_max<uint32_t>), wgrid, 128, 0, M.rows(), M.val_u32.p, M.n, d.p);
      else if (M.vt == VAL_F64) KL_LAUNCH((row_sqnorm_max<double>), wgrid, 128, 0, M.rows(), M.val_f64.p, M.n, d.p);
      else KL_LAUNCH((row_sqnorm_max<uint32_t>), wgrid, 128, 0, M.rows(), (const uint32_t *)nullptr, M.n, d.p);
    }
    if (M.nnz > 0) {
      if (M.vt == VAL_U32) KL_LAUNCH((abs_max<uint32_t>), 1024, 256, 0, M.val_u32.p, M.nnz, d.p + 1);
      else if (M.vt == VAL_F64) KL_LAUNCH((abs_max<double>), 1024, 256, 0, M.val_f64.p, M.nnz, d.p + 1);
    }
    unsigned long long bits[2] = {0, 0};
    d.download(bits, 2);
    sync_stream();
    memcpy(v, bits, sizeof(v));
    if (M.vt == VAL_ONE) v[1] = M.nnz > 0 ? 1.0 : 0.0;
  }
  if (M.sharded) {
    DevBuf<double> t(2);
    t.upload(v, 2);
    comm_allreduce_max_f64(t.p, 2);
    t.download(v, 2);
    sync_stream();
  }
  M.maxsq = v[0]; M.has_maxsq = true;
  M.vmax = v[1]; M.has_vmax = true;
}

double matrix_maxsq(Matrix &M) {
  ensure_stats(M);
  return M.maxsq;
}

double matrix_vmax(Matrix &M) {
  ensure_stats(M);
  return M.vmax;
}

}
```

Before: 53.58 million.

## Cache class numbering, fuse fold/tail kernels, batch host readbacks via pinned staging

Caches the all-classes numbering (bits, rank, interleaved table) in the context so repeated extractions skip rebuilding it. Batches the extraction's small device-to-host reads into one pinned staging download and fuses the row-count sum with the bitmap comparison. Merges the fold-level kernels into a single ticketed kernel that does the small levels in the last block. Fuses the loss reduction, L1 partials and hook into a pass-tail kernel, and counts labels on the GPU. Together these aim to cut launch count and host synchronisation, but they add persistent cached state and ticket-based cross-block ordering that must stay correct.

```diff
diff --git a/kmerlr_b200/csrc/abi.cu b/kmerlr_b200/csrc/abi.cu
--- a/kmerlr_b200/csrc/abi.cu
+++ b/kmerlr_b200/csrc/abi.cu
@@ -52,6 +52,18 @@
   for (auto &kv : g_block_size) cudaFree(kv.first);
   g_block_size.clear();
   g_free_blocks.clear();
+}
+
+void *host_staging(size_t bytes) {
+  KL_CUDA(cudaEventSynchronize(g_ctx.staging_ev));
+  if (bytes > g_ctx.staging_bytes) {
+    if (g_ctx.staging) KL_CUDA(cudaFreeHost(g_ctx.staging));
+    g_ctx.staging = nullptr; g_ctx.staging_bytes = 0;
+    const size_t want = (bytes + ARENA_GRAIN - 1) / ARENA_GRAIN * ARENA_GRAIN;
+    KL_CUDA(cudaMallocHost(&g_ctx.staging, want));
+    g_ctx.staging_bytes = want;
+  }
+  return g_ctx.staging;
 }
 
 namespace {
@@ -214,6 +226,7 @@
 
     KL_CUDA(cudaEventCreate(&g_ctx.ev0));
     KL_CUDA(cudaEventCreate(&g_ctx.ev1));
+    KL_CUDA(cudaEventCreateWithFlags(&g_ctx.staging_ev, cudaEventDisableTiming));
     g_ctx.ready = true;
   }, false);
 }
@@ -226,6 +239,8 @@
       arena_release_all();
       comm_destroy();
       cudaEventDestroy(g_ctx.ev0); cudaEventDestroy(g_ctx.ev1);
+      cudaEventDestroy(g_ctx.staging_ev);
+      if (g_ctx.staging) cudaFreeHost(g_ctx.staging);
       cudaStreamSynchronize(g_ctx.copy_stream);
       for (int i = 0; i < CTX_COPY_EVENTS; i++) cudaEventDestroy(g_ctx.copy_ev[i]);
       cudaStreamDestroy(g_ctx.copy_stream);
diff --git a/kmerlr_b200/csrc/common.cuh b/kmerlr_b200/csrc/common.cuh
--- a/kmerlr_b200/csrc/common.cuh
+++ b/kmerlr_b200/csrc/common.cuh
@@ -60,6 +60,7 @@
 };
 
 constexpr int CTX_COPY_EVENTS = 11;
+struct Numbering;
 struct Ctx {
   bool ready = false;
   int device = 0;
@@ -70,6 +71,10 @@
   cudaEvent_t join_ev[2] = {nullptr, nullptr};
   cudaEvent_t copy_ev[CTX_COPY_EVENTS] = {nullptr};
   cudaEvent_t ev0 = nullptr, ev1 = nullptr;
+  void *staging = nullptr;
+  size_t staging_bytes = 0;
+  cudaEvent_t staging_ev = nullptr;
+  std::vector<std::shared_ptr<const Numbering>> numbering;
   int64_t launches = 0;
   double last_ms = 0.0;
   bool profiling = false;
@@ -105,6 +110,9 @@
 
 inline void sync_stream() { KL_CUDA(cudaStreamSynchronize(ctx().stream)); }
 
+void *host_staging(size_t bytes);
+inline void host_staging_done() { KL_CUDA(cudaEventRecord(ctx().staging_ev, ctx().stream)); }
+
 struct Trace {
   bool on;
   std::chrono::steady_clock::time_point t0, last;
@@ -180,6 +188,14 @@
 
 enum ValType : int { VAL_ONE = 0, VAL_U32 = 1, VAL_F64 = 2 };
 
+struct Numbering {
+  int M = 0, N = 0, op = 0;
+  int64_t nw = 0;
+  uint32_t count = 0;
+  DevBuf<uint32_t> bits, rank;
+  DevBuf<uint2> nbx;
+};
+
 constexpr int IMP_MAX_N = 10;
 constexpr int IMP_SUPER_MAX = 11;
 constexpr uint32_t NOCOL = 0xFFFFFFFFu;
@@ -189,7 +205,7 @@
   int Mlo = 0;
   uint32_t level_off[16] = {0};
   uint32_t fo[16] = {0};
-  DevBuf<uint32_t> bitmap, rank;
+  std::shared_ptr<const Numbering> num;
   bool binarized = false;
   int low_words = 0;
   DevBuf<uint32_t> lowbits;
@@ -241,6 +257,8 @@
   DevBuf<uint8_t> labels;
   int64_t n_pos = 0, n_neg = 0;
   bool counts_global = true;
+  bool counts_pending = false;
+  DevBuf<unsigned long long> label_ones;
   int64_t n_classes = 0;
   DevBuf<uint32_t> class_ids;
   int class_M = 0, class_N = 0;
@@ -292,6 +310,7 @@
                                         const double *val, int flags);
 void matrix_rows(Matrix &M, int64_t *rowptr, int32_t *col, double *val);
 void matrix_set_labels(Matrix &M, const uint8_t *labels, int64_t n);
+void matrix_label_counts_local(Matrix &M);
 void matrix_label_counts(Matrix &M);
 void matrix_column_moments(Matrix &M, double *sum, double *sumsq, double *absmax, int64_t *count);
 void matrix_pair_moments(Matrix &M, double *sum, double *sumsq, double *absmax, int64_t *count);
diff --git a/kmerlr_b200/csrc/extract.cu b/kmerlr_b200/csrc/extract.cu
--- a/kmerlr_b200/csrc/extract.cu
+++ b/kmerlr_b200/csrc/extract.cu
@@ -113,10 +113,20 @@
   int64_t w = (int64_t)blockIdx.x * blockDim.x + threadIdx.x;
   if (w < nw) out[w] = make_uint2(bits[w], rank[w]);
 }
-__global__ void bitmaps_differ(const uint32_t *__restrict__ a, const uint32_t *__restrict__ b, int64_t nw,
-                               uint32_t *__restrict__ flag) {
-  int64_t w = (int64_t)blockIdx.x * blockDim.x + threadIdx.x;
-  if (w < nw && a[w] != b[w]) atomicOr(flag, 1u);
+__global__ void extract_totals(const uint32_t *__restrict__ rowcnt, int64_t n, const uint32_t *__restrict__ a,
+                               const uint32_t *__restrict__ b, int64_t nw, unsigned long long *__restrict__ tot) {
+  __shared__ unsigned long long sh;
+  if (threadIdx.x == 0) sh = 0ull;
+  __syncthreads();
+  const int64_t stride = (int64_t)gridDim.x * blockDim.x, i0 = (int64_t)blockIdx.x * blockDim.x + threadIdx.x;
+  unsigned long long s = 0ull;
+  for (int64_t i = i0; i < n; i += stride) s += rowcnt[i];
+  if (b)
+    for (int64_t w = i0; w < nw; w += stride)
+      if (a[w] != b[w]) tot[3] = 1ull;
+  if (s) atomicAdd(&sh, s);
+  __syncthreads();
+  if (threadIdx.x == 0 && sh) atomicAdd(tot, sh);
 }
 __global__ void renumber_rows(uint32_t *__restrict__ col, const uint32_t *__restrict__ rowcnt, int64_t stride, int64_t n,
                               const uint32_t *__restrict__ ids, const uint32_t *__restrict__ bm,
@@ -398,6 +408,29 @@
   return out;
 }
 
+static void number_set(Numbering &S) {
+  const int64_t nw = S.nw;
+  DevBuf<uint32_t> pc((size_t)nw);
+  KL_LAUNCH(popc_words, (unsigned)((nw + 255) / 256), 256, 0, S.bits.p, nw, pc.p);
+  exclusive_scan_u32(pc.p, S.rank.p, nw);
+  S.nbx.alloc((size_t)nw);
+  KL_LAUNCH(interleave_numbering, (unsigned)((nw + 255) / 256), 256, 0, S.bits.p, S.rank.p, nw, S.nbx.p);
+}
+
+static std::shared_ptr<const Numbering> numbering_all(const LevelInfo &LI, int64_t nw) {
+  for (auto &s : ctx().numbering)
+    if (s->M == LI.M && s->N == LI.N && s->op == LI.op) return s;
+  auto S = std::make_shared<Numbering>();
+  S->M = LI.M; S->N = LI.N; S->op = LI.op; S->nw = nw;
+  S->bits.alloc((size_t)nw); S->rank.alloc((size_t)nw + 1);
+  KL_LAUNCH(all_classes_bits, (unsigned)((nw + 255) / 256), 256, 0, LI, S->bits.p, nw);
+  number_set(*S);
+  KL_CUDA(cudaMemcpyAsync(&S->count, S->rank.p + nw, sizeof(uint32_t), cudaMemcpyDeviceToHost, ctx().stream));
+  sync_stream();
+  ctx().numbering.push_back(S);
+  return S;
+}
+
 static std::shared_ptr<Matrix> extract_impl(const kmerlr_config &cfg, std::shared_ptr<SeqSet> seqs,
                                             const int32_t *frozen_k, const uint64_t *frozen_code, int64_t n_frozen,
                                             const int32_t *features, int64_t n_features, int flags, HostFeed *feed) {
@@ -488,11 +521,12 @@
   if (!P.binarize) out->val_u32.alloc((size_t)(s.n ? s.n * stride : 1));
   out->rowcnt.alloc((size_t)(s.n ? s.n : 1));
   DevBuf<uint32_t> dummy_cnt(1);
-  DevBuf<uint32_t> nb((size_t)nw), nbrank((size_t)nw + 1), pc((size_t)nw), bitmap((size_t)nw);
+  DevBuf<uint32_t> bitmap((size_t)nw);
   std::vector<uint32_t> frozen_bits;
   LevelInfo LI{};
   LI.M = cfg.M; LI.N = cfg.N; LI.op = P.op;
   for (int k = cfg.M; k <= cfg.N + 1; k++) LI.level_off[k] = P.level_off[k];
+  std::shared_ptr<const Numbering> num;
   if (n_frozen > 0) {
     frozen_bits.assign((size_t)nw, 0u);
     uint64_t prev = 0;
@@ -504,22 +538,23 @@
       prev = id;
       frozen_bits[id >> 5] |= 1u << (id & 31);
     }
-    nb.upload(frozen_bits.data(), (size_t)nw);
+    auto F = std::make_shared<Numbering>();
+    F->M = cfg.M; F->N = cfg.N; F->op = P.op; F->nw = nw; F->count = (uint32_t)n_frozen;
+    F->bits.alloc((size_t)nw); F->rank.alloc((size_t)nw + 1);
+    F->bits.upload(frozen_bits.data(), (size_t)nw);
+    number_set(*F);
+    num = F;
   } else {
-    KL_LAUNCH(all_classes_bits, (unsigned)((nw + 255) / 256), 256, 0, LI, nb.p, nw);
-  }
-  KL_LAUNCH(popc_words, (unsigned)((nw + 255) / 256), 256, 0, nb.p, nw, pc.p);
-  exclusive_scan_u32(pc.p, nbrank.p, nw);
+    num = numbering_all(LI, nw);
+  }
+  DevBuf<unsigned long long> tot(9);
+  tot.zero();
   bitmap.zero();
   DevBuf<uint32_t> full(1);
   full.zero();
   P.full = full.p; P.nb_words = nw;
-  DevBuf<unsigned long long> stats(2);
-  stats.zero();
   P.st_id = out->col.p; P.st_cnt = P.binarize ? dummy_cnt.p : out->val_u32.p; P.rowcnt = out->rowcnt.p;
-  DevBuf<uint2> nbx((size_t)nw);
-  KL_LAUNCH(interleave_numbering, (unsigned)((nw + 255) / 256), 256, 0, nb.p, nbrank.p, nw, nbx.p);
-  P.bitmap = bitmap.p; P.nbx = nbx.p; P.filter = n_frozen > 0; P.stats = stats.p;
+  P.bitmap = bitmap.p; P.nbx = num->nbx.p; P.filter = n_frozen > 0; P.stats = tot.p + 1;
   P.mark = n_frozen == 0;
   DevBuf<uint32_t> lowbits, rowdup;
   if (hybrid) {
@@ -579,37 +614,38 @@
     P.row0 = 0; P.n = s.n;
   }
   tr.mark("extract_kernel");
-  DevBuf<uint32_t> differ(1);
-  differ.zero();
-  DevBuf<unsigned long long> gres(3);
+  unsigned long long *const gres = tot.p + 6;
   if (sharded) {
     const int64_t xw = n_frozen == 0 ? nw : 0, per = xw + 6;
     DevBuf<uint32_t> mine((size_t)per), all((size_t)(per * ctx().world));
-    KL_LAUNCH(pack_exchange, (unsigned)((xw + 256) / 256), 256, 0, bitmap.p, xw, (unsigned long long)s.n, stats.p, mine.p);
+    KL_LAUNCH(pack_exchange, (unsigned)((xw + 256) / 256), 256, 0, bitmap.p, xw, (unsigned long long)s.n, tot.p + 1, mine.p);
     comm_allgather_bytes(mine.p, all.p, per * 4);
-    KL_LAUNCH(merge_exchange, (unsigned)((xw + 256) / 256), 256, 0, all.p, ctx().world, xw, bitmap.p, gres.p);
-  }
-  if (n_frozen == 0)
-    KL_LAUNCH(bitmaps_differ, (unsigned)((nw + 255) / 256), 256, 0, bitmap.p, nb.p, nw, differ.p);
-  DevBuf<int64_t> rp((size_t)s.n + 1);
-  if (s.n > 0) exclusive_scan_u32_to_i64(out->rowcnt.p, rp.p, s.n); else rp.zero();
-  int64_t nn = s.n;
-  unsigned long long hres[3] = {0, 0, 0};
-  if (sharded) gres.download(hres, 3);
-  uint32_t m32 = 0, hdiffer = 0;
-  unsigned long long hstats[2] = {0, 0};
+    KL_LAUNCH(merge_exchange, (unsigned)((xw + 256) / 256), 256, 0, all.p, ctx().world, xw, bitmap.p, gres);
+  }
+  {
+    int64_t blocks = ((s.n > nw ? s.n : nw) + 255) / 256;
+    if (blocks > 4 * ctx().sm_count) blocks = 4 * ctx().sm_count;
+    KL_LAUNCH(extract_totals, (unsigned)(blocks ? blocks : 1), 256, 0, out->rowcnt.p, s.n, bitmap.p,
+              n_frozen == 0 ? num->bits.p : (const uint32_t *)nullptr, nw, tot.p);
+  }
   DevBuf<int64_t> evptr;
-  int64_t n_events = 0;
   if (hybrid) {
     evptr.alloc((size_t)s.n + 1);
     exclusive_scan_u32_to_i64(rowdup.p, evptr.p, s.n);
-    KL_CUDA(cudaMemcpyAsync(&n_events, evptr.p + s.n, sizeof(int64_t), cudaMemcpyDeviceToHost, ctx().stream));
-  }
-  KL_CUDA(cudaMemcpyAsync(&m32, nbrank.p + nw, sizeof(uint32_t), cudaMemcpyDeviceToHost, ctx().stream));
-  KL_CUDA(cudaMemcpyAsync(&out->nnz, rp.p + s.n, sizeof(int64_t), cudaMemcpyDeviceToHost, ctx().stream));
-  differ.download(&hdiffer, 1);
-  stats.download(hstats, 2);
+    KL_CUDA(cudaMemcpyAsync(tot.p + 4, evptr.p + s.n, sizeof(int64_t), cudaMemcpyDeviceToDevice, ctx().stream));
+  }
+  uint32_t m32 = num->count;
+  out->class_ids.alloc((size_t)(m32 ? m32 : 1));
+  KL_LAUNCH(enumerate_bits, (unsigned)((nw + 255) / 256), 256, 0, num->bits.p, num->rank.p, nw, out->class_ids.p);
+  unsigned long long *htot = (unsigned long long *)host_staging(9 * sizeof(unsigned long long));
+  tot.download(htot, 9);
+  host_staging_done();
   sync_stream();
+  out->nnz = (int64_t)htot[0];
+  const unsigned long long hstats[2] = {htot[1], htot[2]}, hres[3] = {htot[6], htot[7], htot[8]};
+  const bool hdiffer = htot[3] != 0;
+  const int64_t n_events = (int64_t)htot[4];
+  int64_t nn = s.n;
   if (sharded) {
     nn = (int64_t)hres[0];
     out->maxsq = (double)hres[1]; out->vmax = (double)hres[2];
@@ -620,22 +656,28 @@
   out->local_maxsq = (double)hstats[0]; out->local_vmax = (double)hstats[1];
   tr.mark("sizes");
   if (hdiffer) {
-    DevBuf<uint32_t> rank2((size_t)nw + 1), ids_nb((size_t)(m32 ? m32 : 1));
-    KL_LAUNCH(popc_words, (unsigned)((nw + 255) / 256), 256, 0, bitmap.p, nw, pc.p);
-    exclusive_scan_u32(pc.p, rank2.p, nw);
-    KL_LAUNCH(enumerate_bits, (unsigned)((nw + 255) / 256), 256, 0, nb.p, nbrank.p, nw, ids_nb.p);
+    auto obs = std::make_shared<Numbering>();
+    obs->M = cfg.M; obs->N = cfg.N; obs->op = P.op; obs->nw = nw;
+    obs->rank.alloc((size_t)nw + 1);
+    {
+      DevBuf<uint32_t> pc((size_t)nw);
+      KL_LAUNCH(popc_words, (unsigned)((nw + 255) / 256), 256, 0, bitmap.p, nw, pc.p);
+      exclusive_scan_u32(pc.p, obs->rank.p, nw);
+    }
     if (s.n > 0)
-      KL_LAUNCH(renumber_rows, (unsigned)((s.n * 32 + 127) / 128), 128, 0, out->col.p, out->rowcnt.p, stride, s.n, ids_nb.p,
-                bitmap.p, rank2.p, hybrid ? rowdup.p : (const uint32_t *)nullptr);
-    KL_CUDA(cudaMemcpyAsync(&m32, rank2.p + nw, sizeof(uint32_t), cudaMemcpyDeviceToHost, ctx().stream));
+      KL_LAUNCH(renumber_rows, (unsigned)((s.n * 32 + 127) / 128), 128, 0, out->col.p, out->rowcnt.p, stride, s.n,
+                out->class_ids.p, bitmap.p, obs->rank.p, hybrid ? rowdup.p : (const uint32_t *)nullptr);
+    KL_CUDA(cudaMemcpyAsync(&obs->count, obs->rank.p + nw, sizeof(uint32_t), cudaMemcpyDeviceToHost, ctx().stream));
     sync_stream();
-    nb = std::move(bitmap); nbrank = std::move(rank2);
+    obs->bits = std::move(bitmap);
+    m32 = obs->count;
+    num = obs;
+    out->class_ids.alloc((size_t)(m32 ? m32 : 1));
+    KL_LAUNCH(enumerate_bits, (unsigned)((nw + 255) / 256), 256, 0, num->bits.p, num->rank.p, nw, out->class_ids.p);
     tr.mark("renumber");
   }
   out->m = (int64_t)m32;
   out->n_classes = (int64_t)m32;
-  out->class_ids.alloc((size_t)(m32 ? m32 : 1));
-  KL_LAUNCH(enumerate_bits, (unsigned)((nw + 255) / 256), 256, 0, nb.p, nbrank.p, nw, out->class_ids.p);
   out->class_M = cfg.M; out->class_N = cfg.N; out->classes_on_host = false;
   for (int k = cfg.M; k <= cfg.N + 1; k++) out->class_level_off[k] = P.level_off[k];
   if (n_features > 0) { sync_stream(); return apply_features(*out, features, n_features); }
@@ -654,14 +696,14 @@
       imp->low_words = P.low_words;
       imp->lowcol.alloc((size_t)(P.low_words ? P.low_words * 32 : 1));
       if (P.low_words)
-        KL_LAUNCH(low_columns, (unsigned)((P.low_words * 32 + 127) / 128), 128, 0, P.tl, P.tl_cnt, P.low_words * 32, nb.p,
-                  nbrank.p, imp->lowcol.p);
+        KL_LAUNCH(low_columns, (unsigned)((P.low_words * 32 + 127) / 128), 128, 0, P.tl, P.tl_cnt, P.low_words * 32,
+                  num->bits.p, num->rank.p, imp->lowcol.p);
       imp->lowbits = std::move(lowbits);
       imp->events.alloc((size_t)(n_events ? n_events : 1));
       KL_LAUNCH(gather_events, (unsigned)((s.n * 32 + 127) / 128), 128, 0, out->col.p, stride, s.n, evptr.p, imp->events.p);
       imp->evptr = std::move(evptr);
     }
-    imp->bitmap = std::move(nb); imp->rank = std::move(nbrank);
+    imp->num = num;
     out->imp = imp;
   }
   sync_stream();
diff --git a/kmerlr_b200/csrc/logistic.cu b/kmerlr_b200/csrc/logistic.cu
--- a/kmerlr_b200/csrc/logistic.cu
+++ b/kmerlr_b200/csrc/logistic.cu
@@ -204,14 +204,40 @@
   T[P.sup0 + U] = s;
 }
 
-__global__ void imp_fold_super(const ImpParams P, unsigned long long *__restrict__ H, const PgState *st) {
+constexpr int IMP_FOLD_TAIL = 7;
+constexpr int IMP_FOLD_THREADS = 1024;
+__global__ void __launch_bounds__(IMP_FOLD_THREADS) imp_fold(const ImpParams P, int level, int tail_top,
+                                                             unsigned long long *__restrict__ H, unsigned int *ticket,
+                                                             const PgState *st) {
   if (st && st->done == 1) return;
-  const uint32_t U = blockIdx.x * blockDim.x + threadIdx.x;
-  if (U >= (1u << (2 * P.S))) return;
-  const unsigned long long h = H[P.sup0 + U];
-  if (!h) return;
-  const uint32_t maskN = (1u << (2 * P.N)) - 1u;
-  for (int t = 0; t < P.c; t++) atomicAdd(H + P.fo[P.N] + ((U >> (2 * (P.S - P.N - t))) & maskN), h);
+  const uint32_t u = blockIdx.x * blockDim.x + threadIdx.x;
+  if (level == P.N) {
+    if (u < (1u << (2 * P.S))) {
+      const unsigned long long h = H[P.sup0 + u];
+      const uint32_t maskN = (1u << (2 * P.N)) - 1u;
+      if (h)
+        for (int t = 0; t < P.c; t++) atomicAdd(H + P.fo[P.N] + ((u >> (2 * (P.S - P.N - t))) & maskN), h);
+    }
+  } else if (level >= P.Mlo && u < (1u << (2 * level))) {
+    const unsigned long long *c = H + P.fo[level + 1] + 4ull * u;
+    H[P.fo[level] + u] += c[0] + c[1] + c[2] + c[3];
+  }
+  if (tail_top < P.Mlo) return;
+  __shared__ int s_last;
+  __threadfence();
+  __syncthreads();
+  if (threadIdx.x == 0) s_last = atomicAdd(ticket, 1u) == gridDim.x - 1 ? 1 : 0;
+  __syncthreads();
+  if (!s_last) return;
+  __threadfence();
+  for (int j = tail_top; j >= P.Mlo; j--) {
+    for (uint32_t v = threadIdx.x; v < (1u << (2 * j)); v += blockDim.x) {
+      const unsigned long long *c = H + P.fo[j + 1] + 4ull * v;
+      H[P.fo[j] + v] = __ldcg(H + P.fo[j] + v) + __ldcg(c) + __ldcg(c + 1) + __ldcg(c + 2) + __ldcg(c + 3);
+    }
+    __syncthreads();
+  }
+  if (threadIdx.x == 0) *ticket = 0u;
 }
 
 __global__ void imp_build_low(const uint32_t *__restrict__ lowcol, int low_words, int lwp,
@@ -487,20 +513,8 @@
   }
 }
 
-__global__ void imp_fold_level(const ImpParams P, int j, unsigned long long *__restrict__ H, const PgState *st) {
-  if (st && st->done == 1) return;
-  const uint32_t u = blockIdx.x * blockDim.x + threadIdx.x;
-  if (u >= (1u << (2 * j))) return;
-  const unsigned long long *c = H + P.fo[j + 1] + 4ull * u;
-  H[P.fo[j] + u] += c[0] + c[1] + c[2] + c[3];
-}
-
-__global__ void imp_columns(const ImpParams P, const uint32_t *__restrict__ col_id, int64_t m,
-                            const unsigned long long *__restrict__ F, unsigned long long *__restrict__ G,
-                            const PgState *st) {
-  if (st && st->done == 1) return;
-  const int64_t j = (int64_t)blockIdx.x * blockDim.x + threadIdx.x;
-  if (j >= m) return;
+__device__ __forceinline__ void imp_column(const ImpParams &P, const uint32_t *__restrict__ col_id, int64_t j,
+                                           const unsigned long long *__restrict__ F, unsigned long long *__restrict__ G) {
   const uint32_t id = col_id[j];
   int k = P.M;
   while (k < P.N && id >= P.level_off[k + 1]) k++;
@@ -639,40 +653,14 @@
   const int r = threadIdx.x;
   if (r < world) slots[r] = r == rank ? (unsigned long long)__double_as_longlong(local[0]) : 0ull;
 }
-__global__ void unpack_loss_slots(const PgState *st, const unsigned long long *__restrict__ slots, int world,
-                                  double *__restrict__ out) {
-  if (st && st->done == 1) return;
-  if (threadIdx.x == 0) {
-    double s = 0.0;
-    for (int r = 0; r < world; r++) s += __longlong_as_double((long long)slots[r]);
-    out[0] = s;
-  }
-}
-
-__global__ void l1_partials(const PgState *st, const double *__restrict__ theta, int64_t ntheta, double lambda,
-                            double *__restrict__ l1part) {
-  if (st && st->done == 1) return;
-  __shared__ double sh[256];
-  double s = 0.0;
-  if (!isnan(lambda) && lambda != 0.0)
-    for (int64_t j = 1 + (int64_t)blockIdx.x * blockDim.x + threadIdx.x; j < ntheta; j += (int64_t)gridDim.x * blockDim.x)
-      s += lambda * fabs(theta[j]);
-  sh[threadIdx.x] = s;
-  __syncthreads();
-  for (int o = 128; o > 0; o >>= 1) {
-    if ((int)threadIdx.x < o) sh[threadIdx.x] += sh[threadIdx.x + o];
-    __syncthreads();
-  }
-  if (threadIdx.x == 0) l1part[blockIdx.x] = sh[0];
-}
-__global__ void hook_kernel(PgState *st, const double *__restrict__ losssum, const double *__restrict__ l1part, int nparts,
-                            double inv_n, double eps_loss) {
-  if (st->done == 1) return;
+
+__device__ __forceinline__ void hook_warp(PgState *st, double losssum, const double *l1part, int nparts, double inv_n,
+                                          double eps_loss) {
   double l1 = 0.0;
-  for (int b = threadIdx.x; b < nparts; b += 32) l1 += l1part[b];
+  for (int b = (int)lane_id(); b < nparts; b += 32) l1 += __ldcg(l1part + b);
   l1 = warp_sum_down(l1);
-  if (threadIdx.x == 0) {
-    double l = losssum[0] * inv_n + l1;
+  if (lane_id() == 0) {
+    double l = losssum * inv_n + l1;
     st->lossval = l;
     if (st->first) { st->first = 0; return; }
     double t = st->loss_old; st->loss_old = st->loss_new; st->loss_new = t;
@@ -684,11 +672,72 @@
   }
 }
 
-__global__ void prox_update(const PgState *st, double *__restrict__ theta, const unsigned long long *__restrict__ G,
+__global__ void unpack_loss_hook(PgState *st, const unsigned long long *__restrict__ slots, int world,
+                                 double *__restrict__ out, const double *l1part, int nparts, double inv_n, double eps_loss) {
+  if (st->done == 1) return;
+  double s = 0.0;
+  if (threadIdx.x == 0) {
+    for (int r = 0; r < world; r++) s += __longlong_as_double((long long)slots[r]);
+    out[0] = s;
+  }
+  hook_warp(st, s, l1part, nparts, inv_n, eps_loss);
+}
+
+__device__ __forceinline__ double block_sum_256(double *sh, double v) {
+  sh[threadIdx.x] = v;
+  __syncthreads();
+  for (int o = 128; o > 0; o >>= 1) {
+    if ((int)threadIdx.x < o) sh[threadIdx.x] += sh[threadIdx.x + o];
+    __syncthreads();
+  }
+  const double r = sh[0];
+  __syncthreads();
+  return r;
+}
+
+__global__ void __launch_bounds__(256) pass_tail(PgState *st, const ImpParams P, const uint32_t *__restrict__ col_id,
+                                                 int64_t m, const unsigned long long *__restrict__ F,
+                                                 unsigned long long *__restrict__ G, const double *__restrict__ lossterm,
+                                                 int64_t n, double *__restrict__ part, double *__restrict__ losssum,
+                                                 const double *__restrict__ theta, int64_t ntheta, double lambda,
+                                                 double *__restrict__ l1part, int hook, double inv_n, double eps_loss,
+                                                 unsigned int *ticket) {
+  if (st && st->done == 1) return;
+  __shared__ double sh[256];
+  __shared__ int s_last;
+  const int64_t stride = (int64_t)gridDim.x * blockDim.x, i0 = (int64_t)blockIdx.x * blockDim.x + threadIdx.x;
+  if (F)
+    for (int64_t j = i0; j < m; j += stride) imp_column(P, col_id, j, F, G);
+  double s = 0.0;
+  for (int64_t i = i0; i < n; i += stride) s += lossterm[i];
+  s = block_sum_256(sh, s);
+  if (threadIdx.x == 0) part[blockIdx.x] = s;
+  double l1 = 0.0;
+  if (!isnan(lambda) && lambda != 0.0)
+    for (int64_t j = 1 + i0; j < ntheta; j += stride) l1 += lambda * fabs(theta[j]);
+  l1 = block_sum_256(sh, l1);
+  if (threadIdx.x == 0) l1part[blockIdx.x] = l1;
+  __threadfence();
+  __syncthreads();
+  if (threadIdx.x == 0) s_last = atomicAdd(ticket, 1u) == gridDim.x - 1 ? 1 : 0;
+  __syncthreads();
+  if (!s_last) return;
+  __threadfence();
+  if (threadIdx.x < 32) {
+    double t = 0.0;
+    for (int i = threadIdx.x; i < (int)gridDim.x; i += 32) t += __ldcg(part + i);
+    t = warp_sum_down(t);
+    if (threadIdx.x == 0) { losssum[0] = t; *ticket = 0u; }
+    if (hook) hook_warp(st, t, l1part, (int)gridDim.x, inv_n, eps_loss);
+  }
+}
+
+__global__ void prox_update(PgState *st, double *__restrict__ theta, const unsigned long long *__restrict__ G,
                             double inv_scale, int64_t ntheta, double step, double lambda,
-                            double *__restrict__ blockmax) {
+                            double *__restrict__ blockmax, double eps, long long max_iter, unsigned int *ticket) {
   if (st->done) return;
   __shared__ double shx[256], shd[256], shn[256];
+  __shared__ int s_last;
   double mx = 0.0, md = 0.0, nn = 0.0;
   for (int64_t k = (int64_t)blockIdx.x * blockDim.x + threadIdx.x; k < ntheta; k += (int64_t)gridDim.x * blockDim.x) {
     double g = (double)(long long)G[k] * inv_scale;
@@ -713,12 +762,15 @@
     __syncthreads();
   }
   if (threadIdx.x == 0) { blockmax[3 * blockIdx.x] = shx[0]; blockmax[3 * blockIdx.x + 1] = shd[0]; blockmax[3 * blockIdx.x + 2] = shn[0]; }
-}
-__global__ void prox_finish(PgState *st, const double *__restrict__ blockmax, int nblocks, double eps, long long max_iter) {
-  if (st->done) return;
-  double mx = 0.0, md = 0.0, nn = 0.0;
-  for (int i = threadIdx.x; i < nblocks; i += 32) {
-    mx = fmax(mx, blockmax[3 * i]); md = fmax(md, blockmax[3 * i + 1]); nn = fmax(nn, blockmax[3 * i + 2]);
+  __threadfence();
+  __syncthreads();
+  if (threadIdx.x == 0) s_last = atomicAdd(ticket, 1u) == gridDim.x - 1 ? 1 : 0;
+  __syncthreads();
+  if (!s_last || threadIdx.x >= 32) return;
+  __threadfence();
+  mx = 0.0; md = 0.0; nn = 0.0;
+  for (int i = threadIdx.x; i < (int)gridDim.x; i += 32) {
+    mx = fmax(mx, __ldcg(blockmax + 3 * i)); md = fmax(md, __ldcg(blockmax + 3 * i + 1)); nn = fmax(nn, __ldcg(blockmax + 3 * i + 2));
   }
 #pragma unroll
   for (int o = 16; o > 0; o >>= 1) {
@@ -727,6 +779,7 @@
     nn = fmax(nn, __shfl_xor_sync(0xffffffffu, nn, o));
   }
   if (threadIdx.x == 0) {
+    *ticket = 0u;
     st->iter += 1;
     if (nn != 0.0) { st->delta = nan(""); st->done = 1; return; }
     st->delta = mx != 0.0 ? md / mx : md;
@@ -1284,7 +1337,10 @@
   DevBuf<unsigned long long> G, H;
   DevBuf<double> T, lowtab;
   DevBuf<unsigned long long> q;
+  DevBuf<unsigned int> tickets;
   double scale = 1.0, inv_scale = 1.0;
+  const unsigned long long *F = nullptr;
+  ImpParams P{};
 };
 
 template <typename VT>
@@ -1392,6 +1448,7 @@
   P.M = I.M; P.N = I.N; P.op = I.op; P.Mlo = I.Mlo;
   for (int k = 0; k < 16; k++) { P.level_off[k] = I.level_off[k]; P.fo[k] = I.fo[k]; }
   const bool levels = I.Mlo <= I.N;
+  wk.F = nullptr;
   P.S = levels ? super_length(I.N) : I.N;
   P.c = P.S - I.N + 1;
   const int64_t tlev = levels ? I.fo[I.N + 1] : 0, tsup = P.c > 1 ? (int64_t)1 << (2 * P.S) : 0, total = tlev + tsup;
@@ -1399,7 +1456,7 @@
   if (wk.T.n < (size_t)(total ? total : 1)) { wk.T.alloc((size_t)(total ? total : 1)); wk.H.alloc((size_t)(total ? total : 1)); }
   if (scatter && total) KL_CUDA(cudaMemsetAsync(wk.H.p, 0, (size_t)total * sizeof(unsigned long long), ctx().stream));
   if (levels) {
-    KL_LAUNCH(imp_build_T, (unsigned)((tlev + 255) / 256), 256, 0, P, I.bitmap.p, I.rank.p, wk.theta.p, wk.T.p, tlev, st);
+    KL_LAUNCH(imp_build_T, (unsigned)((tlev + 255) / 256), 256, 0, P, I.num->bits.p, I.num->rank.p, wk.theta.p, wk.T.p, tlev, st);
     if (P.c > 1) KL_LAUNCH(imp_build_TS, (unsigned)((tsup + 255) / 256), 256, 0, P, wk.T.p, st);
   }
   ImpArgs A{};
@@ -1437,10 +1494,19 @@
                 wk.G.p, st);
   if (!scatter) return;
   if (!levels) return;
-  if (P.c > 1) KL_LAUNCH(imp_fold_super, (unsigned)((tsup + 255) / 256), 256, 0, P, wk.H.p, st);
-  for (int j = I.N - 1; j >= I.Mlo; j--)
-    KL_LAUNCH(imp_fold_level, (unsigned)(((1u << (2 * j)) + 255) / 256), 256, 0, P, j, wk.H.p, st);
-  KL_LAUNCH(imp_columns, (unsigned)((M.m + 255) / 256), 256, 0, P, M.class_ids.p, M.m, wk.H.p, wk.G.p, st);
+  const int small_top = I.N - 1 < IMP_FOLD_TAIL ? I.N - 1 : IMP_FOLD_TAIL;
+  int steps[IMP_MAX_N + 1], nsteps = 0;
+  if (P.c > 1) steps[nsteps++] = I.N;
+  for (int j = I.N - 1; j > small_top && j >= I.Mlo; j--) steps[nsteps++] = j;
+  if (nsteps == 0 && small_top >= I.Mlo) steps[nsteps++] = -1;
+  for (int s = 0; s < nsteps; s++) {
+    const int j = steps[s];
+    const int64_t items = j == I.N ? tsup : (j < 0 ? 1 : (int64_t)1 << (2 * j));
+    KL_LAUNCH(imp_fold, (unsigned)((items + IMP_FOLD_THREADS - 1) / IMP_FOLD_THREADS), IMP_FOLD_THREADS, 0, P, j,
+              s == nsteps - 1 ? small_top : -1, wk.H.p, wk.tickets.p, st);
+  }
+  wk.P = P;
+  wk.F = wk.H.p;
 }
 
 template <typename VT>
@@ -1487,6 +1553,16 @@
   wk.scalars.alloc(8);
   wk.blockmax.alloc(4 * PROX_BLOCKS);
   wk.gathered.alloc((size_t)(M.sharded ? ntheta * ctx().world : 1));
+  wk.tickets.alloc(3);
+  wk.tickets.zero();
+}
+
+void launch_pass_tail(const Matrix &M, Work &wk, PgState *st, int64_t ntheta, double lambda, int hook, double eps_loss) {
+  static_assert(RED_BLOCKS == PROX_BLOCKS, "the L1 partials of pass_tail are the hook's PROX_BLOCKS partials");
+  KL_LAUNCH(pass_tail, RED_BLOCKS, 256, 0, st, wk.P, M.class_ids.p, M.m, wk.F, wk.G.p, wk.lossterm.p, st ? M.n : 0,
+            wk.red.p, wk.scalars.p, wk.theta.p, st ? ntheta : 0, lambda, wk.blockmax.p + 3 * PROX_BLOCKS, hook,
+            1.0 / (double)M.n_global, eps_loss, wk.tickets.p + 1);
+  wk.F = nullptr;
 }
 
 void check_theta(const Matrix &M, int64_t ntheta, int cooc) {
@@ -1531,6 +1607,7 @@
     using VT = typename std::remove_pointer<decltype(tag)>::type;
     if (!cooc) {
       launch_fused<VT>(M, wk, cw, nullptr);
+      if (wk.F) launch_pass_tail(M, wk, nullptr, ntheta, NAN, 0, 0.0);
       if (M.sharded) comm_allreduce_sum_i64_fast((int64_t *)wk.G.p, M.m + 1);
     } else {
       PairTerms terms;
@@ -1599,12 +1676,16 @@
   double step = 1.0 / (2.0 * L + std::fmin(2.0 * l2, L)) * step_factor;
   Work wk; alloc_work(M, ntheta, wk);
   set_scale(M, wk, cw);
-  wk.theta.upload(theta, (size_t)ntheta);
+  double *hth = (double *)host_staging((size_t)ntheta * sizeof(double) + sizeof(PgState));
+  PgState *hst = reinterpret_cast<PgState *>(hth + ntheta);
+  memcpy(hth, theta, (size_t)ntheta * sizeof(double));
+  wk.theta.upload(hth, (size_t)ntheta);
   DevBuf<PgState> st(1);
   PgState h{};
   h.iter = 0; h.done = max_iter > 0 ? 0 : 1; h.first = 1; h.delta = 0.0;
   h.loss_old = hook ? hook[0] : NAN; h.loss_new = hook ? hook[1] : NAN; h.lossval = NAN; h.error = 0;
-  st.upload(&h, 1);
+  *hst = h;
+  st.upload(hst, 1);
   const double inv_n = 1.0 / (double)M.n_global;
   const bool small = ntheta <= SMALL_MAX_THETA && !use_implicit(M);
   const bool p2p = M.sharded && ctx().peer && ctx().p2p_ok;
@@ -1744,29 +1825,30 @@
       dispatch_vt(M, [&](auto *tag) {
         using VT = typename std::remove_pointer<decltype(tag)>::type;
         launch_fused<VT>(M, wk, cw, st.p, scatter);
-        reduce_sum(M, wk.lossterm.p, M.n, wk, wk.scalars.p, st.p, false);
+        launch_pass_tail(M, wk, st.p, M.m + 1, lambda, M.sharded ? 0 : 1, epsilon_loss);
         if (M.sharded) {
           unsigned long long *slots = wk.G.p + M.m + 1;
           KL_LAUNCH(pack_loss_slots, 1, 32, 0, st.p, wk.scalars.p, slots, ctx().rank, ctx().world);
           if (scatter) comm_allreduce_sum_i64_fast((int64_t *)wk.G.p, M.m + 1 + ctx().world);
           else comm_allreduce_sum_i64_fast((int64_t *)slots, ctx().world);
-          KL_LAUNCH(unpack_loss_slots, 1, 32, 0, st.p, slots, ctx().world, wk.scalars.p);
+          KL_LAUNCH(unpack_loss_hook, 1, 32, 0, st.p, slots, ctx().world, wk.scalars.p, wk.blockmax.p + 3 * PROX_BLOCKS,
+                    PROX_BLOCKS, inv_n, epsilon_loss);
         }
-        KL_LAUNCH(l1_partials, PROX_BLOCKS, 256, 0, st.p, wk.theta.p, M.m + 1, lambda, wk.blockmax.p + 3 * PROX_BLOCKS);
-        KL_LAUNCH(hook_kernel, 1, 32, 0, st.p, wk.scalars.p, wk.blockmax.p + 3 * PROX_BLOCKS, PROX_BLOCKS, inv_n, epsilon_loss);
-        KL_LAUNCH(prox_update, PROX_BLOCKS, 256, 0, st.p, wk.theta.p, wk.G.p, wk.inv_scale, ntheta, step, lambda,
-                  wk.blockmax.p);
-        KL_LAUNCH(prox_finish, 1, 32, 0, st.p, wk.blockmax.p, PROX_BLOCKS, epsilon, (long long)max_iter);
+        if (scatter)
+          KL_LAUNCH(prox_update, PROX_BLOCKS, 256, 0, st.p, wk.theta.p, wk.G.p, wk.inv_scale, ntheta, step, lambda,
+                    wk.blockmax.p, epsilon, (long long)max_iter, wk.tickets.p + 2);
       });
     }
-    st.download(&h, 1);
+    st.download(hst, 1);
+    wk.theta.download(hth, (size_t)ntheta);
+    host_staging_done();
     sync_stream();
+    h = *hst;
     if (h.error) fail(KMERLR_ERR_CUDA, "proxgrad: a rank did not answer the gradient exchange over peer memory");
     if (M.sharded) comm_check_peer_errors();
     if (h.done == 1) break;
   }
-  wk.theta.download(theta, (size_t)ntheta);
-  sync_stream();
+  memcpy(theta, hth, (size_t)ntheta * sizeof(double));
   tr.mark("iterations");
   if (hook) { hook[0] = h.loss_old; hook[1] = h.loss_new; }
   if (iters) *iters = (int64_t)h.iter;
diff --git a/kmerlr_b200/csrc/matrix.cu b/kmerlr_b200/csrc/matrix.cu
--- a/kmerlr_b200/csrc/matrix.cu
+++ b/kmerlr_b200/csrc/matrix.cu
@@ -337,6 +337,7 @@
   if (M.has_labels) {
     R->labels.alloc((size_t)(M.n ? M.n : 1));
     KL_CUDA(cudaMemcpyAsync(R->labels.p, M.labels.p, (size_t)M.n, cudaMemcpyDeviceToDevice, ctx().stream));
+    matrix_label_counts_local(M);
     R->n_pos = M.n_pos; R->n_neg = M.n_neg; R->counts_global = M.counts_global; R->has_labels = true;
     sync_stream();
   }
@@ -487,21 +488,52 @@
   }
 }
 
+__global__ void normalize_labels(uint8_t *__restrict__ labels, int64_t n, unsigned long long *__restrict__ ones) {
+  __shared__ unsigned int sh;
+  if (threadIdx.x == 0) sh = 0u;
+  __syncthreads();
+  unsigned int c = 0;
+  for (int64_t i = (int64_t)blockIdx.x * blockDim.x + threadIdx.x; i < n; i += (int64_t)gridDim.x * blockDim.x) {
+    const uint8_t v = labels[i] != 0;
+    labels[i] = v;
+    c += v;
+  }
+  if (c) atomicAdd(&sh, c);
+  __syncthreads();
+  if (threadIdx.x == 0 && sh) atomicAdd(ones, (unsigned long long)sh);
+}
+
 void matrix_set_labels(Matrix &M, const uint8_t *labels, int64_t n) {
   require_ready();
   KL_REQUIRE(n == M.n, "labels: length does not match the number of rows");
   M.labels.alloc((size_t)(n ? n : 1));
-  std::vector<uint8_t> l((size_t)n);
-  int64_t ones = 0;
-  for (int64_t i = 0; i < n; i++) { const uint8_t v = labels[i] != 0; l[i] = v; ones += v; }
-  M.labels.upload(l.data(), (size_t)n);
-  sync_stream();
-  M.n_neg = n - ones; M.n_pos = ones;
+  M.label_ones.alloc(1);
+  M.label_ones.zero();
+  if (n > 0) {
+    uint8_t *h = (uint8_t *)host_staging((size_t)n);
+    memcpy(h, labels, (size_t)n);
+    M.labels.upload(h, (size_t)n);
+    host_staging_done();
+    int64_t blocks = (n + 255) / 256;
+    if (blocks > 4 * ctx().sm_count) blocks = 4 * ctx().sm_count;
+    KL_LAUNCH(normalize_labels, (unsigned)blocks, 256, 0, M.labels.p, n, M.label_ones.p);
+  }
+  M.counts_pending = true;
   M.counts_global = !M.sharded;
   M.has_labels = true;
 }
 
+void matrix_label_counts_local(Matrix &M) {
+  if (!M.counts_pending) return;
+  unsigned long long ones = 0;
+  M.label_ones.download(&ones, 1);
+  sync_stream();
+  M.n_pos = (int64_t)ones; M.n_neg = M.n - (int64_t)ones;
+  M.counts_pending = false;
+}
+
 void matrix_label_counts(Matrix &M) {
+  matrix_label_counts_local(M);
   if (M.counts_global) return;
   int64_t cnt[2] = {M.n_neg, M.n_pos};
   DevBuf<int64_t> tmp(2);
@@ -792,6 +824,7 @@
   if (M.has_labels) {
     R->labels.alloc((size_t)(M.n ? M.n : 1));
     KL_CUDA(cudaMemcpyAsync(R->labels.p, M.labels.p, (size_t)M.n, cudaMemcpyDeviceToDevice, ctx().stream));
+    matrix_label_counts_local(M);
     R->n_pos = M.n_pos; R->n_neg = M.n_neg; R->counts_global = M.counts_global; R->has_labels = true;
     sync_stream();
   }
```

Result: faster. 58.74 million, median of 6 (+9.6%).
